# zhoupc/CNMF_E

Hardware: AMD Instinct MI355X
Metric: cnmfe_iters_per_sec (higher is better)
Workload: dtype f32; 1 GPU; c3: 512x512x10000 fp32 video, K=500, ring_radius=15, 1x1 patches of distribute_data.m (1 resident blocks per GPU), spatial=hals, deconv_flag=false, bg_ssub=1; lanes_per_rank=1, parallelism=patches round-robin over 1 rank(s)

## Files before the change

### cnmf_e_amd/csrc/api.hip

```cpp
#include "common.hpp"
#include <mutex>
#include <hip/hip_fp16.h>
#include <math.h>
#include <dlfcn.h>

namespace cnmfe {
thread_local char g_err[1024] = "";

template <class S> __device__ inline float to_f32(S v) { return (float)v; }
template <> __device__ inline float to_f32<__half>(__half v) { return __half2float(v); }

template <class S>
__global__ void k_convert(const S *__restrict__ src, float *__restrict__ dst, int64_t n) {
    int64_t i = (int64_t)blockIdx.x * blockDim.x + threadIdx.x;
    int64_t stride = (int64_t)gridDim.x * blockDim.x;
    for (; i < n; i += stride) dst[i] = to_f32<S>(src[i]);
}

__global__ void k_ymean(const float *__restrict__ Y, int64_t d_b, int64_t T, double *__restrict__ ym, float *__restrict__ ymf) {
    int64_t q = (int64_t)blockIdx.x * blockDim.x + threadIdx.x;
    if (q >= d_b) return;
    double s0 = 0, s1 = 0, s2 = 0, s3 = 0;
    int64_t t = 0;
    for (; t + 3 < T; t += 4) {
// ... 110 lines not shown
int download_traces(cnmfe_ctx *ctx, const float *dC, int64_t ldc, float *C, int32_t K, int64_t T, int order) {
    if (K == 0 || !C) return 0;
    if (order == CNMFE_BOUND || order == CNMFE_BOUND_ROWS) order = ctx->bound_order;
    if (order == CNMFE_ROWMAJOR) {
        CK(hipMemcpy2DAsync(C, T * sizeof(float), dC, ldc * sizeof(float), T * sizeof(float), K, hipMemcpyDeviceToHost, ctx->st()));
    } else {
        RET(ctx->stage.ensure((size_t)K * T * sizeof(float)));
        dim3 g((unsigned)((T + 31) / 32), (unsigned)((K + 31) / 32)), b(32, 8);
        LAUNCH(ctx, "transpose_out", k_transpose_out, g, b, 0, dC, ldc, ctx->stage.as<float>(), K, T);
        CK(hipMemcpyAsync(C, ctx->stage.p, (size_t)K * T * sizeof(float), hipMemcpyDeviceToHost, ctx->st()));
    }
    CK(hipStreamSynchronize(ctx->st()));
    return 0;
}

__global__ void __launch_bounds__(256) k_pin_copy(PinSegs s) {
    const int g = blockIdx.y;
    const uint4 *__restrict__ src = s.src[g]; uint4 *__restrict__ dst = s.dst[g];
    const unsigned n16 = s.n16[g];
    for (unsigned i = blockIdx.x * 256u + threadIdx.x; i < n16; i += gridDim.x * 256u) dst[i] = src[i];
}
static std::mutex g_pin_mu;
static std::vector<cnmfe_ctx *> g_pin_live;
void pin_register(cnmfe_ctx *ctx, bool live) {
    std::lock_guard<std::mutex> lk(g_pin_mu);
    auto it = std::find(g_pin_live.begin(), g_pin_live.end(), ctx);
    if (live && it == g_pin_live.end()) g_pin_live.push_back(ctx);
    if (!live && it != g_pin_live.end()) g_pin_live.erase(it);
}
static void flush_locked(cnmfe_ctx *ctx) {
    if (!ctx->npseg) return;
    PinSegs &pseg = ctx->pseg;
    unsigned mx = 0;
    for (int i = 0; i < ctx->npseg; ++i) mx = std::max(mx, pseg.n16[i]);
    for (int i = ctx->npseg; i < PIN_NSEG; ++i) { pseg.src[i] = nullptr; pseg.dst[i] = nullptr; pseg.n16[i] = 0; }
    const unsigned nb = std::min<unsigned>((mx + 255) / 256, 256);
    const int n = ctx->npseg; ctx->npseg = 0;
    hipLaunchKernelGGL(k_pin_copy, dim3(nb, (unsigned)n), dim3(256), 0, ctx->stream_, pseg);
}
void pin_flush_range(const void *p, size_t bytes) {
    std::lock_guard<std::mutex> lk(g_pin_mu);
    const char *lo = (const char *)p, *hi = lo + bytes;
    int cur = -1;
    for (cnmfe_ctx *c : g_pin_live) {
        bool hit = false;
        for (int i = 0; i < c->npseg && !hit; ++i) { const char *d_ = (const char *)c->pseg.dst[i]; hit = d_ >= lo && d_ < hi; }
        if (!hit) continue;
        if (cur < 0) (void)hipGetDevice(&cur);
        if (c->device != cur) (void)hipSetDevice(c->device);
        flush_locked(c);
        if (c->device != cur) (void)hipSetDevice(cur);
    }
}
void pin_flush_all() {
    std::lock_guard<std::mutex> lk(g_pin_mu);
    int cur = -1;
    for (cnmfe_ctx *c : g_pin_live) {
        if (!c->npseg) continue;
        if (cur < 0) (void)hipGetDevice(&cur);
        if (c->device != cur) (void)hipSetDevice(c->device);
        flush_locked(c);
        if (c->device != cur) (void)hipSetDevice(cur);
    }
}
int pinned_to_dev(cnmfe_ctx *ctx, void *dst, const void *src_pinned, size_t bytes) {
    if (bytes > (size_t(8) << 20)) { CK(hipMemcpyAsync(dst, src_pinned, bytes, hipMemcpyHostToDevice, ctx->st())); return 0; }
    std::lock_guard<std::mutex> lk(g_pin_mu);
    if (ctx->npseg == PIN_NSEG) flush_locked(ctx);
    const int i = ctx->npseg++;
    ctx->pseg.src[i] = (const uint4 *)src_pinned; ctx->pseg.dst[i] = (uint4 *)dst; ctx->pseg.n16[i] = (unsigned)((bytes + 15) / 16);
    return 0;
}
}
int cnmfe_ctx::copy_batch_mark() {
    hipEvent_t e;
    if (!copy_ev_pool.empty()) { e = copy_ev_pool.back(); copy_ev_pool.pop_back(); }
    else CK(hipEventCreateWithFlags(&e, hipEventDisableTiming));
    CK(hipEventRecord(e, copy_stream));
    copy_gens.push_back({++copy_gen, e});
    return 0;
}
void cnmfe_ctx::flush_copies() {
    std::lock_guard<std::mutex> lk(cnmfe::g_pin_mu);
    cnmfe::flush_locked(this);
}
namespace cnmfe {

bool bound_rows_of(const cnmfe_ctx *ctx, const float *C, int c_order, int32_t K, std::vector<int32_t> &rows) {
    rows.clear();
    if (!ctx->bound_valid || K <= 0) return false;
    if (c_order == CNMFE_BOUND) {
        if (K != ctx->bound_K) return false;
        rows.resize((size_t)K);
        for (int32_t k = 0; k < K; ++k) rows[k] = k;
        return true;
    }
    if (c_order == CNMFE_BOUND_ROWS && C) {
        const int32_t *r = reinterpret_cast<const int32_t *>(C);
        for (int32_t k = 0; k < K; ++k) if (r[k] < 0 || r[k] >= ctx->bound_K) return false;
        rows.assign(r, r + K);
        return true;
    }
    return false;
}

int ensure_ymean(cnmfe_ctx *ctx, Patch *P) {
    if (P->ymean_valid) return 0;
    if (P->frames_uploaded < P->T) return fail(CNMFE_ESTATE, "block has %lld of %lld frames uploaded", (long long)P->frames_uploaded, (long long)P->T);
    RET(P->ymean_d.ensure(P->d_b * sizeof(double)));
    RET(P->ymean_f.ensure(P->d_b * sizeof(float)));
    LAUNCH(ctx, "ymean", k_ymean, dim3((unsigned)((P->d_b + 255) / 256)), dim3(256), 0,
           P->Y.as<float>(), P->d_b, P->T, P->ymean_d.as<double>(), P->ymean_f.as<float>());
    P->Tc = (P->T + 3) / 4;
    RET(P->Yc4.ensure((size_t)P->Tc * P->d_b * sizeof(float4)));
    LAUNCH(ctx, "center4", k_center4, dim3((unsigned)((P->d_b + 255) / 256), (unsigned)P->Tc), dim3(256), 0,
           P->Y.as<float>(), P->ymean_f.as<float>(), P->d_b, P->T, P->Yc4.as<float4>());
    CK(hipStreamSynchronize(ctx->st()));
    (void)hipFree(P->Y.p); P->Y.p = nullptr; P->Y.cap = 0;
    P->ymean_valid = true;
    return 0;
}

__global__ void k_ring_pmax(const float *__restrict__ W, int64_t d, int p, int *__restrict__ pmax) {
    int64_t m = (int64_t)blockIdx.x * blockDim.x + threadIdx.x;
    int c = 0;
    if (m < d) {
        int i = 0;
        for (; i + 16 <= p; i += 16) {
            float w[16];
#pragma unroll
            for (int u = 0; u < 16; ++u) w[u] = W[(int64_t)(i + u) * d + m];
#pragma unroll
            for (int u = 0; u < 16; ++u) c += w[u] > 0.f;
        }
        for (; i < p; ++i) c += W[(int64_t)i * d + m] > 0.f;
    }
    for (int o = 32; o > 0; o >>= 1) { int v = __shfl_xor(c, o); c = v > c ? v : c; }
    if ((threadIdx.x & 63) == 0) atomicMax(pmax, c);
}
static bool first_run_of_row(const Patch *P, const float *row0) {
    std::vector<float> u;
    const int r = P->prect[0], c = P->prect[2];
    int nvalid = 0;
    for (int i = 0; i < P->p; ++i) {
        const int rr = r + P->dr[i], cc = c + P->dc[i];
        if (rr < 1 || rr > P->d1 || cc < 1 || cc > P->d2) continue;
        ++nvalid; u.push_back(row0[i]);
    }
    if (nvalid < P->d_b) u.push_back(0.f);
    std::sort(u.begin(), u.end());
    u.erase(std::unique(u.begin(), u.end()), u.end());
    return u.size() == 2;
}
int ring_stats_enqueue(cnmfe_ctx *ctx, Patch *P) {
    const size_t bytes = 64 + (size_t)P->p * sizeof(float);
    if (!P->stat_host) CK(hipHostMalloc(&P->stat_host, bytes, hipHostMallocDefault));
    if (!P->stat_ev) CK(hipEventCreateWithFlags(&P->stat_ev, hipEventDisableTiming));
    RET(P->stat_dev.ensure(64));
    CK(hipMemsetAsync(P->stat_dev.p, 0, 64, ctx->st()));
    LAUNCH(ctx, "ring_pmax", k_ring_pmax, dim3((unsigned)((P->d + 255) / 256)), dim3(256), 0, P->W.as<float>(), P->d, P->p, P->stat_dev.as<int>());
    CK(hipMemcpyAsync(P->stat_host, P->stat_dev.p, sizeof(int), hipMemcpyDeviceToHost, ctx->st()));
    CK(hipMemcpy2DAsync((char *)P->stat_host + 64, sizeof(float), P->W.p, P->d * sizeof(float), sizeof(float), P->p, hipMemcpyDeviceToHost, ctx->st()));
    CK(hipEventRecord(P->stat_ev, ctx->st()));
    P->stat_valid = true;
    return 0;
}
int ring_stats_get(cnmfe_ctx *ctx, Patch *P, int *pmax, bool *first) {
    if (!P->stat_valid) RET(ring_stats_enqueue(ctx, P));
    CK(hipEventSynchronize(P->stat_ev));
    if (pmax) *pmax = *reinterpret_cast<const int *>(P->stat_host);
    if (first) *first = first_run_of_row(P, reinterpret_cast<const float *>((const char *)P->stat_host + 64));
    return 0;
}

int ring_first_run(cnmfe_ctx *ctx, Patch *P, bool *first) { return ring_stats_get(ctx, P, nullptr, first); }
int ctx_errflag(cnmfe_ctx *ctx, int **dflag) {
    if (!ctx->errflag.p) {
        RET(ctx->errflag.ensure(sizeof(int)));
        CK(hipMemsetAsync(ctx->errflag.p, 0, sizeof(int), ctx->st()));
    }
    *dflag = ctx->errflag.as<int>();
    return 0;
}
static int errflag_raise(cnmfe_ctx *ctx, int h, bool taken = false) {
    if (!taken) CK(hipMemsetAsync(ctx->errflag.p, 0, sizeof(int), ctx->st()));
    for (auto &kv : ctx->patches) { Patch *q = kv.second; q->ysig_valid = false; q->ysig_virtual = false; q->pend = false; q->res_ac = false; q->res_kind = 0; q->pt_valid = false; }
    ctx->bgs_patch = -1;
    if (h & 2) return fail(CNMFE_EUNSUPPORTED, "a pixel's ring touches more than 256 footprints of A_prev (flag %d)", h);
    if (h & 4) return fail(CNMFE_EUNSUPPORTED, "bg_ssub > 1: a pixel's interpolation window meets more than 64 footprints of A_prev (flag %d)", h);
    return fail(CNMFE_ESTATE, "a kernel met an inconsistent table (flag %d): the ring regression needed a block pair the covariance table does not hold", h);
}
int ctx_check_errflag(cnmfe_ctx *ctx) {
    if (!ctx->errflag.p) { CK(hipStreamSynchronize(ctx->st())); return 0; }
    int h = 0;
    CK(hipMemcpyAsync(&h, ctx->errflag.p, sizeof(int), hipMemcpyDeviceToHost, ctx->st()));
    CK(hipStreamSynchronize(ctx->st()));
    if (!h) return 0;
    return errflag_raise(ctx, h);
}
__global__ void k_flag_take(int *__restrict__ flag, int *__restrict__ out) { *out = atomicExch(flag, 0); }
__global__ void __launch_bounds__(256) k_fetch_take(const uint4 *__restrict__ src, uint4 *__restrict__ dst, unsigned n16, int *__restrict__ flag, int *__restrict__ flag_out) {
    for (unsigned i = blockIdx.x * 256u + threadIdx.x; i < n16; i += gridDim.x * 256u) dst[i] = src[i];
    if (flag && blockIdx.x == 0 && threadIdx.x == 0) *flag_out = atomicExch(flag, 0);
}

__global__ void __launch_bounds__(256) k_stitch_add(const float *__restrict__ craw, int64_t ldc, const float *__restrict__ aa, const int *__restrict__ ind,
                                                    float *__restrict__ acc, int64_t ld, int64_t T) {
    const int j = blockIdx.y;
    const float w = aa[j];
    float *row = acc + (int64_t)ind[j] * ld;
    const int64_t t = (int64_t)blockIdx.x * 256 + threadIdx.x;
    if (t < T) row[t] += w * craw[(int64_t)j * ldc + t];
    if (t == 0) row[ld - 4] += w;
}
__global__ void __launch_bounds__(256) k_stitch_finish(const float *__restrict__ acc, int64_t ld, int64_t T, int subtract_min, float *__restrict__ out, int64_t ldc) {
    const int k = blockIdx.x;
    const float *row = acc + (int64_t)k * ld;
    float w = row[ld - 4];
    if (w == 0.f) w = 1.f;
    float mn = INFINITY;
    for (int64_t t = threadIdx.x; t < T; t += 256) mn = fminf(mn, row[t] / w);
    __shared__ float red[256];
    red[threadIdx.x] = mn; __syncthreads();
    for (int o = 128; o > 0; o >>= 1) { if ((int)threadIdx.x < o) red[threadIdx.x] = fminf(red[threadIdx.x], red[threadIdx.x + o]); __syncthreads(); }
    const float sub = subtract_min ? red[0] : 0.f;
    for (int64_t t = threadIdx.x; t < ldc; t += 256) out[(int64_t)k * ldc + t] = t < T ? row[t] / w - sub : 0.f;
}

struct Rccl {
    void *h = nullptr;
    int (*CommInitAll)(void **, int, const int *) = nullptr;
    int (*AllReduce)(const void *, void *, size_t, int, int, void *, hipStream_t) = nullptr;
    int (*GroupStart)() = nullptr; int (*GroupEnd)() = nullptr; int (*CommDestroy)(void *) = nullptr;
    const char *(*GetErrorString)(int) = nullptr;
    int load() {
        if (h) return 0;
        for (const char *n : {"librccl.so.1", "librccl.so", "/opt/rocm/lib/librccl.so.1"}) { h = dlopen(n, RTLD_NOW | RTLD_GLOBAL); if (h) break; }
        if (!h) return fail(CNMFE_EUNSUPPORTED, "cnmfe_stitch_temporal over several GPUs needs RCCL (librccl.so not found: %s)", dlerror());
        CommInitAll = (decltype(CommInitAll))dlsym(h, "ncclCommInitAll"); AllReduce = (decltype(AllReduce))dlsym(h, "ncclAllReduce");
        GroupStart = (decltype(GroupStart))dlsym(h, "ncclGroupStart"); GroupEnd = (decltype(GroupEnd))dlsym(h, "ncclGroupEnd");
        CommDestroy = (decltype(CommDestroy))dlsym(h, "ncclCommDestroy"); GetErrorString = (decltype(GetErrorString))dlsym(h, "ncclGetErrorString");
        if (!CommInitAll || !AllReduce || !GroupStart || !GroupEnd || !CommDestroy) { h = nullptr; return fail(CNMFE_EUNSUPPORTED, "librccl.so lacks the ncclCommInitAll / ncclAllReduce / ncclGroup* symbols"); }
        return 0;
    }
};
static Rccl g_rccl;
static int stitch_finish_one(cnmfe_ctx *ctx, int subtract_min, float *C_raw_out, int c_order, bool async_copy = false) {
    if (!ctx->stitch_open) return fail(CNMFE_ESTATE, "cnmfe_stitch_begin has not been called");
    const int32_t K = ctx->stitch_K; const int64_t T = ctx->stitch_T, ldc = (T + 3) & ~int64_t(3);
    CK(hipSetDevice(ctx->device));
    GlobalScope gs_(ctx); if (gs_.rc) return gs_.rc;
    RET(ctx->bound.ensure((size_t)std::max<int64_t>(1, (int64_t)K * ldc) * sizeof(float)));
    if (ctx->copy_pending) { CK(hipStreamWaitEvent(ctx->st(), ctx->ev_copy_done, 0)); ctx->copy_pending = false; }
    if (K > 0) LAUNCH(ctx, "stitch_finish", k_stitch_finish, dim3((unsigned)K), dim3(256), 0, ctx->stitch.as<float>(), ctx->stitch_ld, T, subtract_min, ctx->bound.as<float>(), ldc);
    ctx->bound_K = K; ctx->bound_T = T; ctx->bound_order = (c_order == CNMFE_COLMAJOR) ? CNMFE_COLMAJOR : CNMFE_ROWMAJOR; ctx->bound_valid = K > 0;
    ++ctx->bound_gen;
    ctx->stitch_open = false;
    if (C_raw_out && async_copy && K > 0) {
        if (!ctx->copy_stream) {
            CK(hipStreamCreateWithFlags(&ctx->copy_stream, hipStreamNonBlocking));
            CK(hipEventCreateWithFlags(&ctx->ev_bound_ready, hipEventDisableTiming));
            CK(hipEventCreateWithFlags(&ctx->ev_copy_done, hipEventDisableTiming));
        }
        CK(hipEventRecord(ctx->ev_bound_ready, ctx->st()));
        CK(hipStreamWaitEvent(ctx->copy_stream, ctx->ev_bound_ready, 0));
        CK(hipMemcpy2DAsync(C_raw_out, T * sizeof(float), ctx->bound.p, ldc * sizeof(float), T * sizeof(float), K, hipMemcpyDeviceToHost, ctx->copy_stream));
        CK(hipEventRecord(ctx->ev_copy_done, ctx->copy_stream));
        ctx->copy_pending = true;
        RET(ctx->copy_batch_mark());
        return 0;
    }
    if (C_raw_out) RET(download_traces(ctx, ctx->bound.as<float>(), ldc, C_raw_out, K, T, c_order == CNMFE_COLMAJOR ? CNMFE_COLMAJOR : CNMFE_ROWMAJOR));
    return 0;
}

static void ring_offsets(int radius, int k, std::vector<int32_t> &dr, std::vector<int32_t> &dc) {
    dr.clear(); dc.clear();
    for (int c = -radius; c <= radius; ++c)
        for (int r = -radius; r <= radius; ++r) {
            int d2 = c * c + r * r;
            if (d2 >= radius * radius && d2 < (radius + 1) * (radius + 1)) { dr.push_back(r); dc.push_back(c); }
        }
    int n = (int)dr.size();
    if (k <= 0 || k > n) return;
    std::vector<int> ids(n);
    for (int i = 0; i < n; ++i) ids[i] = i;
    std::vector<double> ang(n);
    for (int i = 0; i < n; ++i) ang[i] = atan2((double)dr[i], (double)dc[i]);
    std::stable_sort(ids.begin(), ids.end(), [&](int a, int b) { return ang[a] < ang[b]; });
    std::vector<std::pair<int, int>> sel;
    for (int j = 0; j < k; ++j) {
        double x = (k == 1) ? 1.0 : 1.0 + (double)(n - 1) * j / (double)(k - 1);
        int idx = (int)floor(x + 0.5) - 1;
        sel.push_back({dc[ids[idx]], dr[ids[idx]]});
    }
    std::sort(sel.begin(), sel.end());
    sel.erase(std::unique(sel.begin(), sel.end()), sel.end());
    dr.clear(); dc.clear();
    for (auto &s : sel) { dc.push_back(s.first); dr.push_back(s.second); }
}
}

using namespace cnmfe;

cnmfe_ctx::~cnmfe_ctx() {
    if (rccl_comm && g_rccl.CommDestroy) { (void)hipSetDevice(device); g_rccl.CommDestroy(rccl_comm); rccl_comm = nullptr; }
    for (auto &kv : patches) delete kv.second;
    prof.drain();
    if (copy_stream) { (void)hipStreamSynchronize(copy_stream); (void)hipStreamDestroy(copy_stream); }
    if (ev_bound_ready) (void)hipEventDestroy(ev_bound_ready);
    if (ev_copy_done) (void)hipEventDestroy(ev_copy_done);
    for (auto &g : copy_gens) (void)hipEventDestroy(g.second);
    for (auto e : copy_ev_pool) (void)hipEventDestroy(e);
    cnmfe::pin_register(this, false);
    for (auto *j : tjobs) delete j;
    for (auto e : tickets) (void)hipEventDestroy(e);
    if (ticket_flags) (void)hipHostFree(ticket_flags);
    if (stream_) (void)hipStreamDestroy(stream_);
    for (auto *L : lanes) delete L;
    if (ev_fork) (void)hipEventDestroy(ev_fork);
}

void cnmfe_ctx::swap_lane(cnmfe_lane &L) {
    std::swap(stream_, L.stream_); std::swap(pseg, L.pseg); std::swap(npseg, L.npseg); pin.swap(L.pin); std::swap(spatial_nnz, L.spatial_nnz);
    for (int i = 0; i < 32; ++i) vp[i].swap(L.vp[i]);
    std::swap(last_ldc, L.last_ldc);
    ysig_low.swap(L.ysig_low); up_tmp.swap(L.up_tmp); bgs_r.swap(L.bgs_r); bgs_b.swap(L.bgs_b); bgs_upr.swap(L.bgs_upr); bgs_upc.swap(L.bgs_upc);
    std::swap(bgs_patch, L.bgs_patch); std::swap(bgs_d1s, L.bgs_d1s); std::swap(bgs_dF, L.bgs_dF);
    bf.swap(L.bf); dig_smax.swap(L.dig_smax); dig_rspart.swap(L.dig_rspart); dig_scale.swap(L.dig_scale); tdig.swap(L.tdig); tscale.swap(L.tscale); gk.swap(L.gk);
    win_items.swap(L.win_items); bf2.swap(L.bf2); outl_cnt.swap(L.outl_cnt); outl_sel.swap(L.outl_sel); cov.swap(L.cov); rowsum.swap(L.rowsum);
    for (int i = 0; i < 16; ++i) tmp[i].swap(L.tmp[i]);
    for (int i = 0; i < 7; ++i) inc[i].swap(L.inc[i]);
    for (int i = 0; i < 4; ++i) stg[i].swap(L.stg[i]);
    wcodes.swap(L.wcodes); solve_fill.swap(L.solve_fill); stage.swap(L.stage);
    for (int i = 0; i < 24; ++i) scr[i].swap(L.scr[i]);
    dscr.swap(L.dscr);
}
int cnmfe_ctx::activate(int lane) {
    if (lanes.empty() || lane == cur_lane) {
        if (!lanes.empty() && lane != 0 && lanes[lane]->fork_seen != fork_gen) {
            CK(hipStreamWaitEvent(stream_, ev_fork, 0)); lanes[lane]->fork_seen = fork_gen;
        }
        if (!lanes.empty() && lane != 0) lanes[lane]->dirty = true;
        return 0;
    }
    if (lane < 0 || lane >= (int)lanes.size()) return fail(CNMFE_ESTATE, "lane %d of %d", lane, (int)lanes.size());
    if (npseg) flush_copies();
    swap_lane(*lanes[cur_lane]);
    swap_lane(*lanes[lane]);
    cur_lane = lane;
    if (lane != 0) {
        if (lanes[lane]->fork_seen != fork_gen) { CK(hipStreamWaitEvent(stream_, ev_fork, 0)); lanes[lane]->fork_seen = fork_gen; }
        lanes[lane]->dirty = true;
    }
    return 0;
}
int cnmfe_ctx::join_lanes() {
    if (lanes.empty()) return 0;
    for (int l = 1; l < (int)lanes.size(); ++l) {
        if (!lanes[l]->dirty) continue;
        RET(activate(l));
        CK(hipEventRecord(lanes[l]->ev, st()));
    }
    RET(activate(0));
    for (int l = 1; l < (int)lanes.size(); ++l)
        if (lanes[l]->dirty) { CK(hipStreamWaitEvent(st(), lanes[l]->ev, 0)); lanes[l]->dirty = false; }
    return 0;
}
int cnmfe_ctx::fork_mark() {
    if (lanes.empty()) return 0;
    RET(activate(0));
    CK(hipEventRecord(ev_fork, st()));
    ++fork_gen;
    return 0;
}
static int lanes_set(cnmfe_ctx *ctx, int64_t n) {
    if (n < 1 || n > 4) return fail(CNMFE_EINVAL, "option lanes = %lld: 1 .. 4", (long long)n);
    if (!ctx->patches.empty() && (int)std::max<size_t>(1, ctx->lanes.size()) != n) return fail(CNMFE_ESTATE, "option lanes is set before the first patch is created");
    if (n == 1 || (int)ctx->lanes.size() == n) return 0;
    CK(hipSetDevice(ctx->device));
    for (int l = 0; l < n; ++l) {
        cnmfe_lane *L = new cnmfe_lane();
        ctx->lanes.push_back(L);
        CK(hipEventCreateWithFlags(&L->ev, hipEventDisableTiming));
        if (l == 0) continue;
        CK(hipStreamCreate(&L->stream_));
        hipLaunchKernelGGL(k_scratch_warm, dim3(1), dim3(64), 0, L->stream_, (int *)nullptr, 3);
        CK(hipStreamSynchronize(L->stream_));
        if (L->pin.init(size_t(64) << 20) != 0) return fail(CNMFE_EHIP, "pinned staging arena (64 MB) of lane %d could not be allocated", l);
    }
    CK(hipEventCreateWithFlags(&ctx->ev_fork, hipEventDisableTiming));
    CK(hipEventRecord(ctx->ev_fork, ctx->st()));
    return 0;
}

extern "C" {

const char *cnmfe_last_error(void) { return g_err; }
const char *cnmfe_version(void) { return "cnmfe-mi355x 0.1 (gfx950)"; }

cnmfe_ctx *cnmfe_create(int device) {
    int n = 0;
    hipError_t e = hipGetDeviceCount(&n);
    if (e != hipSuccess || n <= 0) { fail(CNMFE_EHIP, "no HIP device visible (%s)", hipGetErrorString(e)); return nullptr; }
    if (device < 0 || device >= n) { fail(CNMFE_EINVAL, "device %d out of range (0..%d)", device, n - 1); return nullptr; }
    if (hipSetDevice(device) != hipSuccess) { fail(CNMFE_EHIP, "hipSetDevice(%d) failed", device); return nullptr; }
    cnmfe_ctx *ctx = new cnmfe_ctx();
    ctx->device = device;
    if (hipStreamCreate(&ctx->stream_) != hipSuccess) { fail(CNMFE_EHIP, "hipStreamCreate failed"); delete ctx; return nullptr; }
    if (hipStreamCreateWithFlags(&ctx->copy_stream, hipStreamNonBlocking) != hipSuccess || hipEventCreateWithFlags(&ctx->ev_bound_ready, hipEventDisableTiming) != hipSuccess ||
        hipEventCreateWithFlags(&ctx->ev_copy_done, hipEventDisableTiming) != hipSuccess) { fail(CNMFE_EHIP, "copy stream / events could not be created"); delete ctx; return nullptr; }
    pin_register(ctx, true);
    if (ctx->pin.init(size_t(64) << 20) != 0) { fail(CNMFE_EHIP, "pinned staging arena (64 MB) could not be allocated"); delete ctx; return nullptr; }
    hipLaunchKernelGGL(k_scratch_warm, dim3(1), dim3(64), 0, ctx->stream_, (int *)nullptr, 3);
    hipLaunchKernelGGL(k_scratch_warm, dim3(1), dim3(64), 0, ctx->copy_stream, (int *)nullptr, 3);
    (void)hipStreamSynchronize(ctx->stream_); (void)hipStreamSynchronize(ctx->copy_stream); (void)hipGetLastError();
    (void)tu_warm_resid(); (void)tu_warm_bg(); (void)tu_warm_factor(); (void)tu_warm_deconv(); (void)tu_warm_ssub(); (void)tu_warm_vproj();
    if (const char *env = getenv("CNMFE_OPTS")) {
        std::string s(env), applied, ignored;
        size_t pos = 0;
        while (pos < s.size()) {
            size_t end = s.find(',', pos); if (end == std::string::npos) end = s.size();
            const std::string kv = s.substr(pos, end - pos); pos = end + 1;
            const size_t eq = kv.find('=');
            if (eq == std::string::npos || eq == 0) continue;
            const int rc_ = cnmfe_set_option(ctx, kv.substr(0, eq).c_str(), strtoll(kv.c_str() + eq + 1, nullptr, 10));
            (rc_ == 0 ? applied : ignored) += (rc_ == 0 ? (applied.empty() ? "" : ",") : (ignored.empty() ? "" : ",")) + kv;
        }
        static bool said = false;
        if (!said) { said = true; fprintf(stderr, "[cnmfe] CNMFE_OPTS applied to every context: %s%s%s\n", applied.empty() ? "(none)" : applied.c_str(), ignored.empty() ? "" : "; not known to this build, ignored: ", ignored.c_str()); }
    }
    return ctx;
}

void cnmfe_destroy(cnmfe_ctx *ctx) {
    if (!ctx) return;
    (void)hipSetDevice(ctx->device);
    (void)ctx->join_lanes();
    (void)hipStreamSynchronize(ctx->st());
    delete ctx;
}

int cnmfe_synchronize(cnmfe_ctx *ctx) {
    if (!ctx) return fail(CNMFE_EINVAL, "null context");
    RET(ctx->join_lanes());
    CK(hipStreamSynchronize(ctx->st()));
    if (ctx->copy_stream) CK(hipStreamSynchronize(ctx->copy_stream));
    return ctx_check_errflag(ctx);
}

int cnmfe_set_option(cnmfe_ctx *ctx, const char *name, int64_t value) {
    if (!ctx || !name) return fail(CNMFE_EINVAL, "null argument");
    static const char *known[] = {"r1_variant", "r1_delta", "r1_lazy", "r1_defer", "r1_virtual", "gram_incremental", "prealloc", "solve_packed", "sweep_dag", "win_i8_planes", "solve_staged", "solve_inv", "solve_inv_terms", "gram_i8", "win_i8", "proj_tiled", "proj_i8", "proj_i8_planes", "ssub_virtual",
                                  "solve_probe", "r1_probe", "deconv_trace", "host_trace", "debug", nullptr};
    if (!strcmp(name, "lanes")) { RET(lanes_set(ctx, value)); ctx->opts[name] = value; return 0; }
    for (int i = 0; known[i]; ++i) if (!strcmp(known[i], name)) { ctx->opts[name] = value; if (!strcmp(name, "host_trace")) ctx->trace_level = (int)value; return 0; }
    return fail(CNMFE_EINVAL, "unknown option '%s'", name);
}

int cnmfe_patch_create(cnmfe_ctx *ctx, int patch_id, const int32_t pr[4], const int32_t br[4], int32_t d1, int32_t d2, int64_t T) {
    if (!ctx || !pr || !br) return fail(CNMFE_EINVAL, "null argument");
    if (d1 <= 0 || d2 <= 0 || T <= 0) return fail(CNMFE_EINVAL, "bad dims d1=%d d2=%d T=%lld", d1, d2, (long long)T);
    if (!(1 <= br[0] && br[0] <= pr[0] && pr[0] <= pr[1] && pr[1] <= br[1] && br[1] <= d1 &&
          1 <= br[2] && br[2] <= pr[2] && pr[2] <= pr[3] && pr[3] <= br[3] && br[3] <= d2))
        return fail(CNMFE_EINVAL, "patch [%d %d %d %d] must lie inside block [%d %d %d %d] inside the %dx%d FOV",
                    pr[0], pr[1], pr[2], pr[3], br[0], br[1], br[2], br[3], d1, d2);
    CK(hipSetDevice(ctx->device));
    if (ctx->patches.count(patch_id)) { delete ctx->patches[patch_id]; ctx->patches.erase(patch_id); }
    Patch *P = new Patch();
    P->lane = ctx->lanes.empty() ? 0 : (ctx->patches_created++ % (int)ctx->lanes.size());
    memcpy(P->prect, pr, sizeof(P->prect)); memcpy(P->brect, br, sizeof(P->brect));
    P->d1 = d1; P->d2 = d2; P->T = T;
    P->nr = pr[1] - pr[0] + 1; P->nc = pr[3] - pr[2] + 1;
    P->nr_b = br[1] - br[0] + 1; P->nc_b = br[3] - br[2] + 1;
    P->roff = pr[0] - br[0]; P->coff = pr[2] - br[2];
    P->d = (int64_t)P->nr * P->nc; P->d_b = (int64_t)P->nr_b * P->nc_b;
    int rc = P->Y.ensure((size_t)P->d_b * T * sizeof(float));
    if (rc) { delete P; return rc; }
    if (hipMemsetAsync(P->Y.p, 0, (size_t)P->d_b * T * sizeof(float), ctx->st()) != hipSuccess) { delete P; return fail(CNMFE_EHIP, "hipMemsetAsync of the upload staging failed"); }
    P->frame_seen.assign((size_t)T, 0);
    P->Tc = (T + 3) / 4;
    ctx->patches[patch_id] = P;
    return 0;
}

int cnmfe_upload_block(cnmfe_ctx *ctx, int patch_id, const void *Y, int dtype, int memspace, int64_t t0, int64_t nt) {
    if (!ctx || !Y) return fail(CNMFE_EINVAL, "null argument");
    Patch *P = get_patch(ctx, patch_id);
    if (!P) return fail(CNMFE_ESTATE, "patch %d not created", patch_id);
    if (t0 < 0 || nt <= 0 || t0 + nt > P->T) return fail(CNMFE_EINVAL, "frames [%lld,%lld) outside [0,%lld)", (long long)t0, (long long)(t0 + nt), (long long)P->T);
    CK(hipSetDevice(ctx->device));
    size_t esz = dtype == CNMFE_F32 ? 4 : dtype == CNMFE_F64 ? 8 : dtype == CNMFE_U16 ? 2 : dtype == CNMFE_U8 ? 1 : dtype == CNMFE_F16 ? 2 : 0;
    if (!esz) return fail(CNMFE_EINVAL, "unknown dtype %d", dtype);
    if (memspace != CNMFE_HOST && memspace != CNMFE_DEVICE) return fail(CNMFE_EINVAL, "unknown memspace %d", memspace);
    if (!P->Y.p) {
        RET(P->Y.ensure((size_t)P->d_b * P->T * sizeof(float)));
        CK(hipMemsetAsync(P->Y.p, 0, (size_t)P->d_b * P->T * sizeof(float), ctx->st()));
        P->frames_uploaded = 0;
        P->frame_seen.assign((size_t)P->T, 0);
    }
    for (int64_t t = t0; t < t0 + nt; ++t)
        if (P->frame_seen[(size_t)t]) return fail(CNMFE_EINVAL, "frame %lld of patch %d was already uploaded (chunks must not overlap; re-create the patch to replace its video)", (long long)t, patch_id);
    float *dst = P->Y.as<float>() + t0 * P->d_b;
    int64_t n = nt * P->d_b;
    if (dtype == CNMFE_F32) {
        CK(hipMemcpyAsync(dst, Y, (size_t)n * 4, memspace == CNMFE_HOST ? hipMemcpyHostToDevice : hipMemcpyDeviceToDevice, ctx->st()));
    } else {
        const int64_t slab = int64_t(1) << 26;
        for (int64_t o = 0; o < n; o += slab) {
            int64_t m = std::min(slab, n - o);
            const void *src = (const char *)Y + (size_t)o * esz;
            if (memspace == CNMFE_HOST) {
                RET(ctx->stage.ensure((size_t)m * esz));
                CK(hipMemcpyAsync(ctx->stage.p, src, (size_t)m * esz, hipMemcpyHostToDevice, ctx->st()));
                src = ctx->stage.p;
            }
            dim3 g((unsigned)std::min<int64_t>((m + 255) / 256, 65535)), b(256);
            switch (dtype) {
                case CNMFE_F64: LAUNCH(ctx, "convert", k_convert<double>, g, b, 0, (const double *)src, dst + o, m); break;
                case CNMFE_U16: LAUNCH(ctx, "convert", k_convert<uint16_t>, g, b, 0, (const uint16_t *)src, dst + o, m); break;
                case CNMFE_U8:  LAUNCH(ctx, "convert", k_convert<uint8_t>, g, b, 0, (const uint8_t *)src, dst + o, m); break;
                default:        LAUNCH(ctx, "convert", k_convert<__half>, g, b, 0, (const __half *)src, dst + o, m); break;
            }
            if (memspace == CNMFE_HOST) CK(hipStreamSynchronize(ctx->st()));
        }
    }
    CK(hipStreamSynchronize(ctx->st()));
    std::fill(P->frame_seen.begin() + t0, P->frame_seen.begin() + t0 + nt, (uint8_t)1);
    P->frames_uploaded += nt;
    P->ymean_valid = false; P->ysig_valid = false; P->base_valid = false; P->base_alt_valid = false; P->sys_valid = false; P->sys_alt_valid = false; P->kinv_valid = false; P->kinv_lam_valid = false; P->kinv_fits = 0; P->pt_valid = false; P->dig_valid = false; P->digp_valid = false; P->yt4_valid = false;
    return 0;
}

int cnmfe_get_ymean(cnmfe_ctx *ctx, int patch_id, double *out) {
    if (!ctx || !out) return fail(CNMFE_EINVAL, "null argument");
    Patch *P = get_patch(ctx, patch_id);
    if (!P) return fail(CNMFE_ESTATE, "patch %d not created", patch_id);
    CK(hipSetDevice(ctx->device));
    RET(ensure_ymean(ctx, P));
    CK(hipMemcpyAsync(out, P->ymean_d.p, P->d_b * sizeof(double), hipMemcpyDeviceToHost, ctx->st()));
    CK(hipStreamSynchronize(ctx->st()));
    return 0;
}

int cnmfe_ring_init(cnmfe_ctx *ctx, int patch_id, int32_t radius, int32_t num_neighbors) {
    if (!ctx) return fail(CNMFE_EINVAL, "null context");
    Patch *P = get_patch(ctx, patch_id);
    if (!P) return fail(CNMFE_ESTATE, "patch %d not created", patch_id);
    if (radius < 1 || radius > 64) return fail(CNMFE_EINVAL, "ring radius %d out of range", radius);
    CK(hipSetDevice(ctx->device));
    std::vector<int32_t> ndr, ndc;
    ring_offsets(radius, num_neighbors, ndr, ndc);
    const int32_t np_ = (int32_t)ndr.size();
    if (np_ < 1) return fail(CNMFE_EINVAL, "ring of radius %d has no neighbours", radius);
    if (np_ > PMAX_RING) return fail(CNMFE_EUNSUPPORTED, "ring with %d neighbours exceeds the supported %d", np_, PMAX_RING);
    if (radius > 24) return fail(CNMFE_EUNSUPPORTED, "ring radius %d: the block-pair covariance table of the ring regression covers radii <= 24", radius);
    int h = radius;
    if ((P->prect[0] - P->brect[0] < std::min(h, P->prect[0] - 1)) || (P->brect[1] - P->prect[1] < std::min(h, P->d1 - P->prect[1])) ||
        (P->prect[2] - P->brect[2] < std::min(h, P->prect[2] - 1)) || (P->brect[3] - P->prect[3] < std::min(h, P->d2 - P->prect[3])))
        return fail(CNMFE_EINVAL, "block halo is narrower than the ring radius %d", radius);
    P->ring_ready = false;
    P->dr.swap(ndr); P->dc.swap(ndc); P->p = np_; P->radius = radius;
    RET(to_dev(ctx, P->ring_dr, P->dr.data(), P->dr.size()));
    RET(to_dev(ctx, P->ring_dc, P->dc.data(), P->dc.size()));
    RET(P->W.ensure((size_t)P->p * P->d * sizeof(float)));
    RET(P->b0.ensure(P->d * sizeof(double)));
// ... 86 lines not shown
int cnmfe_b0_get(cnmfe_ctx *ctx, int patch_id, float *b0) {
    if (!ctx || !b0) return fail(CNMFE_EINVAL, "null argument");
    Patch *P = get_patch(ctx, patch_id);
    if (!P || !P->ring_ready) return fail(CNMFE_ESTATE, "ring of patch %d not initialised", patch_id);
    CK(hipSetDevice(ctx->device));
    std::vector<double> tmp(P->d);
    CK(hipMemcpyAsync(tmp.data(), P->b0.p, P->d * sizeof(double), hipMemcpyDeviceToHost, ctx->st()));
    CK(hipStreamSynchronize(ctx->st()));
    for (int64_t i = 0; i < P->d; ++i) b0[i] = (float)tmp[i];
    return 0;
}

int cnmfe_b0_set(cnmfe_ctx *ctx, int patch_id, const float *b0) {
    if (!ctx || !b0) return fail(CNMFE_EINVAL, "null argument");
    Patch *P = get_patch(ctx, patch_id);
    if (!P || !P->ring_ready) return fail(CNMFE_ESTATE, "ring of patch %d not initialised", patch_id);
    CK(hipSetDevice(ctx->device));
    std::vector<double> tmp(P->d);
    for (int64_t i = 0; i < P->d; ++i) tmp[i] = (double)b0[i];
    CK(hipMemcpyAsync(P->b0.p, tmp.data(), P->d * sizeof(double), hipMemcpyHostToDevice, ctx->st()));
    CK(hipStreamSynchronize(ctx->st()));
    P->ysig_valid = false;
    return 0;
}

static int check_csc(const char *what, int32_t K, int64_t nrow, const int64_t *colptr, const int32_t *rowidx) {
    if (K < 0) return fail(CNMFE_EINVAL, "%s: K=%d", what, K);
    if (K == 0) return 0;
    if (!colptr) return fail(CNMFE_EINVAL, "%s: null colptr", what);
    if (colptr[0] != 0) return fail(CNMFE_EINVAL, "%s: colptr[0] != 0", what);
    for (int32_t k = 0; k < K; ++k) if (colptr[k + 1] < colptr[k]) return fail(CNMFE_EINVAL, "%s: colptr not monotone at %d", what, k);
    int64_t nnz = colptr[K];
    if (nnz && !rowidx) return fail(CNMFE_EINVAL, "%s: null rowidx", what);
    for (int32_t k = 0; k < K; ++k)
        for (int64_t e = colptr[k]; e < colptr[k + 1]; ++e) {
            if (rowidx[e] < 0 || rowidx[e] >= nrow) return fail(CNMFE_EINVAL, "%s: row index %d out of [0,%lld)", what, rowidx[e], (long long)nrow);
            if (e > colptr[k] && rowidx[e] <= rowidx[e - 1]) return fail(CNMFE_EINVAL, "%s: rows of column %d not strictly ascending", what, k);
        }
    return 0;
}
extern "C++" { namespace cnmfe { int check_csc_pub(const char *what, int32_t ncol, int64_t nrow, const int64_t *colptr, const int32_t *rowidx) { return check_csc(what, ncol, nrow, colptr, rowidx); } } }

int cnmfe_ring_solve_stats(cnmfe_ctx *ctx, int patch_id, int64_t out[4]) {
    if (!ctx || !out) return fail(CNMFE_EINVAL, "null argument");
    Patch *P = get_patch(ctx, patch_id);
    if (!P) return fail(CNMFE_EINVAL, "no patch %d", patch_id);
    out[0] = out[1] = out[2] = out[3] = -1;
    if (!P->kinv_valid || !P->kinv_list.p) return 0;
    CK(hipSetDevice(ctx->device));
    int h[4];
    CK(hipMemcpyAsync(h, P->kinv_list.as<int>() + 2 * P->d, sizeof(h), hipMemcpyDeviceToHost, ctx->st()));
    CK(hipStreamSynchronize(ctx->st()));
    for (int i = 0; i < 4; ++i) out[i] = h[i];
    return 0;
}

int cnmfe_fit_ring_model(cnmfe_ctx *ctx, int patch_id, int32_t K, const int64_t *A_colptr, const int32_t *A_rowidx,
                         const float *A_val, const float *C, int c_order, double thresh_outlier, int with_projection,
                         float *b0_out, int64_t info[4]) {
    if (!ctx) return fail(CNMFE_EINVAL, "null context");
    Patch *P = get_patch(ctx, patch_id);
    if (!P || !P->ring_ready) return fail(CNMFE_ESTATE, "ring of patch %d not initialised", patch_id);
    RET(check_csc("A", K, P->d_b, A_colptr, A_rowidx));
    if (K > 0 && ((!A_val && A_colptr[K] > 0) || (!C && c_order != CNMFE_BOUND))) return fail(CNMFE_EINVAL, "null A_val / C");
    CK(hipSetDevice(ctx->device));
    RET(ensure_ymean(ctx, P));
    int64_t dummy[4];
    int rc = bg_fit_ring(ctx, P, K, A_colptr, A_rowidx, A_val, C, c_order, with_projection, b0_out, info ? info : dummy, 0, thresh_outlier);
    P->ysig_valid = false;
    return rc;
}

int cnmfe_fit_reserve(cnmfe_ctx *ctx, int patch_id) {
    if (!ctx) return fail(CNMFE_EINVAL, "null context");
    Patch *P = get_patch(ctx, patch_id);
    if (!P || !P->ring_ready) return fail(CNMFE_ESTATE, "ring of patch %d not initialised", patch_id);
    CK(hipSetDevice(ctx->device));
    if (ctx->opt("prealloc", 1) == 0) return 0;
    return bg_reserve(ctx, P);
}

int cnmfe_set_noise(cnmfe_ctx *ctx, int patch_id, const float *sn_block) {
    if (!ctx) return fail(CNMFE_EINVAL, "null context");
    Patch *P = get_patch(ctx, patch_id);
    if (!P) return fail(CNMFE_ESTATE, "patch %d not created", patch_id);
    if (!sn_block) return fail(CNMFE_EINVAL, "null sn_block");
    CK(hipSetDevice(ctx->device));
    RET(to_dev(ctx, P->sn_b, sn_block, (size_t)P->d_b));
    CK(hipStreamSynchronize(ctx->st()));
    P->sn_ready = true;
    return 0;
}

int cnmfe_residual(cnmfe_ctx *ctx, int patch_id, int32_t Ksel, const int64_t *A_colptr, const int32_t *A_rowidx,
                   const float *A_val, const float *C, int c_order, float *Ysig_out, int out_memspace) {
    if (!ctx) return fail(CNMFE_EINVAL, "null context");
    Patch *P = get_patch(ctx, patch_id);
    if (!P || !P->ring_ready) return fail(CNMFE_ESTATE, "ring of patch %d not initialised", patch_id);
    RET(check_csc("A_prev", Ksel, P->d_b, A_colptr, A_rowidx));
    if (Ksel > 0 && ((!A_val && A_colptr[Ksel] > 0) || (!C && c_order != CNMFE_BOUND))) return fail(CNMFE_EINVAL, "null A_val / C");
    CK(hipSetDevice(ctx->device));
    RET(ensure_ymean(ctx, P));
    return residual_run(ctx, P, patch_id, Ksel, A_colptr, A_rowidx, A_val, C, c_order, Ysig_out, out_memspace);
}

int cnmfe_get_sn(cnmfe_ctx *ctx, int patch_id, float *sn_out) {
    if (!ctx) return fail(CNMFE_EINVAL, "null context");
    Patch *P = get_patch(ctx, patch_id);
    if (!P) return fail(CNMFE_ESTATE, "patch %d not created", patch_id);
    if (!P->ysig_valid) return fail(CNMFE_ESTATE, "cnmfe_residual has not been run for patch %d", patch_id);
    RET(residual_materialize(ctx, P));
    if (!sn_out) return fail(CNMFE_EINVAL, "null sn_out");
    CK(hipSetDevice(ctx->device));
    return sn_pixels_run(ctx, P, sn_out);
}

int cnmfe_estimate_noise(cnmfe_ctx *ctx, int patch_id, int64_t nframes, float *sn_block_out) {
    if (!ctx) return fail(CNMFE_EINVAL, "null context");
    Patch *P = get_patch(ctx, patch_id);
    if (!P) return fail(CNMFE_ESTATE, "patch %d not created", patch_id);
    if (!sn_block_out) return fail(CNMFE_EINVAL, "null sn_block_out");
    CK(hipSetDevice(ctx->device));
    RET(ensure_ymean(ctx, P));
    return sn_video_run(ctx, P, nframes, sn_block_out);
}

int cnmfe_update_spatial(cnmfe_ctx *ctx, int patch_id, int algorithm, int32_t K, const int64_t *A_colptr,
                         const int32_t *A_rowidx, const float *A_val, const float *C, int c_order,
                         const int64_t *IND_colptr, const int32_t *IND_rowidx, const float *sn, int32_t param, float *A_out) {
    if (!ctx) return fail(CNMFE_EINVAL, "null context");
    Patch *P = get_patch(ctx, patch_id);
    if (!P) return fail(CNMFE_ESTATE, "patch %d not created", patch_id);
    if (!P->ysig_valid) return fail(CNMFE_ESTATE, "cnmfe_residual has not been run for patch %d", patch_id);
    if (algorithm < CNMFE_SPATIAL_HALS || algorithm > CNMFE_SPATIAL_NNLS) return fail(CNMFE_EINVAL, "unknown spatial algorithm %d", algorithm);
    if (K <= 0) return fail(CNMFE_EINVAL, "K=%d", K);
    RET(check_csc("A", K, P->d, A_colptr, A_rowidx));
    RET(check_csc("IND", K, P->d, IND_colptr, IND_rowidx));
    if (!C && c_order != CNMFE_BOUND) return fail(CNMFE_EINVAL, "null C");
    if (algorithm == CNMFE_SPATIAL_HALS_THRESH && !sn) return fail(CNMFE_EINVAL, "HALS_THRESH needs sn");
    if (param <= 0) return fail(CNMFE_EINVAL, "maxIter/maxN must be positive");
    CK(hipSetDevice(ctx->device));
    ctx->spatial_lane = P->lane;
    return spatial_run(ctx, P, algorithm, K, A_colptr, A_rowidx, A_val, C, c_order, IND_colptr, IND_rowidx, sn, param, A_out);
}

int cnmfe_update_spatial_fetch(cnmfe_ctx *ctx, float *A_out, int64_t nnz) {
    if (!ctx) return fail(CNMFE_EINVAL, "null context");
    if (!A_out && nnz) return fail(CNMFE_EINVAL, "null A_out");
    CK(hipSetDevice(ctx->device));
    RET(ctx->activate(ctx->spatial_lane));
    return spatial_fetch(ctx, A_out, nnz);
}

static int ticket_record(cnmfe_ctx *ctx, int64_t *ticket, const void *src = nullptr, void *dst_pinned = nullptr, size_t bytes = 0) {
    size_t t = 0;
    while (t < ctx->tickets.size() && ctx->ticket_busy[t]) ++t;
    if (t == ctx->tickets.size()) {
        hipEvent_t e; CK(hipEventCreateWithFlags(&e, hipEventDisableTiming));
        ctx->tickets.push_back(e); ctx->ticket_busy.push_back(0);
    }
    const bool flagged = ctx->errflag.p && t < cnmfe_ctx::TICKET_FLAGS;
    if (flagged) {
        if (!ctx->ticket_flags) { CK(hipHostMalloc((void **)&ctx->ticket_flags, cnmfe_ctx::TICKET_FLAGS * sizeof(int), hipHostMallocDefault)); memset(ctx->ticket_flags, 0, cnmfe_ctx::TICKET_FLAGS * sizeof(int)); }
        ctx->ticket_flags[t] = 0;
    }
    if (bytes) {
        const unsigned n16 = (unsigned)((bytes + 15) / 16), nb = std::min<unsigned>((n16 + 255) / 256, 64);
        hipLaunchKernelGGL(k_fetch_take, dim3(nb), dim3(256), 0, ctx->st(), (const uint4 *)src, (uint4 *)dst_pinned, n16, flagged ? ctx->errflag.as<int>() : (int *)nullptr,
                           flagged ? ctx->ticket_flags + t : (int *)nullptr);
    } else if (flagged) {
        RET(ctx->ticket_dev.ensure(cnmfe_ctx::TICKET_FLAGS * sizeof(int)));
        hipLaunchKernelGGL(k_flag_take, dim3(1), dim3(1), 0, ctx->st(), ctx->errflag.as<int>(), ctx->ticket_dev.as<int>() + t);
        CK(hipMemcpyAsync(&ctx->ticket_flags[t], ctx->ticket_dev.as<int>() + t, sizeof(int), hipMemcpyDeviceToHost, ctx->st()));
    }
    CK(hipEventRecord(ctx->tickets[t], ctx->st()));
    ctx->ticket_busy[t] = 1;
    *ticket = (int64_t)t;
    return 0;
}

int cnmfe_update_spatial_fetch_async(cnmfe_ctx *ctx, float *A_out_pinned, int64_t nnz, int64_t *ticket) {
    if (!ctx || !ticket) return fail(CNMFE_EINVAL, "null context / ticket");
    if (!A_out_pinned && nnz) return fail(CNMFE_EINVAL, "null A_out");
    CK(hipSetDevice(ctx->device));
    RET(ctx->activate(ctx->spatial_lane));
    if (ctx->spatial_nnz < 0 || nnz != ctx->spatial_nnz) return fail(CNMFE_ESTATE, "no deferred spatial update of %lld values (last one: %lld)", (long long)nnz, (long long)ctx->spatial_nnz);
    return ticket_record(ctx, ticket, ctx->scr[6].p, A_out_pinned, (size_t)nnz * sizeof(float));
}

int cnmfe_ticket_wait(cnmfe_ctx *ctx, int64_t ticket) {
    if (!ctx) return fail(CNMFE_EINVAL, "null context");
    if (ticket < 0 || (size_t)ticket >= ctx->tickets.size() || !ctx->ticket_busy[ticket]) return fail(CNMFE_ESTATE, "ticket %lld is not outstanding", (long long)ticket);
    CK(hipSetDevice(ctx->device));
    CK(hipEventSynchronize(ctx->tickets[ticket]));
    ctx->ticket_busy[ticket] = 0;
    if ((size_t)ticket >= cnmfe_ctx::TICKET_FLAGS) return ctx_check_errflag(ctx);
    if (ctx->ticket_flags && ctx->ticket_flags[ticket]) {
        const int h = ctx->ticket_flags[ticket];
        ctx->ticket_flags[ticket] = 0;
        return errflag_raise(ctx, h, true);
    }
    return 0;
}

int cnmfe_update_spatial_fetch_connected(cnmfe_ctx *ctx, int32_t d1, int32_t d2, int32_t K, const int64_t *IND_colptr, const int32_t *IND_rowidx,
                                         float *A_out, uint8_t *keep_out) {
    if (!ctx) return fail(CNMFE_EINVAL, "null context");
    if (K <= 0 || d1 <= 0 || d2 <= 0) return fail(CNMFE_EINVAL, "bad K / d1 / d2");
    RET(check_csc("IND", K, (int64_t)d1 * d2, IND_colptr, IND_rowidx));
    if (IND_colptr[K] && (!A_out || !keep_out)) return fail(CNMFE_EINVAL, "null A_out / keep_out");
    CK(hipSetDevice(ctx->device));
    RET(ctx->activate(ctx->spatial_lane));
    return spatial_fetch_connected(ctx, d1, d2, K, IND_colptr, IND_rowidx, A_out, keep_out);
}

int cnmfe_update_spatial_fetch_connected_async(cnmfe_ctx *ctx, int32_t d1, int32_t d2, int32_t K, const int64_t *IND_colptr, const int32_t *IND_rowidx,
                                               float *A_out_pinned, uint8_t *keep_out_pinned, int64_t *ticket) {
    if (!ctx || !ticket) return fail(CNMFE_EINVAL, "null context / ticket");
    if (K <= 0 || d1 <= 0 || d2 <= 0) return fail(CNMFE_EINVAL, "bad K / d1 / d2");
    RET(check_csc("IND", K, (int64_t)d1 * d2, IND_colptr, IND_rowidx));
    if (IND_colptr[K] && (!A_out_pinned || !keep_out_pinned)) return fail(CNMFE_EINVAL, "null A_out / keep_out");
    CK(hipSetDevice(ctx->device));
    RET(ctx->activate(ctx->spatial_lane));
    RET(spatial_fetch_connected(ctx, d1, d2, K, IND_colptr, IND_rowidx, A_out_pinned, keep_out_pinned, false));
    return ticket_record(ctx, ticket);
}

int cnmfe_hals_temporal(cnmfe_ctx *ctx, int patch_id, int32_t K, const int64_t *A_colptr, const int32_t *A_rowidx,
                        const float *A_val, const float *C_in, int c_order, int32_t maxIter,
                        float *C_out, float *C_raw_out, float *aa_out) {
    if (!ctx) return fail(CNMFE_EINVAL, "null context");
    Patch *P = get_patch(ctx, patch_id);
    if (!P) return fail(CNMFE_ESTATE, "patch %d not created", patch_id);
    if (!P->ysig_valid) return fail(CNMFE_ESTATE, "cnmfe_residual has not been run for patch %d", patch_id);
    if (K <= 0) return fail(CNMFE_EINVAL, "K=%d", K);
    RET(check_csc("A", K, P->d, A_colptr, A_rowidx));
    if ((!A_val && A_colptr[K] > 0) || (!C_in && c_order != CNMFE_BOUND)) return fail(CNMFE_EINVAL, "null A_val / C_in");
    if (maxIter <= 0) return fail(CNMFE_EINVAL, "maxIter must be positive");
    CK(hipSetDevice(ctx->device));
    return temporal_run(ctx, P, K, A_colptr, A_rowidx, A_val, C_in, c_order, maxIter, C_out, C_raw_out, aa_out, nullptr, nullptr, nullptr, nullptr);
}

int cnmfe_hals_temporal_deconv(cnmfe_ctx *ctx, int patch_id, int32_t K, const int64_t *A_colptr, const int32_t *A_rowidx,
                               const float *A_val, const float *C_in, int c_order, int32_t maxIter, const cnmfe_deconv_opts *opts,
                               float *kernel_pars, float *C_out, float *C_raw_out, float *S_out, float *sn_out, float *aa_out) {
    if (!ctx) return fail(CNMFE_EINVAL, "null context");
    Patch *P = get_patch(ctx, patch_id);
    if (!P) return fail(CNMFE_ESTATE, "patch %d not created", patch_id);
    if (!P->ysig_valid) return fail(CNMFE_ESTATE, "cnmfe_residual has not been run for patch %d", patch_id);
    if (K <= 0) return fail(CNMFE_EINVAL, "K=%d", K);
    RET(check_csc("A", K, P->d, A_colptr, A_rowidx));
    if ((!A_val && A_colptr[K] > 0) || (!C_in && c_order != CNMFE_BOUND) || !opts || !kernel_pars) return fail(CNMFE_EINVAL, "null A_val / C_in / opts / kernel_pars");
    if (maxIter <= 0) return fail(CNMFE_EINVAL, "maxIter must be positive");
    CK(hipSetDevice(ctx->device));
    return temporal_run(ctx, P, K, A_colptr, A_rowidx, A_val, C_in, c_order, maxIter, C_out, C_raw_out, aa_out, opts, kernel_pars, S_out, sn_out);
}

int cnmfe_fast_temporal(cnmfe_ctx *ctx, int patch_id, int32_t K, const int64_t *A_colptr, const int32_t *A_rowidx, const float *A_val,
                        int c_order, float *C_raw_out, float *aa_out) {
    if (!ctx) return fail(CNMFE_EINVAL, "null context");
    Patch *P = get_patch(ctx, patch_id);
    if (!P) return fail(CNMFE_ESTATE, "patch %d not created", patch_id);
    if (!P->ysig_valid) return fail(CNMFE_ESTATE, "cnmfe_residual has not been run for patch %d", patch_id);
    RET(residual_materialize(ctx, P));
    if (K <= 0) return fail(CNMFE_EINVAL, "K=%d", K);
    RET(check_csc("A", K, P->d, A_colptr, A_rowidx));
    if (!A_val && A_colptr[K] > 0) return fail(CNMFE_EINVAL, "null A_val");
    CK(hipSetDevice(ctx->device));
    return fast_temporal_run(ctx, P, K, A_colptr, A_rowidx, A_val, c_order, C_raw_out, aa_out);
}

int cnmfe_compute_rss(cnmfe_ctx *ctx, int patch_id, int32_t K, const int64_t *A_colptr, const int32_t *A_rowidx, const float *A_val,
                      const float *C, int c_order, const float *b0_block, const float *b0_new, double *rss_out) {
    if (!ctx) return fail(CNMFE_EINVAL, "null context");
    Patch *P = get_patch(ctx, patch_id);
    if (!P) return fail(CNMFE_ESTATE, "patch %d not created", patch_id);
    if (!P->ysig_valid) return fail(CNMFE_ESTATE, "cnmfe_residual has not been run for patch %d", patch_id);
    if (P->res_kind != 1) return fail(CNMFE_EUNSUPPORTED, "compute_RSS needs the residual of cnmfe_residual (bg_ssub = 1)");
    if (K < 0 || !b0_block || !b0_new || !rss_out) return fail(CNMFE_EINVAL, "bad K / null b0_block / b0_new / rss_out");
    if (K > 0) {
        RET(check_csc("A", K, P->d, A_colptr, A_rowidx));
        if ((!A_val && A_colptr[K] > 0) || (!C && c_order != CNMFE_BOUND)) return fail(CNMFE_EINVAL, "null A_val / C");
    }
    CK(hipSetDevice(ctx->device));
    return rss_run(ctx, P, K, A_colptr, A_rowidx, A_val, C, c_order, b0_block, b0_new, rss_out);
}

int cnmfe_reconstruct_background(cnmfe_ctx *ctx, int patch_id, const float *b0_block, const float *b0_new, int64_t frame0, int64_t nframes,
                                  float *Ybg_out, int out_memspace) {
    if (!ctx) return fail(CNMFE_EINVAL, "null context");
    Patch *P = get_patch(ctx, patch_id);
    if (!P) return fail(CNMFE_ESTATE, "patch %d not created", patch_id);
    if (!P->ysig_valid) return fail(CNMFE_ESTATE, "cnmfe_residual has not been run for patch %d", patch_id);
    if (P->res_kind != 1) return fail(CNMFE_EUNSUPPORTED, "reconstruct_background needs the residual of cnmfe_residual (bg_ssub = 1)");
    if (!b0_block || !b0_new || !Ybg_out) return fail(CNMFE_EINVAL, "null b0_block / b0_new / Ybg_out");
    if (frame0 < 0 || nframes <= 0 || frame0 + nframes > P->T || nframes > 65535) return fail(CNMFE_EINVAL, "frames [%lld, %lld) outside [0, %lld) or more than 65535 at once", (long long)frame0, (long long)(frame0 + nframes), (long long)P->T);
    CK(hipSetDevice(ctx->device));
    return bg_reconstruct_run(ctx, P, b0_block, b0_new, frame0, nframes, Ybg_out, out_memspace);
}

int cnmfe_stitch_begin(cnmfe_ctx *ctx, int32_t K, int64_t T) {
    if (!ctx) return fail(CNMFE_EINVAL, "null context");
    if (K < 0 || T <= 0) return fail(CNMFE_EINVAL, "bad K / T");
    CK(hipSetDevice(ctx->device));
    GlobalScope gs_(ctx); if (gs_.rc) return gs_.rc;
    const int64_t ld = ((T + 3) & ~int64_t(3)) + 4;
    RET(ctx->stitch.ensure((size_t)std::max<int64_t>(1, (int64_t)K * ld) * sizeof(float)));
    CK(hipMemsetAsync(ctx->stitch.p, 0, (size_t)std::max<int64_t>(1, (int64_t)K * ld) * sizeof(float), ctx->st()));
    ctx->stitch_K = K; ctx->stitch_T = T; ctx->stitch_ld = ld; ctx->stitch_open = true;
    ctx->tjobs_used = 0;
    return 0;
}

int cnmfe_hals_temporal_job(cnmfe_ctx *ctx, int patch_id, int32_t K, const int64_t *A_colptr, const int32_t *A_rowidx, const float *A_val,
                            const float *C_in, int c_order, int32_t maxIter, const cnmfe_deconv_opts *opts, const float *kernel_pars, int32_t *job_out) {
    if (!ctx || !job_out) return fail(CNMFE_EINVAL, "null context / job_out");
    Patch *P = get_patch(ctx, patch_id);
    if (!P) return fail(CNMFE_ESTATE, "patch %d not created", patch_id);
    if (!P->ysig_valid) return fail(CNMFE_ESTATE, "cnmfe_residual has not been run for patch %d", patch_id);
    if (!ctx->stitch_open) return fail(CNMFE_ESTATE, "cnmfe_stitch_begin has not been called (it opens a round of temporal jobs)");
    if (K <= 0) return fail(CNMFE_EINVAL, "K=%d", K);
    RET(check_csc("A", K, P->d, A_colptr, A_rowidx));
    if ((!A_val && A_colptr[K] > 0) || (!C_in && c_order != CNMFE_BOUND) || (opts && !kernel_pars)) return fail(CNMFE_EINVAL, "null A_val / C_in / kernel_pars");
    if (maxIter <= 0) return fail(CNMFE_EINVAL, "maxIter must be positive");
    CK(hipSetDevice(ctx->device));
    if (ctx->tjobs_used == (int)ctx->tjobs.size()) ctx->tjobs.push_back(new TemporalJob());
    TemporalJob *job = ctx->tjobs[ctx->tjobs_used];
    job->K = 0; job->swept = false;
    RET(temporal_run(ctx, P, K, A_colptr, A_rowidx, A_val, C_in, c_order, maxIter, nullptr, nullptr, nullptr, opts, const_cast<float *>(kernel_pars), nullptr, nullptr, job));
    *job_out = ctx->tjobs_used++;
    return 0;
}
int cnmfe_temporal_jobs_sweep(cnmfe_ctx *ctx) {
    if (!ctx) return fail(CNMFE_EINVAL, "null context");
    CK(hipSetDevice(ctx->device));
    GlobalScope gs_(ctx); if (gs_.rc) return gs_.rc;
    return temporal_sweep_jobs(ctx);
}
int cnmfe_stitch_add_job(cnmfe_ctx *ctx, int32_t job_id, int32_t K_m, const int32_t *ind_m) {
    if (!ctx) return fail(CNMFE_EINVAL, "null context");
    if (!ctx->stitch_open) return fail(CNMFE_ESTATE, "cnmfe_stitch_begin has not been called");
    if (job_id < 0 || job_id >= ctx->tjobs_used) return fail(CNMFE_EINVAL, "temporal job %d does not exist (%d set up since cnmfe_stitch_begin)", job_id, ctx->tjobs_used);
    TemporalJob *job = ctx->tjobs[job_id];
    if (!job->swept) return fail(CNMFE_ESTATE, "temporal job %d has not been swept (cnmfe_temporal_jobs_sweep)", job_id);
    if (K_m != job->K || !ind_m || job->T != ctx->stitch_T) return fail(CNMFE_EINVAL, "temporal job %d holds %d rows x %lld frames", job_id, job->K, (long long)job->T);
    std::vector<char> seen((size_t)ctx->stitch_K, 0);
    for (int32_t j = 0; j < K_m; ++j) {
        if (ind_m[j] < 0 || ind_m[j] >= ctx->stitch_K) return fail(CNMFE_EINVAL, "row %d outside the %d-row accumulator", ind_m[j], ctx->stitch_K);
        if (seen[ind_m[j]]) return fail(CNMFE_EINVAL, "row %d listed twice", ind_m[j]);
        seen[ind_m[j]] = 1;
    }
    CK(hipSetDevice(ctx->device));
    GlobalScope gs_(ctx); if (gs_.rc) return gs_.rc;
    RET(to_dev(ctx, ctx->scr[23], ind_m, (size_t)K_m));
    LAUNCH(ctx, "stitch_add", k_stitch_add, dim3((unsigned)((ctx->stitch_T + 255) / 256), (unsigned)K_m), dim3(256), 0, job->dCraw.as<float>(), job->ldc,
           job->dAa.as<float>(), ctx->scr[23].as<int>(), ctx->stitch.as<float>(), ctx->stitch_ld, ctx->stitch_T);
    return 0;
}

int cnmfe_stitch_add(cnmfe_ctx *ctx, int32_t K_m, const int32_t *ind_m) {
    if (!ctx) return fail(CNMFE_EINVAL, "null context");
    if (!ctx->stitch_open) return fail(CNMFE_ESTATE, "cnmfe_stitch_begin has not been called");
    if (K_m == 0) return 0;
    if (K_m < 0 || !ind_m) return fail(CNMFE_EINVAL, "bad K_m / null ind_m");
    if (!ctx->last_t_valid || ctx->last_t_K != K_m || ctx->last_t_T != ctx->stitch_T)
        return fail(CNMFE_ESTATE, "no temporal result of %d rows x %lld frames on the device (the last cnmfe_hals_temporal / cnmfe_fast_temporal call)", K_m, (long long)ctx->stitch_T);
    std::vector<char> seen((size_t)ctx->stitch_K, 0);
    for (int32_t j = 0; j < K_m; ++j) {
        if (ind_m[j] < 0 || ind_m[j] >= ctx->stitch_K) return fail(CNMFE_EINVAL, "row %d outside the %d-row accumulator", ind_m[j], ctx->stitch_K);
        if (seen[ind_m[j]]) return fail(CNMFE_EINVAL, "row %d listed twice", ind_m[j]);
        seen[ind_m[j]] = 1;
    }
    CK(hipSetDevice(ctx->device));
    GlobalScope gs_(ctx); if (gs_.rc) return gs_.rc;
    RET(to_dev(ctx, ctx->scr[23], ind_m, (size_t)K_m));
    LAUNCH(ctx, "stitch_add", k_stitch_add, dim3((unsigned)((ctx->stitch_T + 255) / 256), (unsigned)K_m), dim3(256), 0, ctx->last_craw.as<float>(), ctx->last_t_ldc,
           ctx->last_aa.as<float>(), ctx->scr[23].as<int>(), ctx->stitch.as<float>(), ctx->stitch_ld, ctx->stitch_T);
// ... 383 lines not shown
```

### cnmf_e_amd/csrc/bg.hip

```cpp
#include "common.hpp"
#include "ring_solve_core.hpp"
#include "win_proj.hpp"
#include <type_traits>

namespace cnmfe {
static inline bool win_planes3(cnmfe_ctx *ctx, int64_t T16) {
    const int64_t o = ctx->opt("win_i8_planes", 0);
    return o == 3 || (o != 4 && T16 * 16 >= 2048);
}


typedef float float4_t __attribute__((ext_vector_type(4)));

__global__ void __launch_bounds__(256) k_build_bf(const float4 *__restrict__ Y4, int64_t Tc, BgGeom g,
                                                  const int *__restrict__ arow, const int *__restrict__ acol, const float *__restrict__ aval,
                                                  const float *__restrict__ Cc, int64_t ldc, float *__restrict__ bf, int tchunk, double *__restrict__ rs) {
    const int blk = blockIdx.x;
    const int bi = blk % g.nbr, bj = blk / g.nbr;
    const int lp = threadIdx.x;
    const int lr = ((lp >> 4) & 3) * 4 + (lp & 3), lc = (lp >> 6) * 4 + ((lp >> 2) & 3);
    const int rb = bi * BLK + lr, cb = bj * BLK + lc;
    const bool in = rb < g.nr_b && cb < g.nc_b;
    const int64_t q = in ? (int64_t)cb * g.nr_b + rb : 0;
    int e0 = 0, e1 = 0;
// ... 287 lines not shown
                                                 const double *__restrict__ GK, const int *__restrict__ lst_k) {
    __shared__ double G[WIN_NLB * WF_S];
    const int blk = blk_list[blockIdx.x];
    const int l0 = lst_ptr[blk], nl = lst_ptr[blk + 1] - l0;
    const int s0 = (int)blockIdx.y * WF_S;
    if (s0 >= nl) return;
    const int lp = threadIdx.x;
    const int nlp = ((nl + 15) >> 4) << 4;
    {
        const int r = lp / WF_S, c = s0 + lp % WF_S;
        double v = 0.0;
        if (GK) {
            if (r < nl && c < nl) v = GK[(int64_t)lst_k[l0 + r] * K + lst_k[l0 + c]];
        } else if (r < nlp && c < nlp) {
            const double *gp = Gb + (int64_t)blk * WIN_NLB * WIN_NLB + r * WIN_NLB + c;
#pragma unroll 4
            for (int sg = 0; sg < nseg; ++sg) v += gp[sg * gb_stride];
        }
        G[lp] = v;
    }
    __syncthreads();
    const int lr = ((lp >> 4) & 3) * 4 + (lp & 3), lc = (lp >> 6) * 4 + ((lp >> 2) & 3);
    const int rb = (blk % g.nbr) * BLK + lr, cb = (blk / g.nbr) * BLK + lc;
    int e0 = 0, e1 = 0;
    if (rb < g.nr_b && cb < g.nc_b) { const int64_t q = (int64_t)cb * g.nr_b + rb; e0 = arow[q]; e1 = arow[q + 1]; }
    const int s1 = s0 + WF_S < nl ? s0 + WF_S : nl;
    for (int s = s0; s < s1; ++s) {
        double *u = Ut + (int64_t)(l0 + s) * BLKPX + lp;
        double v = u[0];
#pragma unroll 4
        for (int sg = 1; sg < nseg; ++sg) v += u[sg * ut_stride];
        double w = 0.0;
        for (int e = e0; e < e1; ++e) w += (double)aval[e] * G[(int)slot_of[(int64_t)blk * K + acol[e]] * WF_S + (s - s0)];
        u[0] = v - 0.5 * w;
        if (Praw) Praw[(int64_t)(l0 + s) * BLKPX + lp] = v;
    }
}
static_assert(WIN_NLB * WF_S == 256, "k_win_fix: one Gram entry per thread");

__global__ void __launch_bounds__(256) k_cov_correct(const double *__restrict__ base, double *__restrict__ cov, const int4 *__restrict__ pairs,
                                                     const unsigned short *__restrict__ needmask, BgGeom g, int K, const int *__restrict__ arow,
                                                     const int *__restrict__ acol, const float *__restrict__ aval, const int *__restrict__ lst_ptr,
                                                     const short *__restrict__ slot_of, const double *__restrict__ Ut) {
    const int pair = blockIdx.x;
    const int4 pr = pairs[pair];
    const int ba = pr.x, bb = pr.y, rel = pr.z;
    const int half = threadIdx.x >> 7, ty = (threadIdx.x >> 3) & 15, tx = (threadIdx.x & 7) * 2;
    const int la = lst_ptr[ba], lb = lst_ptr[bb];
    auto pix = [&](int blk, int lp, int &e0, int &e1) {
        const int lr = ((lp >> 4) & 3) * 4 + (lp & 3), lc = (lp >> 6) * 4 + ((lp >> 2) & 3);
        const int rb = (blk % g.nbr) * BLK + lr, cb = (blk / g.nbr) * BLK + lc;
        e0 = e1 = 0;
        if (rb < g.nr_b && cb < g.nc_b) { const int64_t q = (int64_t)cb * g.nr_b + rb; e0 = arow[q]; e1 = arow[q + 1]; }
    };
    const double *bp = base + (int64_t)pair * BLKPX * BLKPX;
    double *cp = cov + (int64_t)pair * BLKPX * BLKPX;
    const int pi0 = (int)blockIdx.y * (16 / (int)gridDim.y), pi1 = pi0 + 16 / (int)gridDim.y;
    for (int pi = pi0 + half; pi < pi1; pi += 2) {
        const unsigned mask = needmask[rel * 16 + pi];
        if (!mask) continue;
        const int ilp = pi * 16 + ty;
        int ei0, ei1; pix(ba, ilp, ei0, ei1);
        for (int pj = 0; pj < 16; ++pj) {
            if (!((mask >> pj) & 1u)) continue;
            const int jlp = pj * 16 + tx;
            int ej0, ej1, ek0, ek1; pix(bb, jlp, ej0, ej1); pix(bb, jlp + 1, ek0, ek1);
            const int idx = ilp * BLKPX + jlp;
            double2 v = *reinterpret_cast<const double2 *>(bp + idx);
            for (int e = ej0; e < ej1; ++e) v.x -= (double)aval[e] * Ut[(int64_t)(la + slot_of[(int64_t)ba * K + acol[e]]) * BLKPX + ilp];
            for (int e = ek0; e < ek1; ++e) v.y -= (double)aval[e] * Ut[(int64_t)(la + slot_of[(int64_t)ba * K + acol[e]]) * BLKPX + ilp];
            for (int e = ei0; e < ei1; ++e) {
                const double2 u = *reinterpret_cast<const double2 *>(Ut + (int64_t)(lb + slot_of[(int64_t)bb * K + acol[e]]) * BLKPX + jlp);
                v.x -= (double)aval[e] * u.x; v.y -= (double)aval[e] * u.y;
            }
            *reinterpret_cast<double2 *>(cp + idx) = v;
        }
    }
}

__global__ void __launch_bounds__(256) k_rowsum_correct(const double *__restrict__ base, double *__restrict__ rs, BgGeom g, const int *__restrict__ arow,
                                                        const int *__restrict__ acol, const float *__restrict__ aval, const double *__restrict__ csum) {
    const int blk = blockIdx.x, lp = threadIdx.x;
    const int lr = ((lp >> 4) & 3) * 4 + (lp & 3), lc = (lp >> 6) * 4 + ((lp >> 2) & 3);
    const int rb = (blk % g.nbr) * BLK + lr, cb = (blk / g.nbr) * BLK + lc;
    double v = base[(int64_t)blk * BLKPX + lp];
    if (rb < g.nr_b && cb < g.nc_b) {
        const int64_t q = (int64_t)cb * g.nr_b + rb;
        for (int e = arow[q]; e < arow[q + 1]; ++e) v -= (double)aval[e] * csum[acol[e]];
    }
    rs[(int64_t)blk * BLKPX + lp] = v;
}

struct CovTab {
    const double *cov; const int *pair_of;
    const int *wcodes; int woff;
    int nbr, nbc;
    int maxd, nrel;
};
__host__ __device__ __forceinline__ int rel_index(int dR, int dC, int maxd) { return dC == 0 ? dR : (maxd + 1) + (dC - 1) * (2 * maxd + 1) + dR + maxd; }
__host__ __device__ __forceinline__ int nrel_of(int maxd) { return (maxd + 1) + maxd * (2 * maxd + 1); }

__global__ void __launch_bounds__(256) k_win_codes(const int *__restrict__ pair_of, int nbr, int nbc, int woff, int maxd, int nrel, int *__restrict__ wcodes) {
    const int br0 = (int)(blockIdx.x % (nbr + 2 * woff)) - woff, bc0 = (int)(blockIdx.x / (nbr + 2 * woff)) - woff;
    const int q = threadIdx.x, a = q >> 4, b = q & 15;
    int ia = br0 + (a & 3), ja = bc0 + (a >> 2), ib = br0 + (b & 3), jb = bc0 + (b >> 2);
    int code = -1;
    if (ia >= 0 && ja >= 0 && ib >= 0 && jb >= 0 && ia < nbr && ib < nbr && ja < nbc && jb < nbc) {
        int dR = ib - ia, dC = jb - ja, sw = 0;
        if (dC < 0 || (dC == 0 && dR < 0)) { sw = 1; ia = ib; ja = jb; dR = -dR; dC = -dC; }
        if (dC <= maxd && dR <= maxd && dR >= -maxd) {
            const int pidx = pair_of[(ja * nbr + ia) * nrel + rel_index(dR, dC, maxd)];
            code = pidx < 0 ? -1 : ((pidx << 2) | (sw << 1) | ((dR == 0 && dC == 0) ? 1 : 0));
        }
    }
    wcodes[(int64_t)blockIdx.x * 256 + q] = code;
}
}
#include "ring_solve.hpp"
#include "ring_solve_packed.hpp"
#include "ring_solve_inv.hpp"
#include "ring_solve_staged.hpp"
#include "gram_i8.hpp"
#include "win_proj_i8.hpp"
namespace cnmfe {

__global__ void k_active(const float *__restrict__ W, BgGeom g, const int *__restrict__ dr, const int *__restrict__ dc,
                         const float *__restrict__ asum, unsigned char *__restrict__ active, int *__restrict__ nactive) {
    int64_t m = (int64_t)blockIdx.x * blockDim.x + threadIdx.x;
    int on = 0;
    if (m < g.d) {
        const int rbm = (int)(m % g.nr) + g.roff, cbm = (int)(m / g.nr) + g.coff;
        float s = 0.f;
        for (int i0 = 0; i0 < g.p; i0 += 8) {
            float w8[8], a8[8];
#pragma unroll
            for (int u = 0; u < 8; ++u) {
                const int i = i0 + u < g.p ? i0 + u : g.p - 1;
                const int rb = rbm + dr[i], cb = cbm + dc[i];
                const bool in = i0 + u < g.p && rb >= 0 && rb < g.nr_b && cb >= 0 && cb < g.nc_b;
                w8[u] = W[(int64_t)i * g.d + m];
                a8[u] = asum[in ? (int64_t)cb * g.nr_b + rb : 0];
                if (!in) w8[u] = 0.f;
            }
#pragma unroll
            for (int u = 0; u < 8; ++u) if (w8[u] != 0.f) s += fabsf(w8[u]) * a8[u];
        }
        on = s > 0.f;
        active[m] = (unsigned char)on;
    }
    unsigned long long b = __ballot(on);
    if ((threadIdx.x & 63) == 0) atomicAdd(nactive, (int)__popcll(b));
}

__global__ void k_b0(const double *__restrict__ ymean, BgGeom g, const int *__restrict__ arow, const int *__restrict__ acol,
                     const float *__restrict__ aval, const double *__restrict__ Cmean, double *__restrict__ b0) {
    int64_t m = (int64_t)blockIdx.x * blockDim.x + threadIdx.x;
    if (m >= g.d) return;
    const int64_t q = (int64_t)((int)(m / g.nr) + g.coff) * g.nr_b + (int)(m % g.nr) + g.roff;
    double v = ymean[q];
    if (arow) for (int e = arow[q]; e < arow[q + 1]; ++e) v -= (double)aval[e] * Cmean[acol[e]];
    b0[m] = v;
}

__device__ __forceinline__ int64_t bf4_index(const BgGeom &g, int rb, int cb, int64_t c) {
    return ((int64_t)((cb >> 4) * g.nbr + (rb >> 4)) * (g.Tpad >> 2) + c) * BLKPX + lp_of(rb & 15, cb & 15);
}
__global__ void __launch_bounds__(256) k_outlier_clip(const float4 *__restrict__ bf, float4 *__restrict__ bf2, BgGeom g, const int *__restrict__ dr,
                                                      const int *__restrict__ dc, const float *__restrict__ W, const float *__restrict__ sn_b,
                                                      double thresh, int *__restrict__ cnt) {
    const int64_t m = (int64_t)blockIdx.x * blockDim.x + threadIdx.x, c = blockIdx.y;
    if (m >= g.d) return;
    const int rbm = (int)(m % g.nr) + g.roff, cbm = (int)(m / g.nr) + g.coff;
    double o0 = 0, o1 = 0, o2 = 0, o3 = 0;
    for (int i = 0; i < g.p; ++i) {
        const float w = W[(int64_t)i * g.d + m];
        if (w == 0.f) continue;
        const float4 v = bf[bf4_index(g, rbm + dr[i], cbm + dc[i], c)];
        o0 += (double)w * v.x; o1 += (double)w * v.y; o2 += (double)w * v.z; o3 += (double)w * v.w;
    }
    const int64_t at = bf4_index(g, rbm, cbm, c);
    float4 y = bf[at];
    const double lim = thresh * (double)sn_b[(int64_t)cbm * g.nr_b + rbm];
    const int64_t t = c * 4;
    if (t < g.T && (double)y.x > o0 + lim) { y.x = (float)o0; atomicAdd(&cnt[t], 1); }
    if (t + 1 < g.T && (double)y.y > o1 + lim) { y.y = (float)o1; atomicAdd(&cnt[t + 1], 1); }
    if (t + 2 < g.T && (double)y.z > o2 + lim) { y.z = (float)o2; atomicAdd(&cnt[t + 2], 1); }
    if (t + 3 < g.T && (double)y.w > o3 + lim) { y.w = (float)o3; atomicAdd(&cnt[t + 3], 1); }
    bf2[at] = y;
}
__global__ void __launch_bounds__(256) k_select_frames(const float *__restrict__ src, int64_t Tpad_src, float *__restrict__ dst, int64_t Tpad_dst,
                                                       const int *__restrict__ sel, int64_t nsel) {
    const int64_t blk = blockIdx.x, lp = threadIdx.x;
    for (int64_t c = blockIdx.y; c < (Tpad_dst >> 2); c += gridDim.y) {
        float v[4];
        for (int i = 0; i < 4; ++i) {
            const int64_t j = c * 4 + i;
            float x = 0.f;
            if (j < nsel) { const int64_t t = sel[j]; x = src[((blk * (Tpad_src >> 2) + (t >> 2)) * BLKPX + lp) * 4 + (t & 3)]; }
            v[i] = x;
        }
        reinterpret_cast<float4 *>(dst)[(blk * (Tpad_dst >> 2) + c) * BLKPX + lp] = make_float4(v[0], v[1], v[2], v[3]);
    }
}
static double matlab_quantile(std::vector<int> x, double q) {
    std::sort(x.begin(), x.end());
    const int64_t n = (int64_t)x.size();
    const double r = q * (double)n + 0.5;
    if (r <= 1.0) return x[0];
    if (r >= (double)n) return x[n - 1];
    const int64_t lo = (int64_t)std::floor(r);
    return x[lo - 1] + (r - (double)lo) * (double)(x[lo] - x[lo - 1]);
}

static int solve_launch(cnmfe_ctx *ctx, Patch *P, const CovTab &tab, const BgGeom &g, const double *rowsum, const unsigned char *act, int nt, int probe, const double *fill) {
    const unsigned ngrid = (unsigned)P->d;
    const int *pix = nullptr;
    int *dErr = nullptr;
    RET(ctx_errflag(ctx, &dErr));
#define RS5_CASE(NT_) case NT_: LAUNCH(ctx, "bg_ring_solve", (k_ring_solve5<NT_>), dim3(ngrid), dim3(64), 0, tab, g, P->ring_dr.as<int>(), \
                                        P->ring_dc.as<int>(), rowsum, act, P->W.as<float>(), dErr, probe, pix, fill); break;
    switch (nt) { RS5_CASE(1) RS5_CASE(2) RS5_CASE(3) RS5_CASE(4) RS5_CASE(5) RS5_CASE(6) RS5_CASE(7) RS5_CASE(8) default: break; }
#undef RS5_CASE
    return 0;
}

int bg_reserve(cnmfe_ctx *ctx, Patch *P) {
    if (ctx->opt("gram_incremental", 1) == 0 || P->p <= 0) return 0;
    int p_radius = 0;
    for (int i = 0; i < P->p; ++i) p_radius = std::max(p_radius, std::max(std::abs(P->dr[i]), std::abs(P->dc[i])));
    const int maxd = (2 * p_radius + 15) >> 4;
    if (maxd > 3) return 0;
    const int nbr = (P->nr_b + BLK - 1) / BLK, nbc = (P->nc_b + BLK - 1) / BLK, nblk = nbr * nbc;
    const int pi0 = std::max(0, P->roff - p_radius) / BLK, pi1 = std::min(P->nr_b - 1, P->roff + P->nr - 1 + p_radius) / BLK;
    const int pj0 = std::max(0, P->coff - p_radius) / BLK, pj1 = std::min(P->nc_b - 1, P->coff + P->nc - 1 + p_radius) / BLK;
    int64_t npairs = 0;
    for (int j = pj0; j <= pj1; ++j)
        for (int i = pi0; i <= pi1; ++i)
            for (int dC = 0; dC <= maxd; ++dC)
                for (int dR = (dC == 0 ? 0 : -maxd); dR <= maxd; ++dR) {
                    const int i2 = i + dR, j2 = j + dC;
                    if (i2 >= pi0 && i2 <= pi1 && j2 >= pj0 && j2 <= pj1) ++npairs;
                }
    const bool i8 = ctx->opt("gram_i8", 1) != 0 && P->T <= 24576;
    const int64_t Tpad = i8 ? (P->T + 4 * GK - 1) / (4 * GK) * (4 * GK) : (P->T + GK - 1) / GK * GK;
    const size_t tab = (size_t)npairs * BLKPX * BLKPX * sizeof(double);
    RET(P->cov_base.ensure(tab));
    RET(P->rowsum_base.ensure((size_t)nblk * BLKPX * sizeof(double)));
    RET(ctx->cov.ensure(tab));
    RET(ctx->rowsum.ensure((size_t)nblk * BLKPX * sizeof(double)));
    RET(ctx->bf.ensure((size_t)nblk * Tpad * BLKPX * sizeof(float)));
    const int nsg = nblk >= 512 ? std::max(1, std::min(8, (2048 + nblk - 1) / nblk)) : std::max(1, std::min(16, (4096 + nblk - 1) / std::max(1, nblk)));
    RET(ctx->inc[6].ensure((size_t)nsg * nblk * WIN_NLB * WIN_NLB * sizeof(double)));
    const int nt = (P->p + 15) / 16;
    if (ctx->opt("solve_packed", 1) != 0 && nt >= 1 && nt <= 8) {
        const size_t sys_bytes = (size_t)P->d * ((size_t)(nt * (nt + 1) / 2) * 256 + 16 * nt) * sizeof(double);
        if (P->sys.cap < sys_bytes) {
            size_t fr = 0, tot = 0;
            CK(hipMemGetInfo(&fr, &tot));
            if (fr >= sys_bytes + ((size_t)8 << 30)) { P->sys_valid = false; P->kinv_valid = false; P->kinv_lam_valid = false; P->kinv_fits = 0; RET(P->sys.ensure(sys_bytes)); }
        }
    }
    auto reserve = [&](DevBuf &b, size_t bytes) -> int {
        if (b.cap >= bytes) return 0;
        size_t fr = 0, tot = 0;
        CK(hipMemGetInfo(&fr, &tot));
        if (fr >= bytes + std::max((size_t)8 << 30, tot / 4)) RET(b.ensure(bytes));
        return 0;
    };
    const bool stride1 = P->T / std::max<int64_t>(1, std::min<int64_t>(P->T, (int64_t)P->p * 100)) <= 1;
    if (!P->derived) {
        const bool planes = i8 && stride1 && ctx->opt("win_i8", 1) != 0;
        const bool pi8 = planes && ctx->opt("proj_i8", 1) != 0;
        if (planes) { RET(reserve(P->dig, (size_t)nblk * Tpad * BLKPX * sizeof(float))); RET(P->dig_sc.ensure((size_t)nblk * BLKPX * sizeof(double))); }
        if (ctx->opt("r1_virtual", 1) != 0) {
            if (pi8) RET(reserve(P->digp, (size_t)nblk * Tpad * BLKPX * sizeof(float)));
            else if (ctx->opt("proj_tiled", 1) != 0) RET(reserve(P->yt4, (size_t)nblk * ((P->Tc + 15) >> 4) * 64 * 64 * sizeof(float4)));
        }
    }
    return 0;
}

int bg_fit_ring(cnmfe_ctx *ctx, Patch *P, int32_t K, const int64_t *A_colptr, const int32_t *A_rowidx, const float *A_val,
                const float *C, int c_order, int with_projection, float *b0_out, int64_t info[4], int b0_only, double thresh_outlier) {
    HostTrace ht(ctx, "fit_ring");
    const bool outl = thresh_outlier == thresh_outlier;
    if (outl && !P->sn_ready && !(b0_only & 1)) return fail(CNMFE_ESTATE, "fit_ring_model with thresh_outlier needs the noise levels of the block (cnmfe_set_noise)");
    const int64_t T = P->T;
    const int p = P->p;
    DevBuf &dC = ctx->tmp[0], &dCc = ctx->tmp[1], &dCm = ctx->tmp[2], &dArow = ctx->tmp[3], &dAcol = ctx->tmp[4], &dAval = ctx->tmp[5],
           &dMisc = ctx->tmp[6], &dAsum = ctx->tmp[7], &dActive = ctx->tmp[8], &dPairs = ctx->tmp[9], &dPairOf = ctx->tmp[10];
    const bool has_a = K > 0 && A_colptr[K] > 0;
    const bool a_empty = K == 0;
    int64_t ldc = 4;
    HostCSR csr;
    bool trace_i8_done = false;
    if (has_a) {
        RET(upload_centered(ctx, dC, C, K, T, c_order, dCc, dCm, &ldc));
        if (P->dig_valid && !outl && T <= 24576 && ctx->opt("win_i8", 1) != 0 && ctx->opt("gram_incremental", 1) != 0 && !(P->base_valid && P->base_kstride > 1)) {
            const int64_t T16 = P->dig_T16;
            RET(ctx->tdig.ensure((size_t)K * T16 * 4 * sizeof(uint4)));
            RET(ctx->tscale.ensure((size_t)K * sizeof(double)));
            RET(ctx->gk.ensure((size_t)K * K * sizeof(double)));
            LAUNCH(ctx, "bg_trace_dig", k_trace_dig, dim3(K), dim3(256), 0, dCc.as<float>(), ldc, (int64_t)T, T16, ctx->tdig.as<uint4>(), ctx->tscale.as<double>());
            const int ntk = ((int)K + 15) >> 4;
            LAUNCH(ctx, "bg_trace_gram", k_trace_gram, dim3((unsigned)(ntk * (ntk + 1) / 2)), dim3(64 * TG_W), 0, dCc.as<float>(), ldc, (int64_t)T, (int)K, ctx->gk.as<double>());
            trace_i8_done = true;
        }
    }
    auto upload_csr = [&]() -> int {
        if (!has_a) return 0;
        csc_to_csr(P->d_b, K, A_colptr, A_rowidx, A_val, csr);
        RET(to_dev(ctx, dArow, csr.rowptr.data(), csr.rowptr.size()));
        RET(to_dev(ctx, dAcol, csr.col.data(), csr.col.size()));
        RET(to_dev(ctx, dAval, csr.val.data(), csr.val.size()));
        return 0;
    };
    ht.mark("traces");
    if (b0_only & 1) {
        RET(upload_csr());
        BgGeom g0{};
        g0.nr = P->nr; g0.nc = P->nc; g0.nr_b = P->nr_b; g0.nc_b = P->nc_b; g0.roff = P->roff; g0.coff = P->coff; g0.d = P->d; g0.d_b = P->d_b;
        LAUNCH(ctx, "bg_b0", k_b0, dim3((unsigned)((P->d + 255) / 256)), dim3(256), 0, P->ymean_d.as<double>(), g0,
               has_a ? dArow.as<int>() : nullptr, dAcol.as<int>(), dAval.as<float>(), dCm.as<double>(), P->b0.as<double>());
        P->ysig_valid = false;
        return 0;
    }
    bool first_run = false;
    int pmax = 0;
    RET(ring_stats_get(ctx, P, &pmax, &first_run));
    RET(dMisc.ensure(64));
    ht.mark("first_run + pmax");
    int kstride = 1;
    if (with_projection) {
        int64_t nk = std::min<int64_t>(T, (int64_t)pmax * 100);
        if (nk < 1) nk = 1;
        kstride = (int)(T / nk);
        if (kstride < 1) kstride = 1;
    }
    if (outl) kstride = 1;
    BgGeom g;
    g.nr = P->nr; g.nc = P->nc; g.nr_b = P->nr_b; g.nc_b = P->nc_b; g.roff = P->roff; g.coff = P->coff;
    g.r0_abs = P->brect[0]; g.c0_abs = P->brect[2]; g.d1 = P->d1; g.d2 = P->d2;
    g.nbr = (P->nr_b + BLK - 1) / BLK; g.nbc = (P->nc_b + BLK - 1) / BLK;
    g.d = P->d; g.d_b = P->d_b; g.T = T; g.kstride = kstride;
    g.Tp = (T + kstride - 1) / kstride;
    g.nbr = (P->nr_b + BLK - 1) / BLK; g.nbc = (P->nc_b + BLK - 1) / BLK;
    g.p_radius = 0;
    for (int i = 0; i < P->p; ++i) g.p_radius = std::max(g.p_radius, std::max(std::abs(P->dr[i]), std::abs(P->dc[i])));
    g.nbw = ((2 * g.p_radius) >> 4) + 2;
    g.p = p;
    const int maxd = (2 * g.p_radius + 15) >> 4, nrel = nrel_of(maxd);
    if (maxd > 3 || g.nbw > 4) return fail(CNMFE_EUNSUPPORTED, "fit_ring_model: ring offsets up to %d pixels (the block-pair table covers <= 24)", g.p_radius);
    bool incr = !outl && ctx->opt("gram_incremental", 1) != 0 && K < 32768;
    std::vector<int> lst_ptr, lst_k, blk_nt[4];
    std::vector<short> slot_of;
    static thread_local std::vector<int> nbox;
    if (incr) {
        const int nblk_ = g.nbr * g.nbc;
        static thread_local std::vector<int> own, seen, cnt, pairs_b, pairs_k, mark;
        own.assign(nblk_, -1); seen.assign(nblk_, -1); cnt.assign(nblk_ + 1, 0);
        pairs_b.clear(); pairs_k.clear();
        nbox.assign((size_t)4 * std::max(1, K), 0);
        for (int k = 0; k < K && has_a; ++k) {
            mark.clear();
            int bx[4] = {1 << 30, -1, 1 << 30, -1};
            for (int64_t e = A_colptr[k]; e < A_colptr[k + 1];) {
                const int q0 = A_rowidx[e], cb = q0 / P->nr_b, col_end = (cb + 1) * P->nr_b;
                int qlast = q0;
                ++e;
                while (e < A_colptr[k + 1] && A_rowidx[e] < col_end && A_rowidx[e] >= qlast) { qlast = A_rowidx[e]; ++e; }
                bx[0] = std::min(bx[0], q0 - cb * P->nr_b); bx[1] = std::max(bx[1], qlast - cb * P->nr_b); bx[2] = std::min(bx[2], cb); bx[3] = std::max(bx[3], cb);
                for (int bi = (q0 - cb * P->nr_b) >> 4; bi <= (qlast - cb * P->nr_b) >> 4; ++bi) {
                    const int b_ = (cb >> 4) * g.nbr + bi;
                    if (own[b_] != k) { own[b_] = k; mark.push_back(b_); }
                }
            }
            for (int i = 0; i < 4; ++i) nbox[(size_t)4 * k + i] = bx[i];
            for (int b_ : mark)
                for (int dj = -maxd; dj <= maxd; ++dj)
                    for (int di = -maxd; di <= maxd; ++di) {
                        const int i2 = b_ % g.nbr + di, j2 = b_ / g.nbr + dj;
                        if (i2 < 0 || i2 >= g.nbr || j2 < 0 || j2 >= g.nbc) continue;
                        const int nb_ = j2 * g.nbr + i2;
                        if (seen[nb_] != k) { seen[nb_] = k; pairs_b.push_back(nb_); pairs_k.push_back(k); ++cnt[nb_ + 1]; }
                    }
        }
        lst_ptr.assign(nblk_ + 1, 0);
        for (int b_ = 0; b_ < nblk_; ++b_) {
            if (cnt[b_ + 1] > WIN_NLB) { incr = false; break; }
            lst_ptr[b_ + 1] = lst_ptr[b_] + cnt[b_ + 1];
        }
        if (incr) {
            lst_k.resize(pairs_k.size());
            slot_of.assign((size_t)nblk_ * std::max(1, K), (short)-1);
            std::vector<int> &fill = cnt;
            for (int b_ = 0; b_ < nblk_; ++b_) fill[b_] = 0;
            for (size_t i = 0; i < pairs_k.size(); ++i) {
                const int b_ = pairs_b[i], k = pairs_k[i], s_ = fill[b_]++;
                lst_k[lst_ptr[b_] + s_] = k; slot_of[(size_t)b_ * K + k] = (short)s_;
            }
            for (int b_ = 0; b_ < nblk_; ++b_) { const int n = lst_ptr[b_ + 1] - lst_ptr[b_]; if (n) blk_nt[(n - 1) >> 4].push_back(b_); }
        }
    }
    if (incr && P->base_valid && P->base_kstride != kstride) {
        P->cov_base.swap(P->cov_base_alt); P->rowsum_base.swap(P->rowsum_base_alt);
        std::swap(P->base_valid, P->base_alt_valid); std::swap(P->base_kstride, P->base_alt_kstride);
        P->sys.swap(P->sys_alt); std::swap(P->sys_valid, P->sys_alt_valid);
        P->kinv_valid = false; P->kinv_lam_valid = false; P->kinv_fits = 0;
    }
    const bool build_base = incr && !(P->base_valid && P->base_kstride == kstride);
    if (build_base) { P->sys_valid = false; P->kinv_valid = false; P->kinv_lam_valid = false; P->kinv_fits = 0; }
    ht.mark("footprint block lists");
    g.bf4 = 1;
    const bool use_i8 = (build_base || !incr) && !outl && ctx->opt("gram_i8", 1) != 0 && g.Tp <= 24576;
    if (use_i8) g.bf4 = 3;
    g.Tpad = g.bf4 == 3 ? (g.Tp + 4 * GK - 1) / (4 * GK) * (4 * GK) : (g.Tp + GK - 1) / GK * GK;
    const int nblk = g.nbr * g.nbc;

    const bool keep_pt = incr && has_a && kstride == 1 && !P->derived && !(b0_only & 2) && ctx->opt("r1_virtual", 1) != 0;
    DevBuf &dLp = keep_pt ? P->pt_lp : ctx->inc[0], &dLk = ctx->inc[1], &dSlot = keep_pt ? P->pt_slot : ctx->inc[2], &dBl = ctx->inc[3], &dUt = ctx->inc[4], &dCsum = ctx->inc[5], &dGb = ctx->inc[6];
    if (keep_pt) P->pt_valid = false;
    std::vector<int> blall;
    int nsg = 1; int64_t ut_stride = 0, gb_stride = 0;
    bool proj_queued = false;
    bool stage_ok = false;
    bool win_i8 = false;
    auto queue_projection = [&]() -> int {
        for (int t = 3; t >= 0; --t) blall.insert(blall.end(), blk_nt[t].begin(), blk_nt[t].end());
        RET(to_dev(ctx, dLp, lst_ptr.data(), lst_ptr.size()));
        RET(to_dev(ctx, dLk, lst_k.data(), lst_k.size()));
        RET(to_dev(ctx, dBl, blall.data(), blall.size()));
        RET(dCsum.ensure((size_t)K * sizeof(double)));
        LAUNCH(ctx, "bg_trace_subsum", k_trace_subsum, dim3(K), dim3(256), 0, dCc.as<float>(), ldc, g.Tp, g.kstride, dCsum.as<double>());
        const int nb_ = (int)blall.size();
        nsg = nb_ >= 512 ? std::max(1, std::min(8, (2048 + nb_ - 1) / nb_)) : std::max(1, std::min(16, (4096 + nb_ - 1) / std::max(1, nb_)));
        ut_stride = (int64_t)std::max<size_t>(1, lst_k.size()) * BLKPX; gb_stride = (int64_t)nblk * WIN_NLB * WIN_NLB;
        RET(dUt.ensure((size_t)nsg * ut_stride * sizeof(double)));
        RET(dGb.ensure((size_t)nsg * gb_stride * sizeof(double)));
        if (P->dig_valid && g.kstride == 1 && g.Tp <= 24576 && ctx->opt("win_i8", 1) != 0 && K > 0) {
            const int64_t T16 = P->dig_T16;
            if (!trace_i8_done) {
                RET(ctx->tdig.ensure((size_t)K * T16 * 4 * sizeof(uint4)));
                RET(ctx->tscale.ensure((size_t)K * sizeof(double)));
                RET(ctx->gk.ensure((size_t)K * K * sizeof(double)));
                LAUNCH(ctx, "bg_trace_dig", k_trace_dig, dim3(K), dim3(256), 0, dCc.as<float>(), ldc, (int64_t)T, T16, ctx->tdig.as<uint4>(), ctx->tscale.as<double>());
                const int ntk = ((int)K + 15) >> 4;
                LAUNCH(ctx, "bg_trace_gram", k_trace_gram, dim3((unsigned)(ntk * (ntk + 1) / 2)), dim3(64 * TG_W), 0, dCc.as<float>(), ldc, (int64_t)T, (int)K, ctx->gk.as<double>());
            }
            std::vector<int> items;
            for (int b_ : blall) {
                const int ntl = (lst_ptr[b_ + 1] - lst_ptr[b_] + 15) >> 4;
                for (int gq = 0; gq < (ntl + 1) / 2; ++gq) items.push_back(b_ | (gq << 24));
            }
            RET(to_dev(ctx, ctx->win_items, items.data(), items.size()));
            if (!items.empty())
                if (win_planes3(ctx, T16)) { LAUNCH(ctx, "bg_win_proj", k_win_proj_i8<1>, dim3((unsigned)(items.size() * nsg)), dim3(512), 0, P->dig.as<uint4>(), T16, P->dig_sc.as<double>(), ctx->tdig.as<uint4>(),
                       ctx->tscale.as<double>(), dLp.as<int>(), dLk.as<int>(), ctx->win_items.as<int>(), nsg, dUt.as<double>(), ut_stride); } else { LAUNCH(ctx, "bg_win_proj", k_win_proj_i8<0>, dim3((unsigned)(items.size() * nsg)), dim3(512), 0, P->dig.as<uint4>(), T16, P->dig_sc.as<double>(), ctx->tdig.as<uint4>(),
                       ctx->tscale.as<double>(), dLp.as<int>(), dLk.as<int>(), ctx->win_items.as<int>(), nsg, dUt.as<double>(), ut_stride); }
            win_i8 = true;
        } else if (g.kstride == 1 || g.kstride == 2 || g.kstride == 4) {
            const int nbig = (int)blk_nt[3].size();
            if (nbig)
                LAUNCH(ctx, "bg_win_proj", k_win_proj4<true>, dim3((unsigned)(nbig * nsg)), dim3(256), 0, P->Yc4.as<float4>(), g, dCc.as<float>(), ldc, dLp.as<int>(), dLk.as<int>(),
                       dBl.as<int>(), nsg, dUt.as<double>(), ut_stride, dGb.as<double>(), gb_stride);
            if (nb_ > nbig)
                LAUNCH(ctx, "bg_win_proj", k_win_proj4<false>, dim3((unsigned)((nb_ - nbig) * nsg)), dim3(256), 0, P->Yc4.as<float4>(), g, dCc.as<float>(), ldc, dLp.as<int>(),
                       dLk.as<int>(), dBl.as<int>() + nbig, nsg, dUt.as<double>(), ut_stride, dGb.as<double>(), gb_stride);
        } else
        LAUNCH(ctx, "bg_win_proj", k_win_proj, dim3((unsigned)(nb_ * nsg)), dim3(256), 0, P->Yc4.as<float4>(), g, dCc.as<float>(), ldc, dLp.as<int>(), dLk.as<int>(),
               dBl.as<int>(), nsg, dUt.as<double>(), ut_stride, dGb.as<double>(), gb_stride);
        proj_queued = true;
        return 0;
    };
    if (incr && has_a && !build_base) RET(queue_projection());
    ht.mark("projection queued");
    RET(upload_csr());
    ht.mark("A csr");

    RET(dActive.ensure(P->d));
    int64_t nactive = P->d;
    if (first_run) {
        CK(hipMemsetAsync(dActive.p, 1, P->d, ctx->st()));
    } else {
        std::vector<float> asum(P->d_b, 0.f);
        if (a_empty || (b0_only & 2)) std::fill(asum.begin(), asum.end(), 1.0f);
        else if (has_a) for (int64_t q = 0; q < P->d_b; ++q) { double s = 0; for (int64_t e = csr.rowptr[q]; e < csr.rowptr[q + 1]; ++e) s += csr.val[e]; asum[q] = (float)s; }
        RET(to_dev(ctx, dAsum, asum.data(), asum.size()));
        CK(hipMemsetAsync(dMisc.p, 0, 64, ctx->st()));
        LAUNCH(ctx, "bg_active", k_active, dim3((unsigned)((P->d + 255) / 256)), dim3(256), 0, P->W.as<float>(), g,
               P->ring_dr.as<int>(), P->ring_dc.as<int>(), dAsum.as<float>(), dActive.as<unsigned char>(), dMisc.as<int>());
        CK(hipMemcpyAsync((char *)P->stat_host + 8, dMisc.p, sizeof(int), hipMemcpyDeviceToHost, ctx->st()));
        nactive = -1;
    }
    LAUNCH(ctx, "bg_b0", k_b0, dim3((unsigned)((P->d + 255) / 256)), dim3(256), 0, P->ymean_d.as<double>(), g,
           has_a ? dArow.as<int>() : nullptr, dAcol.as<int>(), dAval.as<float>(), dCm.as<double>(), P->b0.as<double>());

    ht.mark("ind_active + b0");
    {
        std::vector<char> touched(nblk, 0);
        {
            const int pi0 = std::max(0, P->roff - g.p_radius) / BLK, pi1 = std::min(P->nr_b - 1, P->roff + P->nr - 1 + g.p_radius) / BLK;
            const int pj0 = std::max(0, P->coff - g.p_radius) / BLK, pj1 = std::min(P->nc_b - 1, P->coff + P->nc - 1 + g.p_radius) / BLK;
            for (int j = pj0; j <= pj1; ++j)
                for (int i = pi0; i <= pi1; ++i) touched[j * g.nbr + i] = 1;
        }
        std::vector<int4> pairs; std::vector<int> pair_of((size_t)nblk * nrel, -1);
        for (int j = 0; j < g.nbc; ++j)
            for (int i = 0; i < g.nbr; ++i) {
                if (!touched[j * g.nbr + i]) continue;
                for (int dC = 0; dC <= maxd; ++dC)
                    for (int dR = (dC == 0 ? 0 : -maxd); dR <= maxd; ++dR) {
                        int i2 = i + dR, j2 = j + dC;
                        if (i2 < 0 || i2 >= g.nbr || j2 >= g.nbc || !touched[j2 * g.nbr + i2]) continue;
                        const int rel = rel_index(dR, dC, maxd);
                        pair_of[(size_t)(j * g.nbr + i) * nrel + rel] = (int)pairs.size();
                        pairs.push_back(make_int4(j * g.nbr + i, j2 * g.nbr + i2, rel, 0));
                    }
            }
        const int npairs = (int)pairs.size();
        const int DB = 2 * g.p_radius, DM = 2 * DB + 1;
        std::vector<char> Dm((size_t)DM * DM, 0);
        auto dset = [&](int dr, int dc) { if (dr >= -DB && dr <= DB && dc >= -DB && dc <= DB) Dm[(size_t)(dr + DB) * DM + dc + DB] = 1; };
        for (int a = 0; a < p; ++a) {
            dset(P->dr[a], P->dc[a]); dset(-P->dr[a], -P->dc[a]);
            for (int b = 0; b < p; ++b) dset(P->dr[b] - P->dr[a], P->dc[b] - P->dc[a]);
        }
        std::vector<int> rel_dR(nrel), rel_dC(nrel);
        for (int dC = 0; dC <= maxd; ++dC)
            for (int dR = (dC == 0 ? 0 : -maxd); dR <= maxd; ++dR) { rel_dR[rel_index(dR, dC, maxd)] = dR; rel_dC[rel_index(dR, dC, maxd)] = dC; }
        std::vector<unsigned short> needmask((size_t)nrel * 16, 0);
        for (int rel = 0; rel < nrel; ++rel) {
            const int dC = rel_dC[rel], dR = rel_dR[rel];
            for (int pi = 0; pi < 16; ++pi)
                for (int pj = 0; pj < 16; ++pj) {
                    if (rel == 0 && pi > pj) continue;
                    const int ri = (pi & 3) * 4, ci = (pi >> 2) * 4, rj = (pj & 3) * 4 + dR * 16, cj = (pj >> 2) * 4 + dC * 16;
                    bool nd = false;
                    for (int x = -3; x <= 3 && !nd; ++x)
                        for (int y = -3; y <= 3; ++y) {
                            const int ddr = rj - ri + x, ddc = cj - ci + y;
                            if (ddr >= -DB && ddr <= DB && ddc >= -DB && ddc <= DB && Dm[(size_t)(ddr + DB) * DM + ddc + DB]) { nd = true; break; }
                        }
                    if (nd) needmask[rel * 16 + pi] |= (unsigned short)(1u << pj);
                }
        }
        std::vector<int> work;
        for (int pp = 0; pp < npairs; ++pp)
            for (int q = 0; q < 4; ++q) {
                const int ih = q & 1, jh = q >> 1;
                bool any = false;
                for (int pi = ih * 8; pi < ih * 8 + 8; ++pi) if ((needmask[pairs[pp].z * 16 + pi] >> (jh * 8)) & 0xff) any = true;
                if (any) work.push_back(pp * 4 + q);
            }
        const int nwork = (int)work.size();
    ht.mark("pair / need / work tables");
        DevBuf &dWork = ctx->tmp[11], &dNeed = ctx->tmp[7];
        RET(to_dev(ctx, dPairs, pairs.data(), pairs.size()));
        RET(to_dev(ctx, dPairOf, pair_of.data(), pair_of.size()));
        RET(to_dev(ctx, dWork, work.data(), work.size()));
        RET(to_dev(ctx, dNeed, needmask.data(), needmask.size()));
        RET(ctx->cov.ensure((size_t)npairs * BLKPX * BLKPX * sizeof(double)));
        if (ctx->opt("debug", 0)) CK(hipMemsetAsync(ctx->cov.p, 0xff, (size_t)npairs * BLKPX * BLKPX * sizeof(double), ctx->st()));
        int nwg = (nwork + 7) / 8 * 8;
        DevBuf &dTcnt = ctx->tmp[12], &dTl = ctx->tmp[13];
        {
            std::vector<int> tcnt((size_t)nrel * 4, 0);
            std::vector<int> tlist((size_t)nrel * 4 * 64, 0);
            for (int rel = 0; rel < nrel; ++rel)
                for (int q = 0; q < 4; ++q) {
                    const int ih = q & 1, jh = q >> 1;
                    int n = 0;
                    for (int i = 0; i < 8; ++i) for (int j = 0; j < 8; ++j)
                        if ((needmask[rel * 16 + ih * 8 + i] >> (jh * 8 + j)) & 1) tlist[(size_t)(rel * 4 + q) * 64 + n++] = i | (j << 4);
                    tcnt[rel * 4 + q] = n;
                }
            RET(to_dev(ctx, dTcnt, tcnt.data(), tcnt.size()));
            RET(to_dev(ctx, dTl, tlist.data(), tlist.size()));
        }
        ht.mark("tile lists + uploads (sync)");
        DevBuf &covT = incr ? P->cov_base : ctx->cov, &rsT = incr ? P->rowsum_base : ctx->rowsum;
        const bool has_a_bf = has_a && !incr;
        if (incr) {
            RET(P->cov_base.ensure((size_t)npairs * BLKPX * BLKPX * sizeof(double)));
            if (build_base && ctx->opt("debug", 0)) CK(hipMemsetAsync(P->cov_base.p, 0xff, (size_t)npairs * BLKPX * BLKPX * sizeof(double), ctx->st()));
        }
        if (!incr || build_base) {
        RET(ctx->bf.ensure((size_t)nblk * g.Tpad * BLKPX * sizeof(float)));
        const int tchunk = (int)((std::max<int64_t>(64, (g.Tpad + 15) / 16) + 7) & ~int64_t(7));
        dim3 gb(nblk, (unsigned)((g.Tpad + tchunk - 1) / tchunk));
        RET(rsT.ensure((size_t)nblk * BLKPX * sizeof(double)));
        uint4 *digp = nullptr; double *digs = nullptr;
        if (use_i8) {
            const size_t dbytes = (size_t)nblk * g.Tpad * BLKPX * sizeof(float);
            bool resident = incr && kstride == 1 && !P->derived && ctx->opt("win_i8", 1) != 0;
            if (resident && P->dig.cap < dbytes) {
                size_t fr = 0, tot = 0;
                CK(hipMemGetInfo(&fr, &tot));
                if (fr < dbytes + ((size_t)8 << 30)) resident = false;
            }
            if (resident) {
                RET(P->dig.ensure(dbytes)); RET(P->dig_sc.ensure((size_t)nblk * BLKPX * sizeof(double)));
                digp = P->dig.as<uint4>(); digs = P->dig_sc.as<double>();
                P->dig_T16 = g.Tpad >> 4; P->dig_valid = true; P->digp_valid = false;
            } else {
                RET(ctx->dig_scale.ensure((size_t)nblk * BLKPX * sizeof(double)));
                digp = ctx->bf.as<uint4>(); digs = ctx->dig_scale.as<double>();
            }
            RET(ctx->dig_smax.ensure((size_t)nblk * BLKPX * sizeof(unsigned)));
            CK(hipMemsetAsync(ctx->dig_smax.p, 0, (size_t)nblk * BLKPX * sizeof(unsigned), ctx->st()));
            DigA da{has_a_bf ? dArow.as<int>() : nullptr, dAcol.as<int>(), dAval.as<float>(), dCc.as<float>(), ldc};
            const int tchunk16 = (int)((std::max<int64_t>(64, (g.Tpad + 15) / 16) + 15) & ~int64_t(15));
            const dim3 gd(nblk, (unsigned)((g.Tpad + tchunk16 - 1) / tchunk16));
            LAUNCH(ctx, "bg_dig_scale", k_dig_scale, gd, dim3(256), 0, P->Yc4.as<float4>(), P->Tc, g, da, tchunk16, ctx->dig_smax.as<unsigned>());
            RET(ctx->dig_rspart.ensure((size_t)gd.y * nblk * BLKPX * sizeof(double)));
            LAUNCH(ctx, "bg_build_dig", k_build_dig, gd, dim3(256), 0, P->Yc4.as<float4>(), P->Tc, g, da, ctx->dig_smax.as<unsigned>(), digs, digp, tchunk16, ctx->dig_rspart.as<double>());
            LAUNCH(ctx, "bg_rs_reduce", k_rs_reduce, dim3((unsigned)nblk), dim3(256), 0, ctx->dig_rspart.as<double>(), (int)gd.y, (int64_t)nblk * BLKPX, rsT.as<double>());
            if (incr && kstride > 1 && !resident && !P->derived && !has_a_bf && T <= (int64_t)I8_SEG_FRAMES * 16 && ctx->opt("win_i8", 1) != 0) {
                BgGeom g1 = g; g1.kstride = 1; g1.Tp = T; g1.Tpad = (T + 4 * GK - 1) / (4 * GK) * (4 * GK);
                const size_t d1bytes = (size_t)nblk * g1.Tpad * BLKPX * sizeof(float);
                bool ok = true;
                if (P->dig.cap < d1bytes) { size_t fr = 0, tot = 0; CK(hipMemGetInfo(&fr, &tot)); if (fr < d1bytes + ((size_t)8 << 30)) ok = false; }
                if (ok) {
                    RET(P->dig.ensure(d1bytes)); RET(P->dig_sc.ensure((size_t)nblk * BLKPX * sizeof(double)));
                    CK(hipMemsetAsync(ctx->dig_smax.p, 0, (size_t)nblk * BLKPX * sizeof(unsigned), ctx->st()));
                    const int tch1 = (int)((std::max<int64_t>(64, (g1.Tpad + 15) / 16) + 15) & ~int64_t(15));
                    const dim3 gd1(nblk, (unsigned)((g1.Tpad + tch1 - 1) / tch1));
                    DigA dv{nullptr, nullptr, nullptr, nullptr, 0};
                    LAUNCH(ctx, "bg_dig_scale", k_dig_scale, gd1, dim3(256), 0, P->Yc4.as<float4>(), P->Tc, g1, dv, tch1, ctx->dig_smax.as<unsigned>());
                    LAUNCH(ctx, "bg_build_dig", k_build_dig, gd1, dim3(256), 0, P->Yc4.as<float4>(), P->Tc, g1, dv, ctx->dig_smax.as<unsigned>(), P->dig_sc.as<double>(), P->dig.as<uint4>(), tch1,
                           (double *)nullptr);
                    P->dig_T16 = g1.Tpad >> 4; P->dig_valid = true; P->digp_valid = false;
                }
            }
        } else
        LAUNCH(ctx, "bg_build_bf", k_build_bf, gb, dim3(256), 0, P->Yc4.as<float4>(), P->Tc, g,
               has_a_bf ? dArow.as<int>() : nullptr, dAcol.as<int>(), dAval.as<float>(), dCc.as<float>(), ldc, ctx->bf.as<float>(), tchunk, rsT.as<double>());
        if (outl) {
            const size_t bfbytes = (size_t)nblk * g.Tpad * BLKPX * sizeof(float);
            RET(ctx->bf2.ensure(bfbytes));
            RET(ctx->outl_cnt.ensure((size_t)T * sizeof(int)));
            CK(hipMemcpyAsync(ctx->bf2.p, ctx->bf.p, bfbytes, hipMemcpyDeviceToDevice, ctx->st()));
            CK(hipMemsetAsync(ctx->outl_cnt.p, 0, (size_t)T * sizeof(int), ctx->st()));
            LAUNCH(ctx, "bg_outlier_clip", k_outlier_clip, dim3((unsigned)((P->d + 255) / 256), (unsigned)(g.Tpad >> 2)), dim3(256), 0, ctx->bf.as<float4>(),
                   ctx->bf2.as<float4>(), g, P->ring_dr.as<int>(), P->ring_dc.as<int>(), P->W.as<float>(), P->sn_b.as<float>(), thresh_outlier,
                   ctx->outl_cnt.as<int>());
            std::vector<int> sel;
            const int64_t nmax = (int64_t)pmax * 100;
            if (nmax < T) {
                std::vector<int> cnt((size_t)T);
                CK(hipMemcpyAsync(cnt.data(), ctx->outl_cnt.p, (size_t)T * sizeof(int), hipMemcpyDeviceToHost, ctx->st()));
                CK(hipStreamSynchronize(ctx->st()));
                const double qv = matlab_quantile(cnt, (double)nmax / (double)T);
                for (int64_t t = 0; t < T; ++t) if ((double)cnt[t] <= qv) sel.push_back((int)t);
            } else for (int64_t t = 0; t < T; ++t) sel.push_back((int)t);
            const int64_t Tpad_src = g.Tpad;
            g.Tp = (int64_t)sel.size();
            g.Tpad = (g.Tp + GK - 1) / GK * GK;
            RET(to_dev(ctx, ctx->outl_sel, sel.data(), sel.size()));
            LAUNCH(ctx, "bg_select_frames", k_select_frames, dim3(nblk, (unsigned)std::min<int64_t>(64, std::max<int64_t>(1, g.Tpad >> 2))), dim3(256), 0,
                   ctx->bf2.as<float>(), Tpad_src, ctx->bf.as<float>(), g.Tpad, ctx->outl_sel.as<int>(), g.Tp);
            CK(hipStreamSynchronize(ctx->st()));
        }
        if (g.bf4 < 2)
            LAUNCH(ctx, "bg_rowsum", k_rowsum, dim3(nblk), dim3(256), 0, ctx->bf.as<float>(), g.Tpad, rsT.as<double>(), g.bf4);

        {
            const size_t shmem = (size_t)G4_NBUF * G4_STAGE_F * sizeof(float);
            static bool attr4 = false;
            if (!attr4) {
                CK(hipFuncSetAttribute((const void *)k_gram4, hipFuncAttributeMaxDynamicSharedMemorySize, (int)shmem));
                attr4 = true;
            }
            if (use_i8) {
                static bool attr8 = false;
                if (!attr8) { CK(hipFuncSetAttribute((const void *)k_gram_i8, hipFuncAttributeMaxDynamicSharedMemorySize, GI_NBUF * GI_STAGE_B)); attr8 = true; }
                LAUNCH(ctx, "bg_gram_i8", k_gram_i8, dim3(nwg), dim3(512), (size_t)GI_NBUF * GI_STAGE_B, digp, g.Tpad >> 4, dPairs.as<int4>(), dWork.as<int>(), nwork,
                       dTcnt.as<int>(), dTl.as<int>(), digs, covT.as<double>());
            } else
                LAUNCH(ctx, "bg_gram_f64", k_gram4, dim3(nwg), dim3(256), shmem, ctx->bf.as<float>(), g.Tpad, dPairs.as<int4>(), dWork.as<int>(), nwork,
                       dTcnt.as<int>(), dTl.as<int>(), 0, covT.as<double>());
        }
        if (incr) { P->base_valid = true; P->base_kstride = kstride; }
        }
        const int nt = (p + 15) / 16;
        if (nt < 1 || nt > 8) return fail(CNMFE_EUNSUPPORTED, "fit_ring_model: %d ring neighbours (<= %d supported)", p, PMAX_RING);
        DevBuf &dFill = ctx->solve_fill;
        const double fillv[2] = {0.0, 1.0};
        RET(to_dev(ctx, dFill, fillv, 2));
        CovTab tab; tab.cov = ctx->cov.as<double>(); tab.pair_of = dPairOf.as<int>(); tab.nbr = g.nbr; tab.nbc = g.nbc; tab.maxd = maxd; tab.nrel = nrel;
        DevBuf &dWcodes = ctx->wcodes;
        const int woff = (g.p_radius + 15) >> 4;
        const int nwin = (g.nbr + 2 * woff) * (g.nbc + 2 * woff);
        bool packed = incr && ctx->opt("solve_packed", 1) != 0 && (int64_t)nblk * std::max(1, K) < (int64_t)1 << 31 &&
                      (int64_t)lst_k.size() * BLKPX < (int64_t)1 << 31;
        const size_t sys_bytes = (size_t)P->d * ((size_t)(nt * (nt + 1) / 2) * 256 + 16 * nt) * sizeof(double);
        if (packed && !(P->sys_valid && P->sys.cap >= sys_bytes)) {
            if (P->sys.cap < sys_bytes) {
                size_t fr = 0, tot = 0;
                CK(hipMemGetInfo(&fr, &tot));
                if (fr < sys_bytes + ((size_t)8 << 30)) packed = false;
            }
            if (packed) {
                RET(P->sys.ensure(sys_bytes));
                RET(dWcodes.ensure((size_t)nwin * 256 * sizeof(int)));
                LAUNCH(ctx, "bg_win_codes", k_win_codes, dim3((unsigned)nwin), dim3(256), 0, dPairOf.as<int>(), g.nbr, g.nbc, woff, maxd, nrel, dWcodes.as<int>());
                CovTab tb = tab; tb.cov = P->cov_base.as<double>(); tb.wcodes = dWcodes.as<int>(); tb.woff = woff;
                int *dErrP = nullptr;
                RET(ctx_errflag(ctx, &dErrP));
#define RSP_CASE(NT_) case NT_: LAUNCH(ctx, "bg_sys_pack", (k_sys_pack<NT_>), dim3((unsigned)P->d), dim3(64), 0, tb, g, P->ring_dr.as<int>(), P->ring_dc.as<int>(), \
                                        P->rowsum_base.as<double>(), (const unsigned char *)nullptr, (float *)nullptr, dErrP, 0, (const int *)nullptr, dFill.as<double>(), P->sys.as<double>()); break;
                switch (nt) { RSP_CASE(1) RSP_CASE(2) RSP_CASE(3) RSP_CASE(4) RSP_CASE(5) RSP_CASE(6) RSP_CASE(7) RSP_CASE(8) default: break; }
#undef RSP_CASE
                P->sys_valid = true; P->kinv_valid = false; P->kinv_lam_valid = false; P->kinv_fits = 0;
            }
        }
        if (incr) {
            RET(ctx->rowsum.ensure((size_t)nblk * BLKPX * sizeof(double)));
            if (has_a) {
                if (!proj_queued) RET(queue_projection());
                RET(to_dev(ctx, dSlot, slot_of.data(), slot_of.size()));
                if (keep_pt) RET(P->pt_tab.ensure(std::max<size_t>(1, lst_k.size()) * BLKPX * sizeof(double)));
                LAUNCH(ctx, "bg_win_fix", k_win_fix, dim3((unsigned)blall.size(), WIN_NLB / WF_S), dim3(256), 0, g, (int)K, dArow.as<int>(), dAcol.as<int>(), dAval.as<float>(), dLp.as<int>(),
                       dSlot.as<short>(), dBl.as<int>(), nsg, dUt.as<double>(), ut_stride, dGb.as<double>(), gb_stride, keep_pt ? P->pt_tab.as<double>() : nullptr,
                       win_i8 ? ctx->gk.as<double>() : (const double *)nullptr, dLk.as<int>());
                if (keep_pt) {
                    P->pt_K = K; P->pt_lp_h = lst_ptr; P->pt_slot_h = slot_of;
                    P->pt_gen = bound_rows_of(ctx, C, c_order, K, P->pt_rows) ? ctx->bound_gen : -1;
                    P->pt_valid = true;
                }
                const int csplit = npairs >= 8192 ? 1 : npairs >= 4096 ? 2 : 4;
// ... 151 lines not shown
```

### cnmf_e_amd/csrc/common.hpp

```cpp
#pragma once
#include <hip/hip_runtime.h>
#include <stdint.h>
#include <stdio.h>
#include <stdarg.h>
#include <string.h>
#include <string>
#include <vector>
#include <cstring>
#include <chrono>
#include <cmath>
#include <map>
#include <algorithm>
#include "../../include/cnmfe.h"

namespace cnmfe {

typedef unsigned nt_u32x4_t __attribute__((ext_vector_type(4)));
__device__ __forceinline__ uint4 ld_stream(const uint4 *p) {
    const nt_u32x4_t v = __builtin_nontemporal_load(reinterpret_cast<const nt_u32x4_t *>(p));
    return make_uint4(v.x, v.y, v.z, v.w);
}


extern thread_local char g_err[1024];
// ... 70 lines not shown
    if (pon_) (ctx)->prof.begin(name, lst_, pr_); \
    const auto lt1_ = ltr_ ? std::chrono::steady_clock::now() : std::chrono::steady_clock::time_point(); \
    hipLaunchKernelGGL(kern, grid, block, shmem, lst_, __VA_ARGS__); \
    if (ltr_) { const auto lt2_ = std::chrono::steady_clock::now(); const double la_ = std::chrono::duration<double, std::milli>(lt1_ - lt0_).count(), lb_ = std::chrono::duration<double, std::milli>(lt2_ - lt1_).count(); \
        if (la_ + lb_ > 2.0) fprintf(stderr, "[host_trace] launch %s: flush of held-back uploads %.2f ms, launch call %.2f ms\n", name, la_, lb_); } \
    if (pon_) (ctx)->prof.end(lst_, pr_); \
    hipError_t le_ = hipGetLastError(); \
    if (le_ != hipSuccess) return cnmfe::fail(CNMFE_EHIP, "launch %s failed: %s", name, hipGetErrorString(le_)); \
} while (0)

constexpr int PMAX_RING = 128;
constexpr int BLK = 16;
constexpr int BLKPX = BLK * BLK;

struct HostCSR { std::vector<int32_t> rowptr;    std::vector<int32_t> col; std::vector<float> val; std::vector<int32_t> src; };
inline void csc_to_csr(int64_t nrow, int32_t ncol, const int64_t *colptr, const int32_t *rowidx, const float *val, HostCSR &out) {
    int64_t nnz = colptr[ncol];
    out.rowptr.assign(nrow + 1, 0); out.col.resize(nnz); out.val.resize(nnz); out.src.resize(nnz);
    for (int64_t e = 0; e < nnz; ++e) out.rowptr[rowidx[e] + 1]++;
    for (int64_t r = 0; r < nrow; ++r) out.rowptr[r + 1] += out.rowptr[r];
    std::vector<int32_t> cur(out.rowptr.begin(), out.rowptr.end() - 1);
    for (int32_t k = 0; k < ncol; ++k)
        for (int64_t e = colptr[k]; e < colptr[k + 1]; ++e) {
            int32_t pos = cur[rowidx[e]]++; out.col[pos] = k; out.val[pos] = val ? val[e] : 1.0f; out.src[pos] = (int32_t)e;
        }
}

struct Patch {
    int32_t prect[4], brect[4];
    int32_t d1 = 0, d2 = 0;
    int32_t nr = 0, nc = 0, nr_b = 0, nc_b = 0;
    int32_t roff = 0, coff = 0;
    int64_t T = 0, d = 0, d_b = 0;
    DevBuf Y;
    DevBuf Yc4;
    int64_t Tc = 0;
    DevBuf ymean_d;
    DevBuf ymean_f;
    bool ymean_valid = false;
    int64_t frames_uploaded = 0;
    std::vector<uint8_t> frame_seen;
    int32_t radius = 0, p = 0;
    std::vector<int32_t> dr, dc;
    DevBuf ring_dr, ring_dc;
    DevBuf W;
    DevBuf b0;
    bool ring_ready = false;
    DevBuf sn_b;
    bool sn_ready = false;
    DevBuf ysig;
    bool ysig_valid = false;
    bool ysig_virtual = false;
    DevBuf pt_tab, pt_lp, pt_slot;
    bool pt_valid = false; int32_t pt_K = 0; int64_t pt_gen = -1;
    std::vector<int32_t> pt_rows; std::vector<int> pt_lp_h; std::vector<short> pt_slot_h;
    bool res_ac = false; int res_kind = 0; int64_t res_ldc = 0;
    DevBuf resCnt, resK, resV, resCc, resCm;
    bool pend = false, pend_ac = false; int64_t pend_ldc = 0; int32_t pend_K = 0, res_K = 0;
    DevBuf pendCnt, pendK, pendV, pendCc, pendCm;
    DevBuf cov_base, rowsum_base;
    bool base_valid = false, derived = false;
    int base_kstride = 0;
    DevBuf cov_base_alt, rowsum_base_alt; bool base_alt_valid = false; int base_alt_kstride = 0;
    DevBuf sys, sys_alt; bool sys_valid = false, sys_alt_valid = false;
    DevBuf kinv, kinv_lam, kinv_list; bool kinv_valid = false, kinv_lam_valid = false; int kinv_fits = 0;
    DevBuf dig, dig_sc; int64_t dig_T16 = 0; bool dig_valid = false;
    DevBuf yt4; bool yt4_valid = false;
    DevBuf digp; bool digp_valid = false;
    int ss_res = -1, ss_ssub = 0, ss_Pr = 0, ss_Pc = 0, ss_d1s = 0, ss_d2s = 0;
    bool ss_taps = false;
    std::vector<int> ss_tr_idx, ss_tc_idx, ss_rlo, ss_rhi, ss_clo, ss_chi, ss_trp_h, ss_tri_h, ss_tcp_h, ss_tci_h;
    std::vector<float> ss_tr_w, ss_tc_w;
    DevBuf ss_ir, ss_wr, ss_ic, ss_wc, ss_trp, ss_tri, ss_trw, ss_tcp, ss_tci, ss_tcw, ss_dlt;
    DevBuf stat_dev; void *stat_host = nullptr; hipEvent_t stat_ev = nullptr; bool stat_valid = false;
    int lane = 0;
    ~Patch() { if (stat_host) (void)hipHostFree(stat_host); if (stat_ev) (void)hipEventDestroy(stat_ev); }
};

struct DeconvScratch { DevBuf pv, pw, pt, pl, tkp, tko, tkl, tkv, pnum, list, ybuf, obuf, tbuf;
    void swap(DeconvScratch &o) { DevBuf *a[] = {&pv, &pw, &pt, &pl, &tkp, &tko, &tkl, &tkv, &pnum, &list, &ybuf, &obuf, &tbuf}, *b[] = {&o.pv, &o.pw, &o.pt, &o.pl, &o.tkp, &o.tko, &o.tkl, &o.tkv, &o.pnum, &o.list, &o.ybuf, &o.obuf, &o.tbuf};
        for (int i = 0; i < 13; ++i) a[i]->swap(*b[i]); } };

struct TemporalJob {
    Patch *P = nullptr; int32_t K = 0; int64_t ldc = 0, T = 0; int maxIter = 0; bool deconv = false; cnmfe_deconv_opts dopts{};
    DevBuf dC, dColptr, dErow, dAval, dU, dCraw, dNk, dNidx, dNval, dNptr, dAa, dOvf, dS, dPars, dSn, dB;
    std::vector<std::vector<int>> levels;
    bool swept = false;
    bool dag = false;
    std::vector<int> diag; std::vector<char> upd; bool term_applied = false, finished = false; int nn = 0;
    float *pin = nullptr; size_t pin_cap = 0;
    ~TemporalJob() { if (pin) (void)hipHostFree(pin); }
};

}

namespace cnmfe {
struct PinArena {
    char *p = nullptr; size_t cap = 0, off = 0; int half = 0;
    hipEvent_t ev[2] = {nullptr, nullptr}; bool ev_set[2] = {false, false};
    int init(size_t bytes) {
        if (p) return 0;
        if (hipHostMalloc((void **)&p, bytes, hipHostMallocDefault) != hipSuccess) { p = nullptr; return -1; }
        cap = bytes;
        for (int i = 0; i < 2; ++i) if (hipEventCreateWithFlags(&ev[i], hipEventDisableTiming) != hipSuccess) return -1;
        return 0;
    }
    template <class F> void *take(size_t n, F &&stream_of) {
        n = (n + 255) & ~size_t(255);
        if (!p || n > cap / 2) return nullptr;
        const size_t end = (size_t)(half + 1) * (cap / 2);
        if (off + n > end) {
            (void)hipEventRecord(ev[half], stream_of()); ev_set[half] = true;
            half ^= 1; off = (size_t)half * (cap / 2);
            if (ev_set[half]) (void)hipEventSynchronize(ev[half]);
        }
        void *r = p + off; off += n; return r;
    }
    void swap(PinArena &o) { std::swap(p, o.p); std::swap(cap, o.cap); std::swap(off, o.off); std::swap(half, o.half); for (int i = 0; i < 2; ++i) { std::swap(ev[i], o.ev[i]); std::swap(ev_set[i], o.ev_set[i]); } }
    ~PinArena() { if (p) (void)hipHostFree(p); for (int i = 0; i < 2; ++i) if (ev[i]) (void)hipEventDestroy(ev[i]); }
};
}

namespace cnmfe {
constexpr int PIN_NSEG = 24;
constexpr int I8_SEG_FRAMES = 24576;
struct PinSegs { const uint4 *src[PIN_NSEG]; uint4 *dst[PIN_NSEG]; unsigned n16[PIN_NSEG]; };
}

struct cnmfe_lane {
    hipStream_t stream_ = nullptr; cnmfe::PinSegs pseg{}; int npseg = 0; cnmfe::PinArena pin; int64_t spatial_nnz = -1;
    cnmfe::DevBuf vp[32]; size_t hw_vp[32] = {}; int64_t last_ldc = 0;
    cnmfe::DevBuf ysig_low, up_tmp, bgs_r, bgs_b, bgs_upr, bgs_upc; int bgs_patch = -1, bgs_d1s = 0; int64_t bgs_dF = 0;
    cnmfe::DevBuf bf, dig_smax, dig_rspart, dig_scale, tdig, tscale, gk, win_items, bf2, outl_cnt, outl_sel, cov, rowsum, tmp[16];
    size_t hw_cc = 0, hw_cm = 0, hw_wa[3] = {0, 0, 0};
    cnmfe::DevBuf inc[7], stg[4], wcodes, solve_fill, stage, scr[24]; cnmfe::DeconvScratch dscr;
    hipEvent_t ev = nullptr; int64_t fork_seen = 0; bool dirty = false;
    ~cnmfe_lane() { if (stream_) (void)hipStreamDestroy(stream_); if (ev) (void)hipEventDestroy(ev); }
};

struct cnmfe_ctx {
    int device = 0;
    hipStream_t stream_ = nullptr;
    cnmfe::PinSegs pseg; int npseg = 0;
    void flush_copies();
    hipStream_t st() { if (npseg) flush_copies(); return stream_; }
    cnmfe::PinArena pin;
    int64_t spatial_nnz = -1;
    hipStream_t copy_stream = nullptr;
    hipEvent_t ev_bound_ready = nullptr, ev_copy_done = nullptr; bool copy_pending = false;
    int64_t copy_gen = 0; std::vector<std::pair<int64_t, hipEvent_t>> copy_gens; std::vector<hipEvent_t> copy_ev_pool;
    int copy_batch_mark();
    std::vector<hipEvent_t> tickets; std::vector<char> ticket_busy;
    int *ticket_flags = nullptr;
    cnmfe::DevBuf ticket_dev;
    static constexpr size_t TICKET_FLAGS = 1024;
    cnmfe::Profiler prof;
    std::map<int, cnmfe::Patch *> patches;
    cnmfe::DevBuf bound;
    int32_t bound_K = 0; int64_t bound_T = 0; int bound_order = 1; bool bound_valid = false;
    int64_t bound_gen = 0;
    cnmfe::DevBuf vp[32];
    size_t hw_vp[32] = {};
    int64_t last_ldc = 0;
    cnmfe::DevBuf ysig_low;
    cnmfe::DevBuf up_tmp;
    cnmfe::DevBuf bgs_r, bgs_b, bgs_upr, bgs_upc;
    int bgs_patch = -1, bgs_d1s = 0; int64_t bgs_dF = 0;
    cnmfe::DevBuf bf;
    cnmfe::DevBuf dig_smax;
    cnmfe::DevBuf dig_rspart;
    cnmfe::DevBuf dig_scale;
    cnmfe::DevBuf tdig, tscale, gk, win_items;
    cnmfe::DevBuf bf2, outl_cnt, outl_sel;
    cnmfe::DevBuf cov;
    cnmfe::DevBuf rowsum;
    cnmfe::DevBuf tmp[16];
    size_t hw_cc = 0, hw_cm = 0, hw_wa[3] = {0, 0, 0};
    cnmfe::DevBuf inc[7];
    cnmfe::DevBuf stg[4];
    cnmfe::DevBuf wcodes, solve_fill;
    cnmfe::DevBuf stage;
    cnmfe::DevBuf scr[24];
    cnmfe::DeconvScratch dscr;
    cnmfe::DevBuf last_craw, last_aa;
    std::vector<cnmfe::TemporalJob *> tjobs; int tjobs_used = 0;
    cnmfe::DevBuf dcv_c, dcv_s, dcv_pars, dcv_sn;
    int32_t last_t_K = 0; int64_t last_t_ldc = 0, last_t_T = 0; bool last_t_valid = false;
    cnmfe::DevBuf stitch;
    int32_t stitch_K = 0; int64_t stitch_T = 0, stitch_ld = 0; bool stitch_open = false;
    void *rccl_comm = nullptr; int rccl_rank = 0, rccl_n = 0;
    cnmfe::DevBuf errflag;
    std::map<std::string, int64_t> opts;
    int trace_level = 0;
    int64_t opt(const char *n, int64_t dflt) const { auto it = opts.find(n); return it == opts.end() ? dflt : it->second; }
    std::vector<cnmfe_lane *> lanes; int cur_lane = 0, patches_created = 0, spatial_lane = 0;
    hipEvent_t ev_fork = nullptr; int64_t fork_gen = 0;
    void swap_lane(cnmfe_lane &L);
    int activate(int lane);
    int join_lanes();
    int fork_mark();
    ~cnmfe_ctx();
};

namespace cnmfe {
struct HostTrace {
    bool on; const char *name; std::chrono::steady_clock::time_point t0, last;
    HostTrace(cnmfe_ctx *ctx, const char *n) : on(ctx->opt("host_trace", 0) != 0), name(n) { if (on) t0 = last = std::chrono::steady_clock::now(); }
    void mark(const char *what) {
        if (!on) return;
        const auto t = std::chrono::steady_clock::now();
        fprintf(stderr, "[host_trace] %s: %-28s %8.3f ms (at %8.3f)\n", name, what, std::chrono::duration<double, std::milli>(t - last).count(),
                std::chrono::duration<double, std::milli>(t - t0).count());
        last = t;
    }
};
inline Patch *get_patch(cnmfe_ctx *ctx, int id) {
    auto it = ctx->patches.find(id);
    if (it == ctx->patches.end()) return nullptr;
    if (!ctx->lanes.empty() && ctx->activate(it->second->lane) != 0) return nullptr;
    return it->second;
}
struct GlobalScope {
    cnmfe_ctx *ctx; int rc = 0;
    explicit GlobalScope(cnmfe_ctx *c) : ctx(c) { if (ctx && !ctx->lanes.empty()) rc = ctx->join_lanes(); }
    ~GlobalScope() { if (ctx && !ctx->lanes.empty()) (void)ctx->fork_mark(); }
};
int pinned_to_dev(cnmfe_ctx *ctx, void *dst, const void *src_pinned, size_t bytes);
void pin_register(cnmfe_ctx *ctx, bool live);
template <class T> inline int to_dev(cnmfe_ctx *ctx, DevBuf &b, const T *h, size_t n) {
    RET(b.ensure(std::max<size_t>(n, 1) * sizeof(T)));
    if (!n) return 0;
    if (void *st = ctx->pin.take(n * sizeof(T), [ctx] { return ctx->st(); })) {
        memcpy(st, h, n * sizeof(T));
        return pinned_to_dev(ctx, b.p, st, n * sizeof(T));
    }
    CK(hipMemcpyAsync(b.p, h, n * sizeof(T), hipMemcpyHostToDevice, ctx->st()));
    CK(hipStreamSynchronize(ctx->st()));
    return 0;
}
int upload_traces(cnmfe_ctx *ctx, DevBuf &dst, const float *C, int32_t K, int64_t T, int order, int64_t *ldc);
int download_traces(cnmfe_ctx *ctx, const float *dC, int64_t ldc, float *C, int32_t K, int64_t T, int order);

int bg_fit_ring(cnmfe_ctx *ctx, Patch *P, int32_t K, const int64_t *A_colptr, const int32_t *A_rowidx, const float *A_val,
                const float *C, int c_order, int with_projection, float *b0_out, int64_t info[4], int b0_only = 0, double thresh_outlier = NAN);
int tu_warm_resid(); int tu_warm_bg();
int win_i8_table(cnmfe_ctx *ctx, Patch *P, const char *name_dig, const char *name_proj, int K, const float *dCc, int64_t ldc, const std::vector<int> &lst_ptr, const std::vector<int> &blall,
                 const int *dLp, const int *dLk, int nsg, double *dUt, int64_t ut_stride);
int tu_warm_factor(); int tu_warm_deconv(); int tu_warm_ssub(); int tu_warm_vproj();
int bg_reserve(cnmfe_ctx *ctx, Patch *P);
int residual_run(cnmfe_ctx *ctx, Patch *P, int pid, int32_t Ksel, const int64_t *A_colptr, const int32_t *A_rowidx,
                 const float *A_val, const float *C, int c_order, float *Ysig_out, int out_memspace, DevBuf *outbuf = nullptr, int tables_only = 0);
int ysig_export(cnmfe_ctx *ctx, Patch *P, DevBuf &ysig, float *Ysig_out, int out_memspace);
int rss_run(cnmfe_ctx *ctx, Patch *P, int32_t K, const int64_t *A_colptr, const int32_t *A_rowidx, const float *A_val, const float *C, int c_order,
            const float *b0_block, const float *b0_new, double *rss_out);
int bg_reconstruct_run(cnmfe_ctx *ctx, Patch *P, const float *b0_block, const float *b0_new, int64_t frame0, int64_t nframes, float *out, int out_memspace);
int residual_materialize(cnmfe_ctx *ctx, Patch *P);
int residual_realize(cnmfe_ctx *ctx, Patch *P);
bool bound_rows_of(const cnmfe_ctx *ctx, const float *C, int c_order, int32_t K, std::vector<int32_t> &rows);
int vproj_spatial(cnmfe_ctx *ctx, Patch *P, int32_t K, const float *C, int c_order, const int64_t *IND_colptr, const int32_t *IND_rowidx,
                  const int *dErow, const int *dEcol, const float *dCc, int64_t ldc, float *dU, double *dQ = nullptr);
int vproj_temporal(cnmfe_ctx *ctx, Patch *P, int32_t K, const int64_t *A_colptr, const int32_t *A_rowidx, const float *A_val,
                   const int64_t *dColptr, const int *dErow, const float *dAval, float *dU, int64_t ldu);
int vproj_spatial_ssub(cnmfe_ctx *ctx, Patch *M, int32_t K, const float *C, int c_order, const int64_t *IND_colptr, const int32_t *IND_rowidx,
                       const int *dErow, const int *dEcol, const float *dCc, int64_t ldc, float *dU);
int vproj_temporal_ssub(cnmfe_ctx *ctx, Patch *M, int32_t K, const int64_t *A_colptr, const int32_t *A_rowidx, const float *A_val,
                        const int64_t *dColptr, const int *dErow, const float *dAval, float *dU, int64_t ldu);
int ssub_taps(cnmfe_ctx *ctx, Patch *M, const Patch *R);
int ssub_realize(cnmfe_ctx *ctx, Patch *M);
int residual_term_project(cnmfe_ctx *ctx, Patch *P, int32_t K, const int64_t *dColptr, const int *dErow, const float *dAval, float *dU, int64_t ldu, int *dOverflow);
bool residual_term_foldable_spatial(const Patch *P, int32_t K, int64_t ldc);
int residual_term_fold_spatial(cnmfe_ctx *ctx, Patch *P, int32_t K, int64_t nnz, const int *dErow, const int *dEcol, const float *dCc, int64_t ldc, float *dU, DevBuf &dG);
int check_csc_pub(const char *what, int32_t ncol, int64_t nrow, const int64_t *colptr, const int32_t *rowidx);
int spatial_run(cnmfe_ctx *ctx, Patch *P, int algorithm, int32_t K, const int64_t *A_colptr, const int32_t *A_rowidx,
                const float *A_val, const float *C, int c_order, const int64_t *IND_colptr, const int32_t *IND_rowidx,
                const float *sn, int32_t param, float *A_out);
int temporal_run(cnmfe_ctx *ctx, Patch *P, int32_t K, const int64_t *A_colptr, const int32_t *A_rowidx, const float *A_val,
                 const float *C_in, int c_order, int32_t maxIter, float *C_out, float *C_raw_out, float *aa_out,
                 const cnmfe_deconv_opts *dopts, float *kernel_pars, float *S_out, float *sn_out, TemporalJob *job = nullptr);
int temporal_sweep_jobs(cnmfe_ctx *ctx);
#ifdef __HIPCC__
__device__ __forceinline__ void glds16(const void *base, unsigned voff, unsigned lds_dst) {
    unsigned keep;
    asm volatile("s_mov_b32 %0, m0\n\ts_mov_b32 m0, %3\n\ts_nop 0\n\tglobal_load_lds_dwordx4 %1, %2\n\ts_mov_b32 m0, %0"
                 : "=&s"(keep) : "v"(voff), "s"(base), "s"(lds_dst) : "memory");
}
#endif

int sn_pixels_run(cnmfe_ctx *ctx, Patch *P, float *sn_out);
int fast_temporal_run(cnmfe_ctx *ctx, Patch *P, int32_t K, const int64_t *A_colptr, const int32_t *A_rowidx, const float *A_val,
                      int c_order, float *C_raw_out, float *aa_out);
int deconv_bound_run(cnmfe_ctx *ctx, const cnmfe_deconv_opts *opts, float *C_out, float *C_raw_out, float *S_out, float *pars_out, float *sn_out);
int deconv_all_run(cnmfe_ctx *ctx, int32_t K, int64_t T, float *C_raw, int c_order, const cnmfe_deconv_opts *opts,
                   float *C_out, float *S_out, float *pars_out, float *sn_out);
int postproc_run(cnmfe_ctx *ctx, int32_t d1, int32_t d2, int32_t K, const int64_t *A_colptr, const int32_t *A_rowidx,
                 const float *A_val, uint8_t *keep);
int ensure_ymean(cnmfe_ctx *ctx, Patch *P);
int sn_video_run(cnmfe_ctx *ctx, Patch *P, int64_t nframes, float *sn_out);
int spatial_fetch(cnmfe_ctx *ctx, float *A_out, int64_t nnz);
int spatial_fetch_connected(cnmfe_ctx *ctx, int32_t d1, int32_t d2, int32_t K, const int64_t *IND_colptr, const int32_t *IND_rowidx, float *A_out, uint8_t *keep, bool wait = true);
int ring_first_run(cnmfe_ctx *ctx, Patch *P, bool *first);
int ring_stats_enqueue(cnmfe_ctx *ctx, Patch *P);
int ring_stats_get(cnmfe_ctx *ctx, Patch *P, int *pmax, bool *first);
int center_traces(cnmfe_ctx *ctx, const float *C, int64_t ldc, int32_t K, int64_t T, DevBuf &Cc, DevBuf &Cmean);
int upload_centered(cnmfe_ctx *ctx, DevBuf &stage, const float *C, int32_t K, int64_t T, int order, DevBuf &Cc, DevBuf &Cmean, int64_t *ldc_out);
int ctx_errflag(cnmfe_ctx *ctx, int **dflag);
int ctx_check_errflag(cnmfe_ctx *ctx);
}
```

### cnmf_e_amd/csrc/factor.hip

```cpp
#include "common.hpp"
#include <math.h>

namespace cnmfe {

__global__ void __launch_bounds__(256) k_proj_spatial(const float4 *__restrict__ ysig4, int64_t d, int64_t T, const int *__restrict__ erow,
                                                      const int *__restrict__ ecol, int64_t nnz, const float *__restrict__ Cc, int64_t ldc,
                                                      int64_t tchunk, float *__restrict__ part) {
    const int64_t e = (int64_t)blockIdx.x * blockDim.x + threadIdx.x;
    if (e >= nnz) return;
    const int64_t t0 = (int64_t)blockIdx.y * tchunk, t1 = t0 + tchunk < T ? t0 + tchunk : T;
    const float4 *y = ysig4 + erow[e];
    const float *c = Cc + (int64_t)ecol[e] * ldc;
    float a0 = 0.f, a1 = 0.f, a2 = 0.f, a3 = 0.f;
    for (int64_t t = t0; t < t1; t += 4) {
        const float4 yv = y[(t >> 2) * d];
        const float4 cv = *reinterpret_cast<const float4 *>(c + t);
        a0 = fmaf(yv.x, cv.x, a0); a1 = fmaf(yv.y, cv.y, a1); a2 = fmaf(yv.z, cv.z, a2); a3 = fmaf(yv.w, cv.w, a3);
    }
    part[(int64_t)blockIdx.y * nnz + e] = (a0 + a1) + (a2 + a3);
}
__global__ void k_reduce_parts(const float *__restrict__ part, int64_t n, int nparts, float *__restrict__ out) {
    const int64_t e = (int64_t)blockIdx.x * blockDim.x + threadIdx.x;
    if (e >= n) return;
    double s = 0;
// ... 458 lines not shown
    ht.mark("u erow");
    RET(to_dev(ctx, dEcol, ecol.data(), (size_t)nnz));
    ht.mark("u ecol");
    RET(to_dev(ctx, dRptr, rptr.data(), rptr.size()));
    ht.mark("u rptr");
    RET(to_dev(ctx, dRcol, csr.col.data(), csr.col.size()));
    RET(to_dev(ctx, dRsrc, csr.src.data(), csr.src.size()));
    ht.mark("u rcol rsrc");
    RET(to_dev(ctx, dAval, aval.data(), aval.size()));
    ht.mark("u aval");
    if (sn) RET(to_dev(ctx, dSn, sn, (size_t)d));
    ht.mark("uploads");
    const int nparts = (int)std::max<int64_t>(1, std::min<int64_t>(32, T / 256));
    const int64_t tchunk = ((T + nparts - 1) / nparts + 3) & ~int64_t(3);
    RET(dPart.ensure((size_t)nparts * nnz * sizeof(float)));
    RET(dU.ensure((size_t)nnz * sizeof(float)));
    ht.mark("buffers");
    bool virt = P->ysig_virtual;
    if (virt) {
        const int rcv = P->res_kind == 2 ? vproj_spatial_ssub(ctx, P, K, C, c_order, IND_colptr, IND_rowidx, dErow.as<int>(), dEcol.as<int>(), dCc.as<float>(), ldc, dU.as<float>())
                                         : vproj_spatial(ctx, P, K, C, c_order, IND_colptr, IND_rowidx, dErow.as<int>(), dEcol.as<int>(), dCc.as<float>(), ldc, dU.as<float>());
        if (rcv < 0) return rcv;
        if (rcv > 0) { RET(residual_realize(ctx, P)); virt = false; }
    }
    if (!virt) {
    LAUNCH(ctx, "spatial_proj_U", k_proj_spatial, dim3((unsigned)((nnz + 255) / 256), nparts), dim3(256), 0, P->ysig.as<float4>(), d, T,
           dErow.as<int>(), dEcol.as<int>(), nnz, dCc.as<float>(), ldc, tchunk, dPart.as<float>());
    LAUNCH(ctx, "reduce_parts", k_reduce_parts, dim3((unsigned)((nnz + 255) / 256)), dim3(256), 0, dPart.as<float>(), nnz, nparts, dU.as<float>());
    }
    ht.mark("projection");
    RET(residual_term_fold_spatial(ctx, P, K, nnz, dErow.as<int>(), dEcol.as<int>(), dCc.as<float>(), ldc, dU.as<float>(), S_[20]));
    ht.mark("footprint term");
    std::vector<char> include(K, 1);
    PairGraph g; build_graph(K, csr, d, include, g);
    ht.mark("graph");
    RET(to_dev(ctx, dPairs, g.pairs.data(), g.pairs.size()));
    RET(dV.ensure((size_t)K * K * sizeof(float)));
    CK(hipMemsetAsync(dV.p, 0, (size_t)K * K * sizeof(float), ctx->st()));
    LAUNCH(ctx, "spatial_pair_gram", k_pair_gram, dim3((unsigned)g.pairs.size()), dim3(256), 0, dCc.as<float>(), ldc, T, dPairs.as<int2>(), K, dV.as<float>());
    if (algorithm == CNMFE_SPATIAL_NNLS) {
        const int maxN = (int)param;
        std::vector<int> rows[3];
        for (int64_t m = 0; m < d; ++m) {
            const int n = std::min<int>(csr.rowptr[m + 1] - csr.rowptr[m], maxN);
            if (n > 0) rows[n <= 4 ? 0 : n <= 8 ? 1 : 2].push_back((int)m);
        }
        DevBuf &dRows = S_[19];
        std::vector<int> all; int off3[4] = {0, 0, 0, 0};
        for (int g_ = 0; g_ < 3; ++g_) { all.insert(all.end(), rows[g_].begin(), rows[g_].end()); off3[g_ + 1] = (int)all.size(); }
        RET(to_dev(ctx, dRows, all.data(), all.size()));
#define NNLS_GO(CAP, G) do { if (off3[G + 1] > off3[G]) { LAUNCH(ctx, "spatial_nnls", k_nnls_spatial<CAP>, dim3((unsigned)((off3[G + 1] - off3[G] + 63) / 64)), dim3(64), 0, \
                            dRows.as<int>() + off3[G], off3[G + 1] - off3[G], dRptr.as<int>(), dRcol.as<int>(), dRsrc.as<int>(), dU.as<float>(), dV.as<float>(), K, \
                            maxN, 1e-4, dAval.as<float>()); } } while (0)
        NNLS_GO(4, 0); NNLS_GO(8, 1);
        if (maxN <= 20) { NNLS_GO(20, 2); } else { NNLS_GO(32, 2); }
#undef NNLS_GO
    } else {
        std::vector<int> flat; std::vector<int> off;
        const bool dag_on = ctx->opt("sweep_dag", 1) != 0 && param > 1;
        if (dag_on) { std::vector<std::vector<int>> dag; dag_schedule(K, g, include, (int)param, false, dag); g.levels.swap(dag); }
        for (auto &l : g.levels) { off.push_back((int)flat.size()); flat.insert(flat.end(), l.begin(), l.end()); }
        RET(to_dev(ctx, dLvl, flat.data(), flat.size()));
        for (int it = 0; it < (dag_on ? 1 : param); ++it)
            for (size_t l = 0; l < g.levels.size(); ++l)
                LAUNCH(ctx, "spatial_hals_level", k_hals_spatial, dim3((unsigned)g.levels[l].size()), dim3(128), 0, dLvl.as<int>() + off[l],
                       dColptr.as<int64_t>(), dErow.as<int>(), dRptr.as<int>(), dRcol.as<int>(), dRsrc.as<int>(), dU.as<float>(), dV.as<float>(), K,
                       dSn.as<float>(), algorithm == CNMFE_SPATIAL_HALS_THRESH ? 1 : 0, dAval.as<float>());
    }
    ht.mark("sweep launches");
    ctx->spatial_nnz = nnz;
    if (!A_out) return 0;
    CK(hipMemcpyAsync(A_out, dAval.p, (size_t)nnz * sizeof(float), hipMemcpyDeviceToHost, ctx->st()));
    return ctx_check_errflag(ctx);
}

int spatial_fetch(cnmfe_ctx *ctx, float *A_out, int64_t nnz) {
    if (ctx->spatial_nnz < 0 || nnz != ctx->spatial_nnz) return fail(CNMFE_ESTATE, "no deferred spatial update of %lld values (last one: %lld)", (long long)nnz, (long long)ctx->spatial_nnz);
    if (nnz) CK(hipMemcpyAsync(A_out, ctx->scr[6].p, (size_t)nnz * sizeof(float), hipMemcpyDeviceToHost, ctx->st()));
    return ctx_check_errflag(ctx);
}

struct DeconvCfg; struct DeconvIO; struct DeconvScratch;
int temporal_deconv_sweeps(cnmfe_ctx *ctx, const cnmfe_deconv_opts *dopts, int64_t T, int K, int maxIter, const std::vector<std::vector<int>> &levels,
                           const int *dLvl, const std::vector<int> &off, float *dC, float *dCraw, float *dS, int64_t ldc, const float *dU,
                           const int *dNptr, const int *dNidx, const float *dNval, const float *dAa, float *dPars, float *dSn);

__global__ void k_scale_rows(float *__restrict__ U, int64_t ldc, int64_t T, const float *__restrict__ inv) {
    const int k = blockIdx.y;
    const int64_t t = (int64_t)blockIdx.x * blockDim.x + threadIdx.x;
    if (t < T) U[(int64_t)k * ldc + t] *= inv[k];
}

int fast_temporal_run(cnmfe_ctx *ctx, Patch *P, int32_t K, const int64_t *A_colptr, const int32_t *A_rowidx, const float *A_val,
                      int c_order, float *C_raw_out, float *aa_out) {
    const int64_t T = P->T, d = P->d, nnz = A_colptr[K];
    if (nnz >= (int64_t(1) << 31)) return fail(CNMFE_EUNSUPPORTED, "nnz(A) too large");
    std::vector<float> av((size_t)std::max<int64_t>(1, nnz)), inv(K), aa(K);
    for (int k = 0; k < K; ++k) {
        double mx = 0.0;
        bool any = false;
        for (int64_t e = A_colptr[k]; e < A_colptr[k + 1]; ++e) { if (!any || A_val[e] > mx) mx = A_val[e]; any = true; }
        if (any && A_colptr[k + 1] - A_colptr[k] < d && mx < 0.0) mx = 0.0;
        double s = 0.0;
        for (int64_t e = A_colptr[k]; e < A_colptr[k + 1]; ++e) {
            const double a = A_val[e];
            const bool keep = (a * (1.0 / mx)) >= 0.5;
            av[e] = keep ? (float)a : 0.f;
            if (keep) s += a * a;
        }
        aa[k] = (float)s; inv[k] = s > 0.0 ? (float)(1.0 / s) : 0.f;
    }
    DevBuf *S_ = ctx->scr;
    DevBuf &dColptr = S_[0], &dErow = S_[1], &dAval = S_[6], &dU = ctx->last_craw, &dInv = S_[13];
    const int64_t ldc = (T + 3) & ~int64_t(3);
    RET(to_dev(ctx, dColptr, A_colptr, (size_t)K + 1));
    RET(to_dev(ctx, dErow, A_rowidx, (size_t)nnz));
    RET(to_dev(ctx, dAval, av.data(), (size_t)nnz));
    RET(to_dev(ctx, dInv, inv.data(), (size_t)K));
    RET(dU.ensure((size_t)K * ldc * sizeof(float)));
    CK(hipMemsetAsync(dU.p, 0, (size_t)K * ldc * sizeof(float), ctx->st()));
    const int64_t Tc = (T + 3) / 4;
    const int nchunk = (int)std::max<int64_t>(1, std::min<int64_t>(64, Tc / 32));
    const int64_t tchunk = (Tc + nchunk - 1) / nchunk;
    if (nnz > 0)
        LAUNCH(ctx, "temporal_proj_U", k_proj_temporal, dim3(K, nchunk), dim3(256), 0, P->ysig.as<float4>(), d, T, dColptr.as<int64_t>(),
               dErow.as<int>(), dAval.as<float>(), tchunk, dU.as<float>(), ldc);
    LAUNCH(ctx, "temporal_scale_rows", k_scale_rows, dim3((unsigned)((T + 255) / 256), (unsigned)K), dim3(256), 0, dU.as<float>(), ldc, T, dInv.as<float>());
    RET(to_dev(ctx, ctx->last_aa, aa.data(), (size_t)K));
    ctx->last_t_K = K; ctx->last_t_ldc = ldc; ctx->last_t_T = T; ctx->last_t_valid = true;
    RET(download_traces(ctx, dU.as<float>(), ldc, C_raw_out, K, T, c_order));
    if (aa_out) memcpy(aa_out, aa.data(), (size_t)K * sizeof(float));
    return 0;
}

int temporal_run(cnmfe_ctx *ctx, Patch *P, int32_t K, const int64_t *A_colptr, const int32_t *A_rowidx, const float *A_val,
                 const float *C_in, int c_order, int32_t maxIter, float *C_out, float *C_raw_out, float *aa_out,
                 const cnmfe_deconv_opts *dopts, float *kernel_pars, float *S_out, float *sn_out, TemporalJob *job) {
    const int64_t T = P->T, d = P->d, nnz = A_colptr[K];
    if (nnz >= (int64_t(1) << 31)) return fail(CNMFE_EUNSUPPORTED, "nnz(A) too large");
    DevBuf *S_ = ctx->scr;
    DevBuf &dC = job ? job->dC : ctx->tmp[0];
    DevBuf &dColptr = job ? job->dColptr : S_[0], &dErow = job ? job->dErow : S_[1], &dAval = job ? job->dAval : S_[6], &dU = job ? job->dU : S_[7],
           &dCraw = job ? job->dCraw : ctx->last_craw, &dNk = job ? job->dNk : S_[14], &dNidx = job ? job->dNidx : S_[15], &dNval = job ? job->dNval : S_[16],
           &dNptr = job ? job->dNptr : S_[17], &dAa = job ? job->dAa : ctx->last_aa, &dLvl = S_[12], &dOvf = job ? job->dOvf : S_[18];
    if (!job) ctx->last_t_valid = false;
    HostTrace ht(ctx, "temporal");
    int64_t ldc;
    RET(upload_traces(ctx, dC, C_in, K, T, c_order, &ldc));
    RET(to_dev(ctx, dColptr, A_colptr, (size_t)K + 1));
    RET(to_dev(ctx, dErow, A_rowidx, (size_t)nnz));
    RET(to_dev(ctx, dAval, A_val, (size_t)nnz));
    RET(dU.ensure((size_t)K * ldc * sizeof(float)));
    RET(dCraw.ensure((size_t)K * ldc * sizeof(float)));
    CK(hipMemsetAsync(dU.p, 0, (size_t)K * ldc * sizeof(float), ctx->st()));
    CK(hipMemsetAsync(dCraw.p, 0, (size_t)K * ldc * sizeof(float), ctx->st()));
    const int64_t Tc = (T + 3) / 4;
    const int nchunk = (int)std::max<int64_t>(1, std::min<int64_t>(64, Tc / 32));
    const int64_t tchunk = (Tc + nchunk - 1) / nchunk;
    bool term_applied = false;
    auto reproject = [&]() -> int {
        RET(residual_materialize(ctx, P));
        CK(hipMemsetAsync(dU.p, 0, (size_t)K * ldc * sizeof(float), ctx->st()));
        LAUNCH(ctx, "temporal_proj_U", k_proj_temporal, dim3(K, nchunk), dim3(256), 0, P->ysig.as<float4>(), d, T, dColptr.as<int64_t>(),
               dErow.as<int>(), dAval.as<float>(), tchunk, dU.as<float>(), ldc);
        return 0;
    };
    if (nnz > 0) {
        if (P->pend && (P->pend_ldc != ldc || (P->res_ac && P->res_ldc != ldc))) RET(residual_materialize(ctx, P));
        bool virt = P->ysig_virtual;
        if (virt) {
            const int rcv = P->res_kind == 2 ? vproj_temporal_ssub(ctx, P, K, A_colptr, A_rowidx, A_val, dColptr.as<int64_t>(), dErow.as<int>(), dAval.as<float>(), dU.as<float>(), ldc)
                                             : vproj_temporal(ctx, P, K, A_colptr, A_rowidx, A_val, dColptr.as<int64_t>(), dErow.as<int>(), dAval.as<float>(), dU.as<float>(), ldc);
            if (rcv < 0) return rcv;
            if (rcv > 0) { RET(residual_realize(ctx, P)); virt = false; }
        }
        if (!virt)
        LAUNCH(ctx, "temporal_proj_U", k_proj_temporal, dim3(K, nchunk), dim3(256), 0, P->ysig.as<float4>(), d, T, dColptr.as<int64_t>(),
               dErow.as<int>(), dAval.as<float>(), tchunk, dU.as<float>(), ldc);
        RET(dOvf.ensure(64));
        CK(hipMemsetAsync(dOvf.p, 0, 64, ctx->st()));
        const int rc_ = residual_term_project(ctx, P, K, dColptr.as<int64_t>(), dErow.as<int>(), dAval.as<float>(), dU.as<float>(), ldc, dOvf.as<int>());
        if (rc_ < 0) return rc_;
        if (rc_ > 0) RET(reproject());
        else term_applied = P->pend;
    }
    ht.mark("uploads + projection launch");
    HostCSR csr; csc_to_csr(d, K, A_colptr, A_rowidx, A_val, csr);
    std::vector<char> nonempty(K, 0);
    for (int k = 0; k < K; ++k) nonempty[k] = A_colptr[k + 1] > A_colptr[k];
    PairGraph g; build_graph(K, csr, d, nonempty, g);
    std::vector<std::vector<int>> nb(K);
    for (auto &p : g.pairs) { nb[p.x].push_back(p.y); if (p.x != p.y) nb[p.y].push_back(p.x); }
    std::vector<int> nptr(K + 1, 0), nk, nidx, diag(K, 0);
    for (int k = 0; k < K; ++k) {
        std::sort(nb[k].begin(), nb[k].end());
        nptr[k] = (int)nidx.size();
        for (int j : nb[k]) { if (j == k) diag[k] = (int)nidx.size(); nk.push_back(k); nidx.push_back(j); }
    }
    nptr[K] = (int)nidx.size();
    const int nn = (int)nidx.size();
    RET(to_dev(ctx, dNk, nk.data(), nk.size())); RET(to_dev(ctx, dNidx, nidx.data(), nidx.size())); RET(to_dev(ctx, dNptr, nptr.data(), nptr.size()));
    RET(dNval.ensure((size_t)std::max(1, nn) * sizeof(float)));
    LAUNCH(ctx, "temporal_ata_pairs", k_ata_pairs, dim3((nn + 3) / 4), dim3(256), 0, dColptr.as<int64_t>(), dErow.as<int>(), dAval.as<float>(),
           dNk.as<int>(), dNidx.as<int>(), nn, dNval.as<float>());
    std::vector<char> upd(K, 0);
    for (int k = 0; k < K; ++k)
        for (int64_t e = A_colptr[k]; e < A_colptr[k + 1] && !upd[k]; ++e) upd[k] = A_val[e] * A_val[e] > 0.f;
    if (upd != nonempty) build_graph(K, csr, d, upd, g);
    std::vector<int> flat, off;
    const bool dag_on = ctx->opt("sweep_dag", 1) != 0 && maxIter > 1;
    if (dag_on) { std::vector<std::vector<int>> dag; dag_schedule(K, g, upd, maxIter, dopts != nullptr, dag); g.levels.swap(dag); }
    for (auto &l : g.levels) { off.push_back((int)flat.size()); flat.insert(flat.end(), l.begin(), l.end()); }
    if (!job) RET(to_dev(ctx, dLvl, flat.data(), flat.size()));
    ht.mark("csr + graph + lists + levels");
    if (job) {
        const size_t need = ((size_t)nn + 1) * sizeof(float);
        if (need > job->pin_cap) {
            if (job->pin) (void)hipHostFree(job->pin);
            job->pin = nullptr; job->pin_cap = 0;
            CK(hipHostMalloc((void **)&job->pin, need * 2, hipHostMallocDefault));
            job->pin_cap = need * 2;
        }
        job->nn = nn; job->pin[nn] = 0.f;
        CK(hipMemcpyAsync(job->pin, dNval.p, (size_t)nn * sizeof(float), hipMemcpyDeviceToHost, ctx->st()));
        if (term_applied) CK(hipMemcpyAsync(job->pin + nn, dOvf.p, sizeof(int), hipMemcpyDeviceToHost, ctx->st()));
        job->P = P; job->K = K; job->ldc = ldc; job->T = T; job->maxIter = maxIter; job->deconv = dopts != nullptr; job->swept = false; job->finished = false;
        job->diag = std::move(diag); job->upd = std::move(upd); job->term_applied = term_applied;
        job->levels = std::move(g.levels); job->dag = dag_on;
        if (dopts) {
            job->dopts = *dopts;
            RET(job->dS.ensure((size_t)K * ldc * sizeof(float)));
            CK(hipMemsetAsync(job->dS.p, 0, (size_t)K * ldc * sizeof(float), ctx->st()));
            RET(to_dev(ctx, job->dPars, kernel_pars, (size_t)K));
            RET(job->dSn.ensure((size_t)K * sizeof(float)));
            CK(hipMemsetAsync(job->dSn.p, 0, (size_t)K * sizeof(float), ctx->st()));
            RET(job->dB.ensure((size_t)K * sizeof(float)));
        }
        ht.mark("job queued");
        return 0;
    }
    std::vector<float> nval(nn);
    int ovf = 0;
    CK(hipMemcpyAsync(nval.data(), dNval.p, (size_t)nn * sizeof(float), hipMemcpyDeviceToHost, ctx->st()));
    if (term_applied) CK(hipMemcpyAsync(&ovf, dOvf.p, sizeof(int), hipMemcpyDeviceToHost, ctx->st()));
    RET(ctx_check_errflag(ctx));
    ht.mark("wait for A'A (sync)");
    if (ovf) RET(reproject());
    std::vector<float> aa(K);
    for (int k = 0; k < K; ++k) {
        aa[k] = nval[diag[k]];
        if ((aa[k] > 0.f) != (upd[k] != 0)) return fail(CNMFE_EHIP, "temporal update: aa(%d) = %g disagrees with the host-side test of its column", k, (double)aa[k]);
    }
    RET(to_dev(ctx, dAa, aa.data(), aa.size()));
    ht.mark("level schedule");
    if (!dopts) {
        for (int it = 0; it < (dag_on ? 1 : maxIter); ++it)
            for (size_t l = 0; l < g.levels.size(); ++l)
                LAUNCH(ctx, "temporal_hals_level", k_hals_temporal, dim3((unsigned)g.levels[l].size()), dim3(T >= 2048 ? 1024 : 256), 0, dLvl.as<int>() + off[l], dNptr.as<int>(),
                       dNidx.as<int>(), dNval.as<float>(), dAa.as<float>(), dU.as<float>(), dC.as<float>(), dCraw.as<float>(), ldc, T);
    } else {
        DevBuf &dS = S_[19], &dPars = S_[21], &dSn = S_[22];
        RET(dS.ensure((size_t)K * ldc * sizeof(float)));
        CK(hipMemsetAsync(dS.p, 0, (size_t)K * ldc * sizeof(float), ctx->st()));
        RET(to_dev(ctx, dPars, kernel_pars, (size_t)K));
        RET(dSn.ensure((size_t)K * sizeof(float)));
        CK(hipMemsetAsync(dSn.p, 0, (size_t)K * sizeof(float), ctx->st()));
        RET(temporal_deconv_sweeps(ctx, dopts, T, K, dag_on ? -1 : maxIter, g.levels, dLvl.as<int>(), off, dC.as<float>(), dCraw.as<float>(), dS.as<float>(), ldc,
                                   dU.as<float>(), dNptr.as<int>(), dNidx.as<int>(), dNval.as<float>(), dAa.as<float>(), dPars.as<float>(), dSn.as<float>()));
        const bool want_back = C_out || C_raw_out || S_out || sn_out;
        RET(download_traces(ctx, dS.as<float>(), ldc, S_out, K, T, c_order));
        if (want_back) {
            CK(hipMemcpyAsync(kernel_pars, dPars.p, (size_t)K * sizeof(float), hipMemcpyDeviceToHost, ctx->st()));
            if (sn_out) CK(hipMemcpyAsync(sn_out, dSn.p, (size_t)K * sizeof(float), hipMemcpyDeviceToHost, ctx->st()));
            CK(hipStreamSynchronize(ctx->st()));
        }
    }
    ctx->last_t_K = K; ctx->last_t_ldc = ldc; ctx->last_t_T = T; ctx->last_t_valid = true;
    RET(download_traces(ctx, dC.as<float>(), ldc, C_out, K, T, c_order));
    RET(download_traces(ctx, dCraw.as<float>(), ldc, C_raw_out, K, T, c_order));
    if (aa_out) memcpy(aa_out, aa.data(), (size_t)K * sizeof(float));
    if (C_out || C_raw_out) CK(hipStreamSynchronize(ctx->st()));
    return 0;
}

struct DeconvJobDev;
int temporal_deconv_sweeps_jobs(cnmfe_ctx *ctx, const cnmfe_deconv_opts *dopts, int64_t T, int maxIter, const std::vector<TemporalJob *> &jobs,
                                const int2 *dList, const std::vector<int> &off, DevBuf &dTab);

int temporal_sweep_jobs(cnmfe_ctx *ctx) {
    std::vector<TemporalJob *> jobs;
    for (int i = 0; i < ctx->tjobs_used; ++i) if (!ctx->tjobs[i]->swept && ctx->tjobs[i]->K > 0) jobs.push_back(ctx->tjobs[i]);
    if (jobs.empty()) return 0;
    bool waiting = false;
    for (auto *j : jobs) waiting = waiting || !j->finished;
    if (waiting) RET(ctx_check_errflag(ctx));
    for (auto *j : jobs) {
        if (j->finished) continue;
        int ovf = 0;
        memcpy(&ovf, j->pin + j->nn, sizeof(int));
        if (j->term_applied && ovf) {
            Patch *P = j->P;
            const int64_t Tc = (j->T + 3) / 4;
            const int nchunk = (int)std::max<int64_t>(1, std::min<int64_t>(64, Tc / 32));
            const int64_t tchunk = (Tc + nchunk - 1) / nchunk;
            RET(residual_materialize(ctx, P));
            CK(hipMemsetAsync(j->dU.p, 0, (size_t)j->K * j->ldc * sizeof(float), ctx->st()));
            LAUNCH(ctx, "temporal_proj_U", k_proj_temporal, dim3(j->K, nchunk), dim3(256), 0, P->ysig.as<float4>(), P->d, j->T, j->dColptr.as<int64_t>(),
                   j->dErow.as<int>(), j->dAval.as<float>(), tchunk, j->dU.as<float>(), j->ldc);
        }
        std::vector<float> aa(j->K);
        for (int k = 0; k < j->K; ++k) {
            aa[k] = j->pin[j->diag[k]];
            if ((aa[k] > 0.f) != (j->upd[k] != 0)) return fail(CNMFE_EHIP, "temporal update: aa(%d) = %g disagrees with the host-side test of its column", k, (double)aa[k]);
        }
        RET(to_dev(ctx, j->dAa, aa.data(), aa.size()));
        j->finished = true;
    }
    const TemporalJob *j0 = jobs[0];
    size_t lmax = 0;
    for (auto *j : jobs) {
        if (j->T != j0->T || j->maxIter != j0->maxIter || j->deconv != j0->deconv || j->dag != j0->dag || (j->deconv && memcmp(&j->dopts, &j0->dopts, sizeof(j->dopts)) != 0))
            return fail(CNMFE_ESTATE, "the temporal jobs of one sweep must share T, maxIter and the deconvolution options");
        lmax = std::max(lmax, j->levels.size());
    }
    std::vector<int2> flat; std::vector<int> off;
    for (size_t l = 0; l < lmax; ++l) {
        off.push_back((int)flat.size());
        for (size_t ji = 0; ji < jobs.size(); ++ji)
            if (l < jobs[ji]->levels.size()) for (int k : jobs[ji]->levels[l]) flat.push_back(make_int2((int)ji, k));
    }
    off.push_back((int)flat.size());
    DevBuf &dList = ctx->scr[12], &dTab = ctx->scr[13];
    RET(to_dev(ctx, dList, flat.data(), flat.size()));
    HostTrace ht(ctx, "temporal sweep (jobs)");
    if (!j0->deconv) {
        std::vector<HJobDev> tab(jobs.size());
        for (size_t ji = 0; ji < jobs.size(); ++ji) {
            TemporalJob *j = jobs[ji];
            tab[ji] = HJobDev{(CNMFE_GPTR(const int))j->dNptr.as<int>(), (CNMFE_GPTR(const int))j->dNidx.as<int>(), (CNMFE_GPTR(const float))j->dNval.as<float>(),
                              (CNMFE_GPTR(const float))j->dAa.as<float>(), (CNMFE_GPTR(const float))j->dU.as<float>(), (CNMFE_GPTR(float))j->dC.as<float>(),
                              (CNMFE_GPTR(float))j->dCraw.as<float>(), j->ldc};
        }
        RET(to_dev(ctx, dTab, tab.data(), tab.size()));
        for (int it = 0; it < (j0->dag ? 1 : j0->maxIter); ++it)
            for (size_t l = 0; l < lmax; ++l) {
                const int n = off[l + 1] - off[l];
                if (n > 0)
                    LAUNCH(ctx, "temporal_hals_level", k_hals_temporal_jobs, dim3((unsigned)n), dim3(j0->T >= 2048 ? 1024 : 256), 0, dTab.as<HJobDev>(), dList.as<int2>() + off[l], j0->T);
            }
    } else {
        RET(temporal_deconv_sweeps_jobs(ctx, &j0->dopts, j0->T, j0->dag ? -1 : j0->maxIter, jobs, dList.as<int2>(), off, dTab));
    }
    for (auto *j : jobs) j->swept = true;
    ht.mark("launches");
    return 0;
}

static int postproc_boxes(int32_t d1, int32_t d2, int32_t K, const int64_t *A_colptr, const int32_t *A_rowidx, std::vector<int4> &box);

int spatial_fetch_connected(cnmfe_ctx *ctx, int32_t d1, int32_t d2, int32_t K, const int64_t *IND_colptr, const int32_t *IND_rowidx, float *A_out, uint8_t *keep, bool wait) {
    const int64_t nnz = IND_colptr[K];
    if (ctx->spatial_nnz < 0 || nnz != ctx->spatial_nnz) return fail(CNMFE_ESTATE, "no deferred spatial update of %lld values (last one: %lld)", (long long)nnz, (long long)ctx->spatial_nnz);
    if (nnz == 0) return 0;
    std::vector<int4> box;
    RET(postproc_boxes(d1, d2, K, IND_colptr, IND_rowidx, box));
    DevBuf *S_ = ctx->scr;
    DevBuf &dColptr = S_[0], &dErow = S_[1], &dAval = S_[6], &dBox = S_[13], &dKeep = S_[14];
    RET(to_dev(ctx, dBox, box.data(), box.size()));
    RET(dKeep.ensure((size_t)nnz));
    CK(hipMemsetAsync(dKeep.p, 0, (size_t)nnz, ctx->st()));
    LAUNCH(ctx, "spatial_connectivity", k_connectivity, dim3(K), dim3(256), 0, dColptr.as<int64_t>(), dErow.as<int>(), dAval.as<float>(),
           dBox.as<int4>(), d1, d2, dKeep.as<unsigned char>());
    CK(hipMemcpyAsync(A_out, dAval.p, (size_t)nnz * sizeof(float), hipMemcpyDeviceToHost, ctx->st()));
    CK(hipMemcpyAsync(keep, dKeep.p, (size_t)nnz, hipMemcpyDeviceToHost, ctx->st()));
    return wait ? ctx_check_errflag(ctx) : 0;
}

static int postproc_boxes(int32_t d1, int32_t d2, int32_t K, const int64_t *A_colptr, const int32_t *A_rowidx, std::vector<int4> &box) {
    box.assign(K, make_int4(0, 0, 0, 0));
    for (int k = 0; k < K; ++k) {
        int rmin = d1, rmax = -1, cmin = d2, cmax = -1;
        for (int64_t e = A_colptr[k]; e < A_colptr[k + 1]; ++e) {
            int r = A_rowidx[e] % d1, c = A_rowidx[e] / d1;
            rmin = std::min(rmin, r); rmax = std::max(rmax, r); cmin = std::min(cmin, c); cmax = std::max(cmax, c);
        }
        if (rmax < 0) continue;
        int h = rmax - rmin + 5, w = cmax - cmin + 5;
        if (h > PP_MAX || w > PP_MAX)
            return fail(CNMFE_EUNSUPPORTED, "footprint %d spans %dx%d pixels; post-processing supports %dx%d", k, h - 4, w - 4, PP_MAX - 4, PP_MAX - 4);
        box[k] = make_int4(rmin - 2, cmin - 2, h, w);
    }
    return 0;
}

int postproc_run(cnmfe_ctx *ctx, int32_t d1, int32_t d2, int32_t K, const int64_t *A_colptr, const int32_t *A_rowidx,
                 const float *A_val, uint8_t *keep) {
    const int64_t nnz = A_colptr[K];
    if (nnz == 0) return 0;
    std::vector<int4> box(K);
    for (int k = 0; k < K; ++k) {
        int rmin = d1, rmax = -1, cmin = d2, cmax = -1;
        for (int64_t e = A_colptr[k]; e < A_colptr[k + 1]; ++e) {
            int r = A_rowidx[e] % d1, c = A_rowidx[e] / d1;
            rmin = std::min(rmin, r); rmax = std::max(rmax, r); cmin = std::min(cmin, c); cmax = std::max(cmax, c);
        }
        if (rmax < 0) { box[k] = make_int4(0, 0, 0, 0); continue; }
        int h = rmax - rmin + 5, w = cmax - cmin + 5;
        if (h > PP_MAX || w > PP_MAX)
            return fail(CNMFE_EUNSUPPORTED, "footprint %d spans %dx%d pixels; post-processing supports %dx%d", k, h - 4, w - 4, PP_MAX - 4, PP_MAX - 4);
        box[k] = make_int4(rmin - 2, cmin - 2, h, w);
    }
    DevBuf *S_ = ctx->scr;
    DevBuf &dColptr = S_[0], &dErow = S_[1], &dAval = S_[6], &dBox = S_[13], &dKeep = S_[14];
    RET(to_dev(ctx, dColptr, A_colptr, (size_t)K + 1));
    RET(to_dev(ctx, dErow, A_rowidx, (size_t)nnz));
    RET(to_dev(ctx, dAval, A_val, (size_t)nnz));
    RET(to_dev(ctx, dBox, box.data(), box.size()));
    RET(dKeep.ensure((size_t)nnz));
    CK(hipMemsetAsync(dKeep.p, 0, (size_t)nnz, ctx->st()));
    LAUNCH(ctx, "spatial_connectivity", k_connectivity, dim3(K), dim3(256), 0, dColptr.as<int64_t>(), dErow.as<int>(), dAval.as<float>(),
           dBox.as<int4>(), d1, d2, dKeep.as<unsigned char>());
    CK(hipMemcpyAsync(keep, dKeep.p, (size_t)nnz, hipMemcpyDeviceToHost, ctx->st()));
    CK(hipStreamSynchronize(ctx->st()));
    return 0;
}

int tu_warm_factor() { hipFuncAttributes at; return hipFuncGetAttributes(&at, (const void *)k_reduce_parts) == hipSuccess ? 0 : -1; }

}
```

Baseline: 90.59 iter/s.

## Replace small memsets and D2H copies with fused device kernels writing to pinned memory

Several small hipMemsetAsync and hipMemcpyAsync calls are replaced with single kernels that write straight into pinned host memory. This covers ring stats, the ticket flag fetch, the A'A fetch plus overflow plus error flag, and the fused value/keep fetch. The per-pixel asum reduction moves from host to a GPU kernel. Several buffer clears are batched into one kernel, the error word is allocated once at context creation, and the host-side pair/need/work table construction is guarded by a condition. The aim is to cut per-call API overhead, DMA launches and host work, at the cost of kernels doing zero-copy writes over PCIe and of more complex control flow.

```diff
diff --git a/cnmf_e_amd/csrc/api.hip b/cnmf_e_amd/csrc/api.hip
--- a/cnmf_e_amd/csrc/api.hip
+++ b/cnmf_e_amd/csrc/api.hip
@@ -286,15 +286,22 @@
     u.erase(std::unique(u.begin(), u.end()), u.end());
     return u.size() == 2;
 }
+__global__ void __launch_bounds__(128) k_ring_stat_take(int *__restrict__ pmax_dev, const float *__restrict__ W, int64_t d, int p, int *__restrict__ pmax_host,
+                                                        float *__restrict__ row_host) {
+    for (int i = threadIdx.x; i < p; i += 128) row_host[i] = W[(int64_t)i * d];
+    if (threadIdx.x == 0) { pmax_host[0] = pmax_dev[0]; pmax_dev[0] = 0; pmax_host[2] = pmax_dev[2]; pmax_dev[2] = 0; }
+}
 int ring_stats_enqueue(cnmfe_ctx *ctx, Patch *P) {
     const size_t bytes = 64 + (size_t)P->p * sizeof(float);
     if (!P->stat_host) CK(hipHostMalloc(&P->stat_host, bytes, hipHostMallocDefault));
     if (!P->stat_ev) CK(hipEventCreateWithFlags(&P->stat_ev, hipEventDisableTiming));
-    RET(P->stat_dev.ensure(64));
-    CK(hipMemsetAsync(P->stat_dev.p, 0, 64, ctx->st()));
+    if (!P->stat_dev.p) {
+        RET(P->stat_dev.ensure(64));
+        CK(hipMemsetAsync(P->stat_dev.p, 0, 64, ctx->st()));
+    }
     LAUNCH(ctx, "ring_pmax", k_ring_pmax, dim3((unsigned)((P->d + 255) / 256)), dim3(256), 0, P->W.as<float>(), P->d, P->p, P->stat_dev.as<int>());
-    CK(hipMemcpyAsync(P->stat_host, P->stat_dev.p, sizeof(int), hipMemcpyDeviceToHost, ctx->st()));
-    CK(hipMemcpy2DAsync((char *)P->stat_host + 64, sizeof(float), P->W.p, P->d * sizeof(float), sizeof(float), P->p, hipMemcpyDeviceToHost, ctx->st()));
+    LAUNCH(ctx, "ring_stat_take", k_ring_stat_take, dim3(1), dim3(128), 0, P->stat_dev.as<int>(), P->W.as<float>(), P->d, P->p, reinterpret_cast<int *>(P->stat_host),
+           reinterpret_cast<float *>((char *)P->stat_host + 64));
     CK(hipEventRecord(P->stat_ev, ctx->st()));
     P->stat_valid = true;
     return 0;
@@ -309,10 +316,7 @@
 
 int ring_first_run(cnmfe_ctx *ctx, Patch *P, bool *first) { return ring_stats_get(ctx, P, nullptr, first); }
 int ctx_errflag(cnmfe_ctx *ctx, int **dflag) {
-    if (!ctx->errflag.p) {
-        RET(ctx->errflag.ensure(sizeof(int)));
-        CK(hipMemsetAsync(ctx->errflag.p, 0, sizeof(int), ctx->st()));
-    }
+    if (!ctx->errflag.p) return fail(CNMFE_ESTATE, "the context has no error word (cnmfe_create allocates it)");
     *dflag = ctx->errflag.as<int>();
     return 0;
 }
@@ -332,10 +336,59 @@
     if (!h) return 0;
     return errflag_raise(ctx, h);
 }
+struct ClearSegs { uint4 *dst[4]; unsigned long long n16[4]; };
+__global__ void __launch_bounds__(256) k_clear_segs(ClearSegs s) {
+    uint4 *__restrict__ dst = s.dst[blockIdx.y];
+    const unsigned long long n16 = s.n16[blockIdx.y];
+    const uint4 z = make_uint4(0u, 0u, 0u, 0u);
+    for (unsigned long long i = (unsigned long long)blockIdx.x * 256u + threadIdx.x; i < n16; i += (unsigned long long)gridDim.x * 256u) dst[i] = z;
+}
+int clear_bufs(cnmfe_ctx *ctx, int n, void *const *ptrs, const size_t *bytes) {
+    if (n < 1 || n > 4) return fail(CNMFE_EINVAL, "clear_bufs: %d ranges", n);
+    ClearSegs s{};
+    unsigned long long mx = 0;
+    for (int i = 0; i < n; ++i) { s.dst[i] = (uint4 *)ptrs[i]; s.n16[i] = ((unsigned long long)bytes[i] + 15) / 16; mx = std::max(mx, s.n16[i]); }
+    if (!mx) return 0;
+    const unsigned nb = (unsigned)std::min<unsigned long long>((mx + 255) / 256, 2048);
+    LAUNCH(ctx, "clear_bufs", k_clear_segs, dim3(nb, (unsigned)n), dim3(256), 0, s);
+    return 0;
+}
+__global__ void __launch_bounds__(256) k_fetch_words(const int *__restrict__ src, int *__restrict__ dst, unsigned n, const int *__restrict__ word, int *__restrict__ flag) {
+    const unsigned i0 = blockIdx.x * 256u + threadIdx.x;
+    for (unsigned i = i0; i < n; i += gridDim.x * 256u) dst[i] = src[i];
+    if (i0 == 0) { dst[n] = word ? *word : 0; dst[n + 1] = flag ? atomicExch(flag, 0) : 0; }
+}
+int ctx_fetch_check(cnmfe_ctx *ctx, const void *src, size_t n, const int *word, const int **host) {
+    if (n >= (size_t(1) << 31)) return fail(CNMFE_EUNSUPPORTED, "ctx_fetch_check: %zu words", n);
+    const size_t need = (n + 2) * sizeof(int);
+    if (need > ctx->fetch_pin_cap) {
+        if (ctx->fetch_pin) { CK(hipStreamSynchronize(ctx->st())); (void)hipHostFree(ctx->fetch_pin); }
+        ctx->fetch_pin = nullptr; ctx->fetch_pin_cap = 0;
+        CK(hipHostMalloc((void **)&ctx->fetch_pin, need * 2, hipHostMallocDefault));
+        ctx->fetch_pin_cap = need * 2;
+    }
+    const unsigned nb = std::max<unsigned>(1, std::min<unsigned>((unsigned)((n + 255) / 256), 64));
+    LAUNCH(ctx, "fetch_words", k_fetch_words, dim3(nb), dim3(256), 0, (const int *)src, ctx->fetch_pin, (unsigned)n, word, ctx->errflag.as<int>());
+    CK(hipStreamSynchronize(ctx->st()));
+    *host = ctx->fetch_pin;
+    const int h = ctx->fetch_pin[n + 1];
+    if (!h) return 0;
+    return errflag_raise(ctx, h, true);
+}
 __global__ void k_flag_take(int *__restrict__ flag, int *__restrict__ out) { *out = atomicExch(flag, 0); }
 __global__ void __launch_bounds__(256) k_fetch_take(const uint4 *__restrict__ src, uint4 *__restrict__ dst, unsigned n16, int *__restrict__ flag, int *__restrict__ flag_out) {
     for (unsigned i = blockIdx.x * 256u + threadIdx.x; i < n16; i += gridDim.x * 256u) dst[i] = src[i];
     if (flag && blockIdx.x == 0 && threadIdx.x == 0) *flag_out = atomicExch(flag, 0);
+}
+
+__global__ void __launch_bounds__(256) k_fetch2_take(const float *__restrict__ val, float *__restrict__ val_out, const unsigned char *__restrict__ keep,
+                                                     unsigned char *__restrict__ keep_out, unsigned n, int *__restrict__ flag, int *__restrict__ flag_out) {
+    const unsigned stride = gridDim.x * 256u, i0 = blockIdx.x * 256u + threadIdx.x, n4 = n >> 2;
+    for (unsigned i = i0; i < n; i += stride) val_out[i] = val[i];
+    const unsigned *__restrict__ k4 = (const unsigned *)keep; unsigned *__restrict__ o4 = (unsigned *)keep_out;
+    for (unsigned i = i0; i < n4; i += stride) o4[i] = k4[i];
+    if (i0 < (n & 3u)) keep_out[4 * n4 + i0] = keep[4 * n4 + i0];
+    if (flag && i0 == 0) *flag_out = atomicExch(flag, 0);
 }
 
 __global__ void __launch_bounds__(256) k_stitch_add(const float *__restrict__ craw, int64_t ldc, const float *__restrict__ aa, const int *__restrict__ ind,
@@ -442,6 +495,7 @@
     for (auto &kv : patches) delete kv.second;
     prof.drain();
     if (copy_stream) { (void)hipStreamSynchronize(copy_stream); (void)hipStreamDestroy(copy_stream); }
+    if (fetch_pin) (void)hipHostFree(fetch_pin);
     if (ev_bound_ready) (void)hipEventDestroy(ev_bound_ready);
     if (ev_copy_done) (void)hipEventDestroy(ev_copy_done);
     for (auto &g : copy_gens) (void)hipEventDestroy(g.second);
@@ -546,6 +600,7 @@
         hipEventCreateWithFlags(&ctx->ev_copy_done, hipEventDisableTiming) != hipSuccess) { fail(CNMFE_EHIP, "copy stream / events could not be created"); delete ctx; return nullptr; }
     pin_register(ctx, true);
     if (ctx->pin.init(size_t(64) << 20) != 0) { fail(CNMFE_EHIP, "pinned staging arena (64 MB) could not be allocated"); delete ctx; return nullptr; }
+    if (ctx->errflag.ensure(sizeof(int)) != 0 || hipMemsetAsync(ctx->errflag.p, 0, sizeof(int), ctx->stream_) != hipSuccess) { fail(CNMFE_EHIP, "the device error word could not be allocated"); delete ctx; return nullptr; }
     hipLaunchKernelGGL(k_scratch_warm, dim3(1), dim3(64), 0, ctx->stream_, (int *)nullptr, 3);
     hipLaunchKernelGGL(k_scratch_warm, dim3(1), dim3(64), 0, ctx->copy_stream, (int *)nullptr, 3);
     (void)hipStreamSynchronize(ctx->stream_); (void)hipStreamSynchronize(ctx->copy_stream); (void)hipGetLastError();
@@ -938,7 +993,8 @@
     return spatial_fetch(ctx, A_out, nnz);
 }
 
-static int ticket_record(cnmfe_ctx *ctx, int64_t *ticket, const void *src = nullptr, void *dst_pinned = nullptr, size_t bytes = 0) {
+static int ticket_record(cnmfe_ctx *ctx, int64_t *ticket, const void *src = nullptr, void *dst_pinned = nullptr, size_t bytes = 0, const void *keep_src = nullptr,
+                         void *keep_pinned = nullptr) {
     size_t t = 0;
     while (t < ctx->tickets.size() && ctx->ticket_busy[t]) ++t;
     if (t == ctx->tickets.size()) {
@@ -950,14 +1006,16 @@
         if (!ctx->ticket_flags) { CK(hipHostMalloc((void **)&ctx->ticket_flags, cnmfe_ctx::TICKET_FLAGS * sizeof(int), hipHostMallocDefault)); memset(ctx->ticket_flags, 0, cnmfe_ctx::TICKET_FLAGS * sizeof(int)); }
         ctx->ticket_flags[t] = 0;
     }
-    if (bytes) {
+    if (bytes && keep_src) {
+        const unsigned n = (unsigned)(bytes / sizeof(float)), nb = std::min<unsigned>((n + 255) / 256, 64);
+        hipLaunchKernelGGL(k_fetch2_take, dim3(nb), dim3(256), 0, ctx->st(), (const float *)src, (float *)dst_pinned, (const unsigned char *)keep_src, (unsigned char *)keep_pinned, n,
+                           flagged ? ctx->errflag.as<int>() : (int *)nullptr, flagged ? ctx->ticket_flags + t : (int *)nullptr);
+    } else if (bytes) {
         const unsigned n16 = (unsigned)((bytes + 15) / 16), nb = std::min<unsigned>((n16 + 255) / 256, 64);
         hipLaunchKernelGGL(k_fetch_take, dim3(nb), dim3(256), 0, ctx->st(), (const uint4 *)src, (uint4 *)dst_pinned, n16, flagged ? ctx->errflag.as<int>() : (int *)nullptr,
                            flagged ? ctx->ticket_flags + t : (int *)nullptr);
     } else if (flagged) {
-        RET(ctx->ticket_dev.ensure(cnmfe_ctx::TICKET_FLAGS * sizeof(int)));
-        hipLaunchKernelGGL(k_flag_take, dim3(1), dim3(1), 0, ctx->st(), ctx->errflag.as<int>(), ctx->ticket_dev.as<int>() + t);
-        CK(hipMemcpyAsync(&ctx->ticket_flags[t], ctx->ticket_dev.as<int>() + t, sizeof(int), hipMemcpyDeviceToHost, ctx->st()));
+        hipLaunchKernelGGL(k_flag_take, dim3(1), dim3(1), 0, ctx->st(), ctx->errflag.as<int>(), ctx->ticket_flags + t);
     }
     CK(hipEventRecord(ctx->tickets[t], ctx->st()));
     ctx->ticket_busy[t] = 1;
@@ -1008,7 +1066,10 @@
     if (IND_colptr[K] && (!A_out_pinned || !keep_out_pinned)) return fail(CNMFE_EINVAL, "null A_out / keep_out");
     CK(hipSetDevice(ctx->device));
     RET(ctx->activate(ctx->spatial_lane));
-    RET(spatial_fetch_connected(ctx, d1, d2, K, IND_colptr, IND_rowidx, A_out_pinned, keep_out_pinned, false));
+    const int64_t nnz = IND_colptr[K];
+    const bool fused = nnz > 0 && nnz < (int64_t(1) << 31) && ((uintptr_t)keep_out_pinned & 3) == 0;
+    RET(spatial_fetch_connected(ctx, d1, d2, K, IND_colptr, IND_rowidx, A_out_pinned, keep_out_pinned, false, !fused));
+    if (fused) return ticket_record(ctx, ticket, ctx->scr[6].p, A_out_pinned, (size_t)nnz * sizeof(float), ctx->scr[14].p, keep_out_pinned);
     return ticket_record(ctx, ticket);
 }
 
diff --git a/cnmf_e_amd/csrc/bg.hip b/cnmf_e_amd/csrc/bg.hip
--- a/cnmf_e_amd/csrc/bg.hip
+++ b/cnmf_e_amd/csrc/bg.hip
@@ -463,6 +463,14 @@
     if ((threadIdx.x & 63) == 0) atomicAdd(nactive, (int)__popcll(b));
 }
 
+__global__ void __launch_bounds__(256) k_asum(const int *__restrict__ arow, const float *__restrict__ aval, int64_t d_b, float *__restrict__ asum) {
+    const int64_t q = (int64_t)blockIdx.x * 256 + threadIdx.x;
+    if (q >= d_b) return;
+    double s = 0;
+    for (int e = arow[q]; e < arow[q + 1]; ++e) s += aval[e];
+    asum[q] = (float)s;
+}
+
 __global__ void k_b0(const double *__restrict__ ymean, BgGeom g, const int *__restrict__ arow, const int *__restrict__ acol,
                      const float *__restrict__ aval, const double *__restrict__ Cmean, double *__restrict__ b0) {
     int64_t m = (int64_t)blockIdx.x * blockDim.x + threadIdx.x;
@@ -599,7 +607,7 @@
     const int64_t T = P->T;
     const int p = P->p;
     DevBuf &dC = ctx->tmp[0], &dCc = ctx->tmp[1], &dCm = ctx->tmp[2], &dArow = ctx->tmp[3], &dAcol = ctx->tmp[4], &dAval = ctx->tmp[5],
-           &dMisc = ctx->tmp[6], &dAsum = ctx->tmp[7], &dActive = ctx->tmp[8], &dPairs = ctx->tmp[9], &dPairOf = ctx->tmp[10];
+           &dAsum = ctx->tmp[7], &dActive = ctx->tmp[8], &dPairs = ctx->tmp[9], &dPairOf = ctx->tmp[10];
     const bool has_a = K > 0 && A_colptr[K] > 0;
     const bool a_empty = K == 0;
     int64_t ldc = 4;
@@ -639,7 +647,6 @@
     bool first_run = false;
     int pmax = 0;
     RET(ring_stats_get(ctx, P, &pmax, &first_run));
-    RET(dMisc.ensure(64));
     ht.mark("first_run + pmax");
     int kstride = 1;
     if (with_projection) {
@@ -793,14 +800,15 @@
     if (first_run) {
         CK(hipMemsetAsync(dActive.p, 1, P->d, ctx->st()));
     } else {
-        std::vector<float> asum(P->d_b, 0.f);
-        if (a_empty || (b0_only & 2)) std::fill(asum.begin(), asum.end(), 1.0f);
-        else if (has_a) for (int64_t q = 0; q < P->d_b; ++q) { double s = 0; for (int64_t e = csr.rowptr[q]; e < csr.rowptr[q + 1]; ++e) s += csr.val[e]; asum[q] = (float)s; }
-        RET(to_dev(ctx, dAsum, asum.data(), asum.size()));
-        CK(hipMemsetAsync(dMisc.p, 0, 64, ctx->st()));
+        if (has_a && !(a_empty || (b0_only & 2))) {
+            RET(dAsum.ensure((size_t)P->d_b * sizeof(float)));
+            LAUNCH(ctx, "bg_asum", k_asum, dim3((unsigned)((P->d_b + 255) / 256)), dim3(256), 0, dArow.as<int>(), dAval.as<float>(), P->d_b, dAsum.as<float>());
+        } else {
+            std::vector<float> asum(P->d_b, (a_empty || (b0_only & 2)) ? 1.0f : 0.f);
+            RET(to_dev(ctx, dAsum, asum.data(), asum.size()));
+        }
         LAUNCH(ctx, "bg_active", k_active, dim3((unsigned)((P->d + 255) / 256)), dim3(256), 0, P->W.as<float>(), g,
-               P->ring_dr.as<int>(), P->ring_dc.as<int>(), dAsum.as<float>(), dActive.as<unsigned char>(), dMisc.as<int>());
-        CK(hipMemcpyAsync((char *)P->stat_host + 8, dMisc.p, sizeof(int), hipMemcpyDeviceToHost, ctx->st()));
+               P->ring_dr.as<int>(), P->ring_dc.as<int>(), dAsum.as<float>(), dActive.as<unsigned char>(), P->stat_dev.as<int>() + 2);
         nactive = -1;
     }
     LAUNCH(ctx, "bg_b0", k_b0, dim3((unsigned)((P->d + 255) / 256)), dim3(256), 0, P->ymean_d.as<double>(), g,
@@ -808,6 +816,12 @@
 
     ht.mark("ind_active + b0");
     {
+        const size_t sys_bytes_kept = (size_t)P->d * ((size_t)(((p + 15) / 16) * ((p + 15) / 16 + 1) / 2) * 256 + 16 * ((p + 15) / 16)) * sizeof(double);
+        const bool fit_tables = !(incr && !build_base && ctx->opt("solve_packed", 1) != 0 && (int64_t)nblk * std::max(1, K) < (int64_t)1 << 31 &&
+                                  (int64_t)lst_k.size() * BLKPX < (int64_t)1 << 31 && P->sys_valid && P->sys.cap >= sys_bytes_kept && !ctx->opt("debug", 0));
+        int npairs = 0, nwork = 0, nwg = 0;
+        DevBuf &dWork = ctx->tmp[11], &dNeed = ctx->tmp[7], &dTcnt = ctx->tmp[12], &dTl = ctx->tmp[13];
+        if (fit_tables) {
         std::vector<char> touched(nblk, 0);
         {
             const int pi0 = std::max(0, P->roff - g.p_radius) / BLK, pi1 = std::min(P->nr_b - 1, P->roff + P->nr - 1 + g.p_radius) / BLK;
@@ -828,7 +842,7 @@
                         pairs.push_back(make_int4(j * g.nbr + i, j2 * g.nbr + i2, rel, 0));
                     }
             }
-        const int npairs = (int)pairs.size();
+        npairs = (int)pairs.size();
         const int DB = 2 * g.p_radius, DM = 2 * DB + 1;
         std::vector<char> Dm((size_t)DM * DM, 0);
         auto dset = [&](int dr, int dc) { if (dr >= -DB && dr <= DB && dc >= -DB && dc <= DB) Dm[(size_t)(dr + DB) * DM + dc + DB] = 1; };
@@ -863,17 +877,15 @@
                 for (int pi = ih * 8; pi < ih * 8 + 8; ++pi) if ((needmask[pairs[pp].z * 16 + pi] >> (jh * 8)) & 0xff) any = true;
                 if (any) work.push_back(pp * 4 + q);
             }
-        const int nwork = (int)work.size();
+        nwork = (int)work.size();
     ht.mark("pair / need / work tables");
-        DevBuf &dWork = ctx->tmp[11], &dNeed = ctx->tmp[7];
         RET(to_dev(ctx, dPairs, pairs.data(), pairs.size()));
         RET(to_dev(ctx, dPairOf, pair_of.data(), pair_of.size()));
         RET(to_dev(ctx, dWork, work.data(), work.size()));
         RET(to_dev(ctx, dNeed, needmask.data(), needmask.size()));
         RET(ctx->cov.ensure((size_t)npairs * BLKPX * BLKPX * sizeof(double)));
         if (ctx->opt("debug", 0)) CK(hipMemsetAsync(ctx->cov.p, 0xff, (size_t)npairs * BLKPX * BLKPX * sizeof(double), ctx->st()));
-        int nwg = (nwork + 7) / 8 * 8;
-        DevBuf &dTcnt = ctx->tmp[12], &dTl = ctx->tmp[13];
+        nwg = (nwork + 7) / 8 * 8;
         {
             std::vector<int> tcnt((size_t)nrel * 4, 0);
             std::vector<int> tlist((size_t)nrel * 4 * 64, 0);
@@ -887,6 +899,7 @@
                 }
             RET(to_dev(ctx, dTcnt, tcnt.data(), tcnt.size()));
             RET(to_dev(ctx, dTl, tlist.data(), tlist.size()));
+        }
         }
         ht.mark("tile lists + uploads (sync)");
         DevBuf &covT = incr ? P->cov_base : ctx->cov, &rsT = incr ? P->rowsum_base : ctx->rowsum;
diff --git a/cnmf_e_amd/csrc/common.hpp b/cnmf_e_amd/csrc/common.hpp
--- a/cnmf_e_amd/csrc/common.hpp
+++ b/cnmf_e_amd/csrc/common.hpp
@@ -246,7 +246,6 @@
     int copy_batch_mark();
     std::vector<hipEvent_t> tickets; std::vector<char> ticket_busy;
     int *ticket_flags = nullptr;
-    cnmfe::DevBuf ticket_dev;
     static constexpr size_t TICKET_FLAGS = 1024;
     cnmfe::Profiler prof;
     std::map<int, cnmfe::Patch *> patches;
@@ -284,6 +283,7 @@
     int32_t stitch_K = 0; int64_t stitch_T = 0, stitch_ld = 0; bool stitch_open = false;
     void *rccl_comm = nullptr; int rccl_rank = 0, rccl_n = 0;
     cnmfe::DevBuf errflag;
+    int *fetch_pin = nullptr; size_t fetch_pin_cap = 0;
     std::map<std::string, int64_t> opts;
     int trace_level = 0;
     int64_t opt(const char *n, int64_t dflt) const { auto it = opts.find(n); return it == opts.end() ? dflt : it->second; }
@@ -391,12 +391,14 @@
 int ensure_ymean(cnmfe_ctx *ctx, Patch *P);
 int sn_video_run(cnmfe_ctx *ctx, Patch *P, int64_t nframes, float *sn_out);
 int spatial_fetch(cnmfe_ctx *ctx, float *A_out, int64_t nnz);
-int spatial_fetch_connected(cnmfe_ctx *ctx, int32_t d1, int32_t d2, int32_t K, const int64_t *IND_colptr, const int32_t *IND_rowidx, float *A_out, uint8_t *keep, bool wait = true);
+int spatial_fetch_connected(cnmfe_ctx *ctx, int32_t d1, int32_t d2, int32_t K, const int64_t *IND_colptr, const int32_t *IND_rowidx, float *A_out, uint8_t *keep, bool wait = true, bool copy = true);
 int ring_first_run(cnmfe_ctx *ctx, Patch *P, bool *first);
 int ring_stats_enqueue(cnmfe_ctx *ctx, Patch *P);
 int ring_stats_get(cnmfe_ctx *ctx, Patch *P, int *pmax, bool *first);
 int center_traces(cnmfe_ctx *ctx, const float *C, int64_t ldc, int32_t K, int64_t T, DevBuf &Cc, DevBuf &Cmean);
 int upload_centered(cnmfe_ctx *ctx, DevBuf &stage, const float *C, int32_t K, int64_t T, int order, DevBuf &Cc, DevBuf &Cmean, int64_t *ldc_out);
+int clear_bufs(cnmfe_ctx *ctx, int n, void *const *ptrs, const size_t *bytes);
 int ctx_errflag(cnmfe_ctx *ctx, int **dflag);
+int ctx_fetch_check(cnmfe_ctx *ctx, const void *src, size_t n, const int *word, const int **host);
 int ctx_check_errflag(cnmfe_ctx *ctx);
 }
diff --git a/cnmf_e_amd/csrc/factor.hip b/cnmf_e_amd/csrc/factor.hip
--- a/cnmf_e_amd/csrc/factor.hip
+++ b/cnmf_e_amd/csrc/factor.hip
@@ -634,8 +634,12 @@
     RET(to_dev(ctx, dAval, A_val, (size_t)nnz));
     RET(dU.ensure((size_t)K * ldc * sizeof(float)));
     RET(dCraw.ensure((size_t)K * ldc * sizeof(float)));
-    CK(hipMemsetAsync(dU.p, 0, (size_t)K * ldc * sizeof(float), ctx->st()));
-    CK(hipMemsetAsync(dCraw.p, 0, (size_t)K * ldc * sizeof(float), ctx->st()));
+    RET(dOvf.ensure(64));
+    {
+        void *const cp_[3] = {dU.p, dCraw.p, dOvf.p};
+        const size_t cb_[3] = {(size_t)K * ldc * sizeof(float), (size_t)K * ldc * sizeof(float), 64};
+        RET(clear_bufs(ctx, 3, cp_, cb_));
+    }
     const int64_t Tc = (T + 3) / 4;
     const int nchunk = (int)std::max<int64_t>(1, std::min<int64_t>(64, Tc / 32));
     const int64_t tchunk = (Tc + nchunk - 1) / nchunk;
@@ -659,8 +663,6 @@
         if (!virt)
         LAUNCH(ctx, "temporal_proj_U", k_proj_temporal, dim3(K, nchunk), dim3(256), 0, P->ysig.as<float4>(), d, T, dColptr.as<int64_t>(),
                dErow.as<int>(), dAval.as<float>(), tchunk, dU.as<float>(), ldc);
-        RET(dOvf.ensure(64));
-        CK(hipMemsetAsync(dOvf.p, 0, 64, ctx->st()));
         const int rc_ = residual_term_project(ctx, P, K, dColptr.as<int64_t>(), dErow.as<int>(), dAval.as<float>(), dU.as<float>(), ldc, dOvf.as<int>());
         if (rc_ < 0) return rc_;
         if (rc_ > 0) RET(reproject());
@@ -721,11 +723,10 @@
         ht.mark("job queued");
         return 0;
     }
-    std::vector<float> nval(nn);
-    int ovf = 0;
-    CK(hipMemcpyAsync(nval.data(), dNval.p, (size_t)nn * sizeof(float), hipMemcpyDeviceToHost, ctx->st()));
-    if (term_applied) CK(hipMemcpyAsync(&ovf, dOvf.p, sizeof(int), hipMemcpyDeviceToHost, ctx->st()));
-    RET(ctx_check_errflag(ctx));
+    const int *fetched = nullptr;
+    RET(ctx_fetch_check(ctx, dNval.p, (size_t)nn, term_applied ? dOvf.as<int>() : nullptr, &fetched));
+    const float *nval = reinterpret_cast<const float *>(fetched);
+    const int ovf = fetched[nn];
     ht.mark("wait for A'A (sync)");
     if (ovf) RET(reproject());
     std::vector<float> aa(K);
@@ -840,7 +841,7 @@
 
 static int postproc_boxes(int32_t d1, int32_t d2, int32_t K, const int64_t *A_colptr, const int32_t *A_rowidx, std::vector<int4> &box);
 
-int spatial_fetch_connected(cnmfe_ctx *ctx, int32_t d1, int32_t d2, int32_t K, const int64_t *IND_colptr, const int32_t *IND_rowidx, float *A_out, uint8_t *keep, bool wait) {
+int spatial_fetch_connected(cnmfe_ctx *ctx, int32_t d1, int32_t d2, int32_t K, const int64_t *IND_colptr, const int32_t *IND_rowidx, float *A_out, uint8_t *keep, bool wait, bool copy) {
     const int64_t nnz = IND_colptr[K];
     if (ctx->spatial_nnz < 0 || nnz != ctx->spatial_nnz) return fail(CNMFE_ESTATE, "no deferred spatial update of %lld values (last one: %lld)", (long long)nnz, (long long)ctx->spatial_nnz);
     if (nnz == 0) return 0;
@@ -853,6 +854,7 @@
     CK(hipMemsetAsync(dKeep.p, 0, (size_t)nnz, ctx->st()));
     LAUNCH(ctx, "spatial_connectivity", k_connectivity, dim3(K), dim3(256), 0, dColptr.as<int64_t>(), dErow.as<int>(), dAval.as<float>(),
            dBox.as<int4>(), d1, d2, dKeep.as<unsigned char>());
+    if (!copy) return 0;
     CK(hipMemcpyAsync(A_out, dAval.p, (size_t)nnz * sizeof(float), hipMemcpyDeviceToHost, ctx->st()));
     CK(hipMemcpyAsync(keep, dKeep.p, (size_t)nnz, hipMemcpyDeviceToHost, ctx->st()));
     return wait ? ctx_check_errflag(ctx) : 0;
```

Result: no change. 92.25 iter/s, median of 6 (+1.8%).
